# fengweie/UDA_CLR

Hardware: AMD Instinct MI355X
Metric: training images/sec (512x512, src+tgt) at 1/2/4/8 MI355X; val Dice vs ref (higher is better)
Workload: dtype f32

## Files before the change

### include/uda_clr_hip.h

```cpp
#ifndef UDA_CLR_HIP_H
#define UDA_CLR_HIP_H

#include <stdint.h>

#ifdef __cplusplus
extern "C" {
#endif

#define UDA_STAT_SLOTS 16

#define UDA_ACT_NONE 0
#define UDA_ACT_RELU 1
#define UDA_ACT_RELU6 2

typedef struct uda_src {
    const float* x;
    int64_t ldx;
    int32_t N, H, W, C;
    const float* scale;
    const float* shift;
    int32_t act;
    int32_t _pad;
    const uint8_t* mask;
    int64_t ldm;
    float mask_scale;
    float _pad2;
} uda_src_t;

const char* uda_last_error(void);
int uda_version(void);

int uda_relayout_ohwi(const float* w, int O, int I, int k, float* out, void* stream);
int uda_relayout_dgrad(const float* w, int O, int I, int k, float* out, void* stream);
int uda_relayout_dw(const float* w, int C, float* out, void* stream);

#define UDA_MFMA_F32 0
#define UDA_MFMA_BF16X3 1
typedef struct uda_conv_args {
    uda_src_t src;
    const float* w;
    int32_t Cout, ksize, dil;
    int32_t origin;
    const float* bias;
    const float* addend;
    int64_t ld_add;
    float* y;
    int64_t ldy;
    double* stats;
    int32_t mfma;
    int32_t stride;
    const void* x3_src;
    const void* x3_w;
    void* workspace;
    uint64_t workspace_bytes;
} uda_conv_args_t;
int uda_conv_uses_x3(const uda_conv_args_t* a);
uint64_t uda_conv_fwd_workspace_bytes(const uda_conv_args_t* a);
int uda_conv_fwd(const uda_conv_args_t* a, void* stream);
uint64_t uda_x3_packed_bytes(int64_t rows, int K);
int uda_x3_pack(const uda_src_t* src, void* out, void* stream);

typedef struct uda_wgrad_args {
    uda_src_t src;
    const float* dy;
    int64_t lddy;
    int32_t Cout, ksize, dil;
    int32_t origin;
    float* dw;
    float* workspace;
    uint64_t workspace_bytes;
    int32_t mfma;
    int32_t stride;
    const void* x3_src;
    const void* x3_dy;
} uda_wgrad_args_t;
uint64_t uda_conv_wgrad_workspace_bytes(int64_t P, int Cout, int Cin, int ksize);
int uda_conv_wgrad_uses_x3(const uda_wgrad_args_t* a);
int uda_conv_wgrad(const uda_wgrad_args_t* a, void* stream);

uint64_t uda_dwconv_workspace_bytes(int64_t Pout, int C);
int uda_dwconv_fwd(const uda_src_t* src, const float* w9c, int stride, int dil, int border_mode,
                   float* y, int64_t ldy, double* stats , void* stream);
int uda_dwconv_dgrad(const float* dy, int64_t lddy, const float* w9c, int C, int stride, int dil,
                     int N, int H, int W, float* dx, int64_t lddx, void* stream);
int uda_dwconv_wgrad(const uda_src_t* src, const float* dy, int64_t lddy, int stride, int dil,
                     int border_mode, float* dw , float* workspace,
                     uint64_t workspace_bytes, void* stream);

int uda_dwconv_cb_fwd(const uda_src_t* src, const float* w9c, int stride, int dil, int border_mode,
                      float* y, int64_t ldy, double* stats , void* stream);
int uda_dwconv_cb_dgrad(const float* dy, int64_t lddy, const float* w9c, int C, int stride, int dil,
                        int N, int H, int W, float* dx, int64_t lddx, void* stream);
int uda_dwconv_cb_wgrad(const uda_src_t* src, const float* dy, int64_t lddy, int stride, int dil,
                        int border_mode, float* dw , float* workspace,
                        uint64_t workspace_bytes, void* stream);

uint64_t uda_stem_workspace_bytes(int64_t Pout);
int uda_stem_fwd(const float* x, int N, int H, int W, const float* w, float* y, int64_t ldy,
                 double* stats , void* stream);
int uda_stem_wgrad(const float* x, int N, int H, int W, const float* dy, int64_t lddy, float* dw,
                   float* workspace, uint64_t workspace_bytes, void* stream);

uint64_t uda_stem7_workspace_bytes(int64_t Pout);
int uda_stem7_fwd(const float* x, int N, int H, int W, const float* w, float* y, int64_t ldy,
                  double* stats , void* stream);
int uda_stem7_wgrad(const float* x, int N, int H, int W, const float* dy, int64_t lddy, float* dw,
                    float* workspace, uint64_t workspace_bytes, void* stream);
int uda_maxpool_fwd(const uda_src_t* src, float* out, int64_t ldo, uint8_t* idx, int64_t ldi, void* stream);
int uda_maxpool_bwd(const float* dz, int64_t lddz, const uint8_t* idx, int64_t ldi, int N, int H, int W,
                    int C, float* du, int64_t ldu, void* stream);
int uda_rows_stride(const float* src, int64_t ld_src, int N, int H, int W, int C, int stride, int scatter,
                    float* dst, int64_t ld_dst, void* stream);
int uda_bn_add_relu(const uda_src_t* a, const uda_src_t* b, float* out, int64_t ldo, void* stream);
int uda_relu_gate(const float* dz, int64_t lddz, const float* z, int64_t ldz, int64_t P, int C, float* out,
                  int64_t ldo, void* stream);

int uda_relayout_s2d(const float* w, int O, int C, int dgrad, float* out, void* stream);
int uda_s2d_fwd(const float* src, int64_t ld_src, int nchw_in, int N, int Hs, int Ws, int C, int valid_h,
                int valid_w, float slope, float* z, int64_t ld_z, int Hz, int Wz, void* stream);
int uda_s2d_bwd(const float* dz, const float* z_sign, int64_t ld_z, int Hz, int Wz, float slope, int N, int Hs,
                int Ws, int C, int valid_h, int valid_w, float* dst, int64_t ld_dst, int nchw_out, void* stream);
int uda_s2d_bwd_gate(const float* dz, int64_t ld_z, int Hz, int Wz, const float* gate_rows, int64_t ld_gate, float slope,
                     int N, int Hs, int Ws, int C, int valid_h, int valid_w, float* dst, int64_t ld_dst, void* stream);
int uda_x3_pack_s2d_fwd(const float* src, int64_t ld_src, int N, int Hs, int Ws, int C, int valid_h, int valid_w, float slope,
                        int Hz, int Wz, void* out, void* stream);
int uda_x3_pack_s2d_bwd(const float* dz, int64_t ld_z, int Hz, int Wz, const float* gate_rows, int64_t ld_gate, float slope,
                        int N, int Hs, int Ws, int C, int valid_h, int valid_w, void* out, void* stream);

int uda_bn_finalize(const double* stats, int C, double count, const float* gamma, const float* beta,
                    float* running_mean, float* running_var, float momentum, float eps, float* scale,
                    float* shift, float* mean, float* invstd, void* stream);
int uda_bn_running_replay(const float* mean, const float* invstd, int C, double count, int k, float momentum,
                          float eps, float* running_mean, float* running_var, void* stream);
int uda_bn_eval_coeffs(const float* gamma, const float* beta, const float* running_mean,
                       const float* running_var, int C, float eps, float* scale, float* shift,
                       void* stream);
int uda_tn_gain(const double* stats0, const double* stats1, int C, double count0, double count1, float eps,
                float* scale0, float* shift0, float* scale1, float* shift1, float* gain, void* stream);
int uda_tn_eval_coeffs(const float* gamma, const float* beta, const float* running_mean_source,
                       const float* running_var_source, const float* running_mean_target,
                       const float* running_var_target, int C, float eps, float* scale, float* shift, void* stream);
int uda_bn_apply(const uda_src_t* src, const float* residual, int64_t ldr, float* out, int64_t ldo,
                 void* stream);
int uda_colstats(const float* x, int64_t ldx, int64_t P, int C, int nq, double* out, void* stream);
int uda_colstats_window(const float* x, int64_t ldx, int64_t P, int C, int nq, double* out, int out_C, void* stream);
int uda_bnbwd_reduce(const float* dU, int64_t ldu, const uda_src_t* y, const float* mean,
                     const float* invstd, double* sums, void* stream);
int uda_bnbwd_finalize(const double* sums, int C, double count, int q1_border, int act,
                       const float* shift, const float* mean, const float* invstd, const float* q1_total,
                       float* c1, float* c2, float* dgamma, float* dbeta, void* stream);
int uda_bnbwd_apply(const float* dU, int64_t ldu, const uda_src_t* y, const float* mean,
                    const float* invstd, const float* c1, const float* c2, const float* addend,
                    int64_t ld_add, float* out, int64_t ldo, void* stream);
int uda_bnbwd_reduce_lowrank(const float* d, int64_t ldd, int k, const float* w, const uda_src_t* y, const float* mean,
                             const float* invstd, double* sums, void* stream);
int uda_bnbwd_apply_lowrank(const float* d, int64_t ldd, int k, const float* w, const uda_src_t* y, const float* mean,
                            const float* invstd, const float* c1, const float* c2, const float* addend, int64_t ld_add,
                            float* out, int64_t ldo, void* stream);

int uda_upsample_fwd(const float* x, int64_t ldx, int N, int h, int w, int C, float* out,
                     int64_t ldo, int H, int W, void* stream);
int uda_upsample_fwd_stats(const float* x, int64_t ldx, int N, int h, int w, int C, float* out, int64_t ldo, int H, int W,
                           double* stats, int stat_C, void* stream);
int uda_mc_seg_head(const float* feature, int64_t ld_feat, int N, int h, int w, int Cf, const float* low, int64_t ld_low,
                    int Cl, int64_t P_low, const float* boundary, int64_t ld_bnd, int H, int W, const float* scale,
                    const float* shift, int act, const uint8_t* mask, int64_t ldm, float mask_scale, const float* weight,
                    int64_t ldw, const float* bias, float* out, int64_t ldo, void* stream);
int uda_upsample_bwd(const float* dout, int64_t ldo, int N, int H, int W, int C, float* dx,
                     int64_t ldx, int h, int w, void* stream);
int uda_head_upsample_fwd(const float* x, int64_t ldx, int N, int h, int w, int C, float* out,
                          int H, int W, void* stream);
int uda_head_upsample_bwd(const float* dout, int N, int C, int H, int W, float* dx, int64_t ldx,
                          int h, int w, int accumulate, void* stream);
int uda_gap_fwd(const float* x, int64_t ldx, int N, int HW, int C, float scale, float* out,
                int64_t ldo, void* stream);
int uda_broadcast_rows(const float* g, int64_t ldg, int N, int HW, int C, float scale,
                       const float* addend, int64_t ld_add, float* out, int64_t ldo, void* stream);

int uda_dropout_mask(uint8_t* mask, int64_t ldm, int64_t P, int C, float p, uint64_t seed,
                     uint64_t offset, void* stream);

int uda_seg_loss_fwd(const float* o, const float* map, int64_t n_o, const float* b, const float* boundary,
                     int64_t n_b, float* loss3, double* workspace2, void* stream);
int uda_seg_loss_bwd(const float* o, const float* map, int64_t n_o, const float* b, const float* boundary,
                     int64_t n_b, const float* gscale, float* d_o, float* d_b, void* stream);
int uda_seg_counts(const float* logits, const float* target, int B, int C, int64_t HW, float thr,
                   uint64_t* counts, void* stream);

int uda_mc_stats(const float* preds, int T, int64_t n, float* std_map, float* mean_map, void* stream);
int uda_proto_weights(int mode, int B, int h, int w, int H, int W, const float* map, const float* logits,
                      int64_t ldl, const float* std_map, const float* mean_map, float* wts, float* mask0,
                      float* mask1, void* stream);
uint64_t uda_proto_workspace_bytes(int64_t P, int C);
int uda_proto_reduce(const float* feat, int64_t ldf, int64_t P, int C, const float* wts, double* sums,
                     float* workspace, uint64_t workspace_bytes, void* stream);
int uda_proto_finalize(const double* sums, int C, float* centroids , void* stream);
int uda_proto_bwd(const float* feat, int64_t ldf, int64_t P, int C, const float* wts, const double* sums,
                  const float* dC, float* coef_ws , float* d_feat, int64_t ldd,
                  int accumulate, float* d_w, void* stream);

int uda_feat_dot4(const float* feat, int64_t ldf, int64_t P, int C, const float* coef, float* out, void* stream);
int uda_feat_rank4(const float* wts, const float* coef, int64_t P, int C, float* d_feat, int64_t ldd,
                   int accumulate, void* stream);

int uda_adam_step(float* params, const float* grads, float* exp_avg, float* exp_avg_sq, int64_t n, double lr,
                  double beta1, double beta2, double eps, int64_t step, void* stream);

int uda_upconv_fused_stats(int h, int w, int H, int W, int C, int dil);
int uda_upconv_fwd(const float* g, int64_t ldg, int N, int h, int w, int C, int dil, const float* addend, int64_t ld_add,
                   int64_t addend_rows, float* y, int64_t ldy, int H, int W, double* stats, void* stream);
int uda_upconv_bwd(const float* dy, int64_t ldy, int N, int H, int W, int C, int dil, float* dg, int64_t ldg, int h, int w,
                   void* stream);

size_t uda_postprocess_workspace_bytes(int B, int H, int W);
int uda_postprocess(const float* pred, int B, int H, int W, float thr_cup, float thr_disc, int sweeps, uint8_t* out,
                    int* not_converged, void* workspace, size_t workspace_bytes, void* stream);

size_t uda_normalize_tf_workspace_bytes(int B, int H, int W);
int uda_normalize_tf(const uint8_t* image_hwc, const uint8_t* label, int B, int H, int W, const double* gauss_w, int radius,
                     float* image, float* map, float* boundary, void* workspace, size_t workspace_bytes, void* stream);
int uda_field_smooth(const double* noise, int B, int H, int W, const double* weights_dev, int radius, double alpha, double* tmp,
                     double* out, void* stream);
int uda_photometric_u8(uint8_t* image_hwc, int B, int H, int W, const int* sp_pos, const int* sp_count, const int* sp_value,
                       int sp_max, const uint8_t* lut, const int* erase_box, void* stream);
int uda_elastic_warp(const uint8_t* image_hwc, const uint8_t* label, const double* dx, const double* dy, const uint8_t* apply,
                     int B, int H, int W, uint8_t* image_out, uint8_t* label_out, void* stream);

int uda_proto_align_fwd(const float* cur_src, const float* cur_tgt, const float* prev_src, const float* prev_tgt, float keep,
                        float decay, int C, float* new_src, float* new_tgt, float* losses2, void* stream);
int uda_proto_align_bwd(const float* new_src, const float* new_tgt, const float* g_intra, float w_src, float w_tgt, int C,
                        float* d_cur_src, float* d_cur_tgt, void* stream);
int uda_adv_loss_fwd(const float* d1, int n1, const float* d2, int n2, float label, float scale, float* loss, void* stream);
int uda_adv_loss_bwd(const float* d1, int n1, const float* d2, int n2, float label, float scale, const float* g, float* g1,
                     float* g2, void* stream);
int uda_adv_s2d_fwd(const float* logits_nchw, int N, int C, int H, int W, int pre_op, float* z, int64_t ld_z, int Hz, int Wz,
                    void* stream);
int uda_adv_s2d_bwd(const float* dz, int64_t ld_z, int Hz, int Wz, const float* logits_nchw, int N, int C, int H, int W,
                    int pre_op, float* d_logits_nchw, void* stream);

#ifdef __cplusplus
}
#endif
#endif
```

### uda_clr_amd/csrc/bn_elementwise.hip

```cpp
#include "common.h"
#include <stdlib.h>

int uda_reduce_partials(const float* part, int nrows, int ncols, double* out, hipStream_t st);

#define RED_ITER 32
#define RED_CBLK 1024
#define RED_CBLK_SUM 128

__device__ __forceinline__ void st4_guard(float* p, const float v[4], int nvalid) {
    if (nvalid >= 4) {
        uda_st4(p, make_float4(v[0], v[1], v[2], v[3]));
    } else {
#pragma unroll
        for (int j = 0; j < 4; ++j)
            if (j < nvalid) p[j] = v[j];
    }
}

__global__ void bn_finalize_kernel(const double* __restrict__ stats, int C, double count,
                                   const float* __restrict__ gamma, const float* __restrict__ beta,
                                   float* __restrict__ rmean, float* __restrict__ rvar, float momentum, float eps,
                                   float* __restrict__ scale, float* __restrict__ shift,
                                   float* __restrict__ mean, float* __restrict__ invstd) {
    const int c = blockIdx.x * blockDim.x + threadIdx.x;
    if (c >= C) return;
    double s1 = 0.0, s2 = 0.0;
#pragma unroll
    for (int k = 0; k < UDA_STAT_SLOTS; ++k) {
        s1 += stats[(k * 2 + 0) * C + c];
        s2 += stats[(k * 2 + 1) * C + c];
    }
    const double m = s1 / count;
    double var = s2 / count - m * m;
    if (var < 0.0) var = 0.0;
    const double istd = 1.0 / sqrt(var + (double)eps);
    const double sc = (double)gamma[c] * istd;
    mean[c] = (float)m;
    invstd[c] = (float)istd;
    scale[c] = (float)sc;
    shift[c] = (float)((double)beta[c] - m * sc);
    const double unbiased = var * (count / (count > 1.0 ? count - 1.0 : 1.0));
    rmean[c] = (1.f - momentum) * rmean[c] + momentum * (float)m;
    rvar[c] = (1.f - momentum) * rvar[c] + momentum * (float)unbiased;
}

__global__ void bn_eval_coeffs_kernel(const float* __restrict__ gamma, const float* __restrict__ beta,
                                      const float* __restrict__ rmean, const float* __restrict__ rvar, int C,
                                      float eps, float* __restrict__ scale, float* __restrict__ shift) {
    const int c = blockIdx.x * blockDim.x + threadIdx.x;
    if (c >= C) return;
    const double sc = (double)gamma[c] / sqrt((double)rvar[c] + (double)eps);
    scale[c] = (float)sc;
    shift[c] = (float)((double)beta[c] - (double)rmean[c] * sc);
}

extern "C" int uda_bn_finalize(const double* stats, int C, double count, const float* gamma, const float* beta,
                               float* running_mean, float* running_var, float momentum, float eps, float* scale,
                               float* shift, float* mean, float* invstd, void* stream) {
    UDA_REQUIRE(stats && gamma && beta && running_mean && running_var && scale && shift && mean && invstd && C > 0 && count > 0,
                "uda_bn_finalize: bad args");
    hipLaunchKernelGGL(bn_finalize_kernel, dim3(uda_cdiv(C, 256)), dim3(256), 0, (hipStream_t)stream, stats, C, count,
                       gamma, beta, running_mean, running_var, momentum, eps, scale, shift, mean, invstd);
    UDA_LAUNCH_CHECK("bn_finalize");
    return 0;
}

__global__ void bn_running_replay_kernel(const float* __restrict__ mean, const float* __restrict__ invstd, int C,
                                         double count, int k, float momentum, float eps, float* __restrict__ rmean,
                                         float* __restrict__ rvar) {
    const int c = blockIdx.x * blockDim.x + threadIdx.x;
    if (c >= C) return;
    const double is = (double)invstd[c];
    double var = 1.0 / (is * is) - (double)eps;
    if (var < 0.0) var = 0.0;
    const double unbiased = var * (count / (count > 1.0 ? count - 1.0 : 1.0));
    const double a = pow(1.0 - (double)momentum, (double)k);
    rmean[c] = (float)(a * (double)rmean[c] + (1.0 - a) * (double)mean[c]);
    rvar[c] = (float)(a * (double)rvar[c] + (1.0 - a) * unbiased);
}

extern "C" int uda_bn_running_replay(const float* mean, const float* invstd, int C, double count, int k, float momentum,
                                     float eps, float* running_mean, float* running_var, void* stream) {
    UDA_REQUIRE(mean && invstd && running_mean && running_var && C > 0 && count > 0 && k >= 1, "uda_bn_running_replay: bad args");
    hipLaunchKernelGGL(bn_running_replay_kernel, dim3(uda_cdiv(C, 256)), dim3(256), 0, (hipStream_t)stream, mean, invstd, C,
                       count, k, momentum, eps, running_mean, running_var);
    UDA_LAUNCH_CHECK("bn_running_replay");
    return 0;
}

extern "C" int uda_bn_eval_coeffs(const float* gamma, const float* beta, const float* running_mean,
                                  const float* running_var, int C, float eps, float* scale, float* shift, void* stream) {
    UDA_REQUIRE(gamma && beta && running_mean && running_var && scale && shift && C > 0, "uda_bn_eval_coeffs: bad args");
    hipLaunchKernelGGL(bn_eval_coeffs_kernel, dim3(uda_cdiv(C, 256)), dim3(256), 0, (hipStream_t)stream, gamma, beta,
                       running_mean, running_var, C, eps, scale, shift);
    UDA_LAUNCH_CHECK("bn_eval_coeffs");
    return 0;
}

__device__ __forceinline__ double tn_block_sum(double v, double* red) {
    for (int d = 32; d > 0; d >>= 1) v += __shfl_xor(v, d);
    if ((threadIdx.x & 63) == 0) red[threadIdx.x >> 6] = v;
    __syncthreads();
    double t = 0.0;
    for (int w = 0; w < (int)(blockDim.x >> 6); ++w) t += red[w];
    __syncthreads();
    return t;
}

__global__ __launch_bounds__(256) void tn_gain_kernel(const double* __restrict__ st0, const double* __restrict__ st1, int C,
                                                      double n0, double n1, float eps, float* __restrict__ scale0,
                                                      float* __restrict__ shift0, float* __restrict__ scale1,
                                                      float* __restrict__ shift1, float* __restrict__ gain) {
    __shared__ double red[4];
    double part = 0.0;
    for (int c = threadIdx.x; c < C; c += 256) {
        double r[2];
#pragma unroll
        for (int h = 0; h < 2; ++h) {
            const double* st = h ? st1 : st0;
            const double n = h ? n1 : n0;
            double s1 = 0.0, s2 = 0.0;
            for (int k = 0; k < UDA_STAT_SLOTS; ++k) {
                s1 += st[(k * 2 + 0) * C + c];
                s2 += st[(k * 2 + 1) * C + c];
            }
            const double m = s1 / n;
            double var = s2 / n - m * m;
            if (var < 0.0) var = 0.0;
            r[h] = m / sqrt(var * (n / (n - 1.0)) + (double)eps);
        }
        const double prob = 1.0 / (1.0 + fabs(r[0] - r[1]));
        gain[c] = (float)prob;
        part += prob;
    }
    const double total = tn_block_sum(part, red);
    for (int c = threadIdx.x; c < C; c += 256) {
        const float g = (float)(1.0 + (double)C * (double)gain[c] / total);
        gain[c] = g;
        scale0[c] *= g; shift0[c] *= g;
        scale1[c] *= g; shift1[c] *= g;
    }
}

extern "C" int uda_tn_gain(const double* stats0, const double* stats1, int C, double count0, double count1, float eps,
                           float* scale0, float* shift0, float* scale1, float* shift1, float* gain, void* stream) {
    UDA_REQUIRE(stats0 && stats1 && scale0 && shift0 && scale1 && shift1 && gain && C > 0, "uda_tn_gain: bad args");
    UDA_REQUIRE(count0 > 1 && count1 > 1, "uda_tn_gain: each domain half needs more than 1 value per channel (got %g, %g)", count0, count1);
    hipLaunchKernelGGL(tn_gain_kernel, dim3(1), dim3(256), 0, (hipStream_t)stream, stats0, stats1, C, count0, count1, eps,
                       scale0, shift0, scale1, shift1, gain);
    UDA_LAUNCH_CHECK("tn_gain");
    return 0;
}

__global__ __launch_bounds__(256) void tn_eval_coeffs_kernel(const float* __restrict__ gamma, const float* __restrict__ beta,
                                                             const float* __restrict__ rms, const float* __restrict__ rvs,
                                                             const float* __restrict__ rmt, const float* __restrict__ rvt, int C,
                                                             float eps, float* __restrict__ scale, float* __restrict__ shift) {
    __shared__ double red[4];
    double part = 0.0;
    for (int c = threadIdx.x; c < C; c += 256) {
        const double rs = (double)rms[c] / sqrt((double)rvs[c] + (double)eps);
        const double rt = (double)rmt[c] / sqrt((double)rvt[c] + (double)eps);
        const double prob = 1.0 / (1.0 + fabs(rs - rt));
        scale[c] = (float)prob;
        part += prob;
    }
    const double total = tn_block_sum(part, red);
    for (int c = threadIdx.x; c < C; c += 256) {
        const double g = 1.0 + (double)C * (double)scale[c] / total;
        const double sc = (double)gamma[c] / sqrt((double)rvt[c] + (double)eps);
        scale[c] = (float)(sc * g);
        shift[c] = (float)(((double)beta[c] - (double)rmt[c] * sc) * g);
    }
}

extern "C" int uda_tn_eval_coeffs(const float* gamma, const float* beta, const float* running_mean_source,
                                  const float* running_var_source, const float* running_mean_target,
                                  const float* running_var_target, int C, float eps, float* scale, float* shift, void* stream) {
    UDA_REQUIRE(gamma && beta && running_mean_source && running_var_source && running_mean_target && running_var_target &&
                scale && shift && C > 0, "uda_tn_eval_coeffs: bad args");
    hipLaunchKernelGGL(tn_eval_coeffs_kernel, dim3(1), dim3(256), 0, (hipStream_t)stream, gamma, beta, running_mean_source,
                       running_var_source, running_mean_target, running_var_target, C, eps, scale, shift);
    UDA_LAUNCH_CHECK("tn_eval_coeffs");
    return 0;
}

#define EW_ITER 16
__global__ __launch_bounds__(256) void bn_apply_kernel(uda_src_t s, const float* __restrict__ res, int64_t ldr,
                                                       float* __restrict__ out, int64_t ldo, int64_t P) {
    const int C = s.C, cblk0 = blockIdx.y * RED_CBLK;
    const int Cb = min(RED_CBLK, C - cblk0), G = (Cb + 3) >> 2, PP = 256 / G;
    const int tid = threadIdx.x, cg = tid % G, pl = tid / G;
    if (pl >= PP) return;
    const int c0 = cblk0 + cg * 4;
    Xf4 xf;
    uda_load_xf4(xf, s.scale, s.shift, c0, C);
    const bool has_xf = s.scale != nullptr;
    const int64_t base = (int64_t)blockIdx.x * (PP * EW_ITER);
#pragma unroll 4
    for (int it = 0; it < EW_ITER; ++it) {
        const int64_t p = base + (int64_t)it * PP + pl;
        if (p >= P) break;
        const float4 xv = uda_ld4(s.x + p * s.ldx + c0);
        float v[4] = {xv.x, xv.y, xv.z, xv.w};
        uint32_t mk = 0x01010101u;
        if (s.mask) mk = *reinterpret_cast<const uint32_t*>(s.mask + p * s.ldm + c0);
        float r[4] = {0.f, 0.f, 0.f, 0.f};
        if (res) {
            const float4 rv = uda_ld4(res + p * ldr + c0);
            r[0] = rv.x; r[1] = rv.y; r[2] = rv.z; r[3] = rv.w;
        }
#pragma unroll
        for (int j = 0; j < 4; ++j) {
            float u = v[j];
            if (has_xf) u = u * xf.sc[j] + xf.sh[j];
            u = uda_act(u, s.act);
            if (s.mask) u *= (float)((mk >> (8 * j)) & 0xffu) * s.mask_scale;
            v[j] = u + r[j];
        }
        st4_guard(out + p * ldo + c0, v, C - c0);
    }
}

static int src_check(const uda_src_t* s, const char* who) {
    UDA_REQUIRE(s && s->x && uda_aligned16(s->x) && s->ldx % 4 == 0 && s->ldx >= ((s->C + 3) / 4) * 4 && s->C > 0,
                "%s: src must be 16-byte aligned with ldx %% 4 == 0 and >= round4(C)", who);
    UDA_REQUIRE((s->scale == nullptr) == (s->shift == nullptr), "%s: scale/shift must come together", who);
    if (s->mask) UDA_REQUIRE(s->ldm % 4 == 0 && s->ldm >= ((s->C + 3) / 4) * 4 && (reinterpret_cast<uintptr_t>(s->mask) & 3u) == 0,
                             "%s: bad mask layout", who);
    return 0;
}
// ... 370 lines not shown
```

### uda_clr_amd/csrc/igemm_conv.hip

```cpp
#include <algorithm>
#include "common.h"
#include <stdlib.h>
#include "igemm_args.h"

typedef float f32x16 __attribute__((ext_vector_type(16)));


#define IGC_MIN_WAVES(TM, TN, PIPE) ((PIPE) ? 2 : ((TM) * (TN) <= 3 ? 4 : 3))
template <int TM, int TN, int WM, int WN, bool PIPE = false, int XF = -1>
__global__ __launch_bounds__(256) void igemm_conv_kernel(ConvKArgs a) {
    constexpr int BM = 32 * TM * WM, BN = 32 * TN * WN;
    constexpr int A_IT = BM / 32, B_IT = BN / 32;
    constexpr int TILE = (BM + BN) * IG_LD;
    extern __shared__ __attribute__((aligned(16))) float smem[];

    const int tid = threadIdx.x, lane = tid & 63, wave = tid >> 6;
    const int wm = wave / WN, wn = wave % WN;
    const int lid = uda_xcd_remap(blockIdx.x, a.nMt * a.nNt);
    const int mt = lid / a.nNt, nt = lid % a.nNt;
    const int H = a.src.H, W = a.src.W, C = a.src.C;
    const int64_t P = (int64_t)a.src.N * H * W;
    const int64_t m0 = (int64_t)mt * BM;
    const int n0 = nt * BN;

// ... 153 lines not shown
            for (int i = 0; i < TM; ++i) af[i] = uda_ld4(&As[(arow + 32 * i) * IG_LD + g * 8 + koff]);
#pragma unroll
            for (int j = 0; j < TN; ++j) bf[j] = uda_ld4(&Bs[(brow + 32 * j) * IG_LD + g * 8 + koff]);
#pragma unroll
            for (int s = 0; s < 4; ++s) {
#pragma unroll
                for (int i = 0; i < TM; ++i) {
                    const float av = s == 0 ? af[i].x : s == 1 ? af[i].y : s == 2 ? af[i].z : af[i].w;
#pragma unroll
                    for (int j = 0; j < TN; ++j) {
                        const float bv = s == 0 ? bf[j].x : s == 1 ? bf[j].y : s == 2 ? bf[j].z : bf[j].w;
                        acc[i][j] = __builtin_amdgcn_mfma_f32_32x32x2f32(av, bv, acc[i][j], 0, 0, 0);
                    }
                }
            }
        }
    };
    float* As = smem;
    float* Bs = smem + BM * IG_LD;
    if constexpr (PIPE) {
        float* As1 = smem + TILE;
        float* Bs1 = As1 + BM * IG_LD;
        issue(0, R0);
        issue(1, R1);
        stage(R0, As, Bs);
        issue(2, R0);
        for (int c = 0; c < nchunks; c += 2) {
            __syncthreads();
            stage(R1, As1, Bs1);
            issue(c + 3, R1);
            math(As, Bs);
            __syncthreads();
            stage(R0, As, Bs);
            issue(c + 4, R0);
            if (c + 1 < nchunks) math(As1, Bs1);
        }
    } else {
        issue(0, R0);
        for (int c = 0; c < nchunks; ++c) {
            __syncthreads();
            stage(R0, As, Bs);
            __syncthreads();
            if (c + 1 < nchunks) issue(c + 1, R0);
            math(As, Bs);
        }
    }

    const int colb = n0 + wn * TN * 32 + (lane & 31);
    const bool vec_ok = uda_aligned16_dev(a.y) && (a.ldy & 3) == 0 && (!a.addend || (uda_aligned16_dev(a.addend) && (a.ld_add & 3) == 0));
    __syncthreads();
    float* patch = smem + wave * (32 * IG_LD);
    float s1[TN], s2[TN];
#pragma unroll
    for (int j = 0; j < TN; ++j) {
        s1[j] = 0.f;
        s2[j] = 0.f;
        const int col = colb + 32 * j;
        const bool cok = col < a.Cout;
        const float bv = (cok && a.bias) ? a.bias[col] : 0.f;
#pragma unroll
        for (int i = 0; i < TM; ++i) {
            const int64_t rbase = m0 + wm * TM * 32 + 32 * i;
#pragma unroll
            for (int r = 0; r < 16; ++r) {
                const int rl = (r & 3) + 8 * (r >> 2) + 4 * (lane >> 5);
                const float v = acc[i][j][r] + bv;
                if (cok && rbase + rl < P) {
                    s1[j] += v;
                    s2[j] += v * v;
                }
                if (vec_ok) {
                    patch[rl * IG_LD + (lane & 31)] = v;
                } else if (cok && rbase + rl < P) {
                    a.y[(rbase + rl) * a.ldy + col] = a.addend ? v + a.addend[(rbase + rl) * a.ld_add + col] : v;
                }
            }
            if (vec_ok) {
                const int cb = n0 + wn * TN * 32 + 32 * j + (lane & 7) * 4;
#pragma unroll
                for (int rq = 0; rq < 4; ++rq) {
                    const int rl = rq * 8 + (lane >> 3);
                    const int64_t row = rbase + rl;
                    float4 o = uda_ld4(&patch[rl * IG_LD + (lane & 7) * 4]);
                    if (row < P && cb < a.Cout) {
                        if (cb + 3 < a.Cout) {
                            if (a.addend) {
                                const float4 ad = uda_ld4(a.addend + row * a.ld_add + cb);
                                o.x += ad.x; o.y += ad.y; o.z += ad.z; o.w += ad.w;
                            }
                            uda_st4(a.y + row * a.ldy + cb, o);
                        } else {
                            const float ov[4] = {o.x, o.y, o.z, o.w};
                            for (int q = 0; q < 4; ++q)
                                if (cb + q < a.Cout) a.y[row * a.ldy + cb + q] = a.addend ? ov[q] + a.addend[row * a.ld_add + cb + q] : ov[q];
                        }
                    }
                }
            }
        }
    }
    if (a.stats) {
        __syncthreads();
        float* red = smem;
#pragma unroll
        for (int j = 0; j < TN; ++j) {
            const float t1 = s1[j] + __shfl_xor(s1[j], 32);
            const float t2 = s2[j] + __shfl_xor(s2[j], 32);
            if (lane < 32) {
                const int cl = wn * TN * 32 + 32 * j + lane;
                red[(wm * 2 + 0) * BN + cl] = t1;
                red[(wm * 2 + 1) * BN + cl] = t2;
            }
        }
        __syncthreads();
        double* dst = a.stats + (int64_t)(mt % UDA_STAT_SLOTS) * 2 * a.Cout;
        for (int e = tid; e < 2 * BN; e += 256) {
            const int qd = e / BN, cl = e % BN;
            if (n0 + cl < a.Cout) {
                float t = 0.f;
#pragma unroll
                for (int m = 0; m < WM; ++m) t += red[(m * 2 + qd) * BN + cl];
                atomicAdd(&dst[qd * a.Cout + n0 + cl], (double)t);
            }
        }
    }
}

__global__ void reduce_partials_kernel(const float* __restrict__ part, int nrows, int ncols,
                                       int rows_per_seg, double* __restrict__ out) {
    __shared__ double red[4][64];
    const int cl = threadIdx.x & 63, rg = threadIdx.x >> 6;
    const int col = blockIdx.x * 64 + cl;
    const int r0 = blockIdx.y * rows_per_seg;
    const int r1 = min(nrows, r0 + rows_per_seg);
    double s = 0.0;
    if (col < ncols)
        for (int r = r0 + rg; r < r1; r += 4) s += (double)part[(int64_t)r * ncols + col];
    red[rg][cl] = s;
    __syncthreads();
    if (rg == 0 && col < ncols) atomicAdd(&out[col], red[0][cl] + red[1][cl] + red[2][cl] + red[3][cl]);
}

int uda_reduce_partials(const float* part, int nrows, int ncols, double* out, hipStream_t st) {
    int segs = nrows / 64;
    if (segs < 1) segs = 1;
    if (segs > 64) segs = 64;
    const int rps = (nrows + segs - 1) / segs;
    dim3 grid(uda_cdiv(ncols, 64), uda_cdiv(nrows, rps));
    hipLaunchKernelGGL(reduce_partials_kernel, grid, dim3(256), 0, st, part, nrows, ncols, rps, out);
    UDA_LAUNCH_CHECK("reduce_partials");
    return 0;
}

static inline int uda_k_row(int C, int ksize) {
    const int Kc = ((C + 3) / 4) * 4;
    if (ksize == 1 || Kc < IG_BK) return ksize * ksize * Kc;
    return ((Kc + IG_BK - 1) / IG_BK) * ksize * ksize * IG_BK;
}

static int check_src(const uda_src_t& s, const char* who) {
    UDA_REQUIRE(s.x && uda_aligned16(s.x), "%s: src.x must be 16-byte aligned", who);
    UDA_REQUIRE(s.ldx % 4 == 0 && s.ldx >= ((s.C + 3) / 4) * 4, "%s: src.ldx=%lld must be a multiple of 4 and >= round4(C=%d)",
                who, (long long)s.ldx, s.C);
    UDA_REQUIRE(s.N > 0 && s.H > 0 && s.W > 0 && s.C > 0, "%s: bad src dims", who);
    UDA_REQUIRE((s.scale == nullptr) == (s.shift == nullptr), "%s: scale/shift must come together", who);
    if (s.mask) UDA_REQUIRE(s.ldm % 4 == 0 && (reinterpret_cast<uintptr_t>(s.mask) & 3u) == 0 && s.ldm >= ((s.C + 3) / 4) * 4,
                            "%s: mask must be 4-byte aligned with ldm %% 4 == 0", who);
    return 0;
}

__global__ __launch_bounds__(256) void conv_cout1_kernel(ConvKArgs a) {
    const int lane = threadIdx.x & 63;
    const int64_t p = (int64_t)blockIdx.x * 4 + (threadIdx.x >> 6);
    const int H = a.src.H, W = a.src.W;
    const int64_t P = (int64_t)a.src.N * H * W;
    if (p >= P) return;
    const int pw = (int)(p % W), ph = (int)((p / W) % H);
    const int T = a.ksize * a.ksize;
    float acc = 0.f;
    for (int t = 0; t < T; ++t) {
        const int th = t / a.ksize;
        const int hh = ph + (th - a.cen) * a.dil, ww = pw + (t - th * a.ksize - a.cen) * a.dil;
        if (hh < 0 || hh >= H || ww < 0 || ww >= W) continue;
        const float* xr = a.src.x + (p + (int64_t)(hh - ph) * W + (ww - pw)) * a.src.ldx;
        for (int c = lane * 4; c < a.Kc; c += 256) {
            const int kq = (T == 1 || a.Kc < IG_BK) ? t * a.Kc + c : ((c / IG_BK) * T + t) * IG_BK + (c % IG_BK);
            const float4 xv = uda_ld4(xr + c), wv = uda_ld4(a.w + kq);
            float s = xv.x * wv.x;
            if (c + 1 < a.src.C) s += xv.y * wv.y;
            if (c + 2 < a.src.C) s += xv.z * wv.z;
            if (c + 3 < a.src.C) s += xv.w * wv.w;
            acc += s;
        }
    }
#pragma unroll
    for (int o = 32; o > 0; o >>= 1) acc += __shfl_xor(acc, o);
    if (lane == 0) {
        float v = acc + (a.bias ? a.bias[0] : 0.f);
        if (a.addend) v += a.addend[p * a.ld_add];
        a.y[p * a.ldy] = v;
    }
}

template <int NO>
__global__ __launch_bounds__(256) void conv_heads_kernel(ConvKArgs a) {
    extern __shared__ __attribute__((aligned(16))) float hsm[];
    const int Kc = a.Kc, C = a.src.C;
    for (int e = threadIdx.x; e < Kc; e += 256) {
        const bool in = e < C;
        hsm[e] = (in && a.src.scale) ? a.src.scale[e] : 1.f;
        hsm[Kc + e] = (in && a.src.shift) ? a.src.shift[e] : 0.f;
#pragma unroll
        for (int o = 0; o < NO; ++o) hsm[(2 + o) * Kc + e] = in ? a.w[(int64_t)o * a.Ktot + e] : 0.f;
    }
    __syncthreads();
    const int l16 = threadIdx.x & 15, pl = threadIdx.x >> 4;
    const int64_t P = (int64_t)a.src.N * a.src.H * a.src.W;
    const float alo = a.src.act == ACT_NONE ? -INFINITY : 0.f, ahi = a.src.act == ACT_RELU6 ? 6.f : INFINITY;
    const float ms = a.src.mask_scale;
    const int G = Kc >> 2;
    for (int it = 0; it < 8; ++it) {
        const int64_t p = (int64_t)blockIdx.x * 128 + it * 16 + pl;
        float acc[NO];
#pragma unroll
        for (int o = 0; o < NO; ++o) acc[o] = 0.f;
        if (p < P) {
            const float* xr = a.src.x + p * a.src.ldx;
            for (int g = l16; g < G; g += 16) {
                const int c = g * 4;
                float4 xv = uda_ld4(xr + c);
                const float4 sc = uda_ld4(&hsm[c]), sh = uda_ld4(&hsm[Kc + c]);
                if (c + 4 > C) {
                    if (c + 1 >= C) xv.y = 0.f;
                    if (c + 2 >= C) xv.z = 0.f;
                    xv.w = 0.f;
                }
                float u[4] = {__builtin_amdgcn_fmed3f(xv.x * sc.x + sh.x, alo, ahi), __builtin_amdgcn_fmed3f(xv.y * sc.y + sh.y, alo, ahi),
                              __builtin_amdgcn_fmed3f(xv.z * sc.z + sh.z, alo, ahi), __builtin_amdgcn_fmed3f(xv.w * sc.w + sh.w, alo, ahi)};
                if (a.src.mask) {
                    uint32_t mk = *reinterpret_cast<const uint32_t*>(a.src.mask + p * a.src.ldm + c);
                    if (c + 4 > C) mk &= 0xffffffffu >> (8 * (c + 4 - C));
                    u[0] *= (float)(mk & 0xffu) * ms; u[1] *= (float)((mk >> 8) & 0xffu) * ms;
                    u[2] *= (float)((mk >> 16) & 0xffu) * ms; u[3] *= (float)(mk >> 24) * ms;
                }
#pragma unroll
                for (int o = 0; o < NO; ++o) {
                    const float4 wv = uda_ld4(&hsm[(2 + o) * Kc + c]);
                    acc[o] += u[0] * wv.x + u[1] * wv.y + u[2] * wv.z + u[3] * wv.w;
                }
            }
        }
#pragma unroll
        for (int o = 0; o < NO; ++o) {
#pragma unroll
            for (int d = 8; d > 0; d >>= 1) acc[o] += __shfl_xor(acc[o], d);
        }
        if (l16 == 0 && p < P) {
#pragma unroll
            for (int o = 0; o < NO; ++o) {
                float v = acc[o] + (a.bias ? a.bias[o] : 0.f);
                if (a.addend) v += a.addend[p * a.ld_add + o];
                a.y[p * a.ldy + o] = v;
            }
        }
    }
}

template <int KH, int NB>
__global__ __launch_bounds__(256, 2) void conv1x1_stream_kernel(ConvKArgs a, int64_t P, int ntiles, int ngroups) {
    const int lane = threadIdx.x & 63, r = lane & 31, h = lane >> 5;
    const int wave = (int)((blockIdx.x * blockDim.x + threadIdx.x) >> 6), nwaves = (int)((gridDim.x * blockDim.x) >> 6);
    const int K = 2 * KH;
    const int grp = wave % ngroups, col0 = grp * (NB * 32);
    float b[NB][KH];
#pragma unroll
    for (int nb = 0; nb < NB; ++nb) {
        const int col = col0 + nb * 32 + r;
#pragma unroll
        for (int q = 0; q < KH / 4; ++q) {
            float4 v = make_float4(0.f, 0.f, 0.f, 0.f);
            if (col < a.Cout) v = uda_ld4(a.w + (int64_t)col * K + h * KH + 4 * q);
            b[nb][4 * q] = v.x; b[nb][4 * q + 1] = v.y; b[nb][4 * q + 2] = v.z; b[nb][4 * q + 3] = v.w;
        }
    }
    const bool has_xf = a.src.scale != nullptr;
    const bool xf16 = has_xf && ((reinterpret_cast<uintptr_t>(a.src.scale) | reinterpret_cast<uintptr_t>(a.src.shift)) & 15) == 0;
    const float alo = a.src.act == ACT_NONE ? -INFINITY : 0.f, ahi = a.src.act == ACT_RELU6 ? 6.f : INFINITY;
    double s1[NB], s2[NB];
#pragma unroll
    for (int nb = 0; nb < NB; ++nb) s1[nb] = s2[nb] = 0.0;
    constexpr int OOB = 0x7ffffff0;
    const int ldy4 = (int)a.ldy * 4, lda4 = (int)a.ld_add * 4;
    for (int t = wave / ngroups; t < ntiles; t += nwaves / ngroups) {
        const int64_t p0 = (int64_t)t * 32;
        const int64_t p = min(p0 + r, P - 1);
        float av[KH];
#pragma unroll
        for (int q = 0; q < KH / 4; ++q) {
            const float4 v = uda_ld4(a.src.x + p * a.src.ldx + h * KH + 4 * q);
            av[4 * q] = v.x; av[4 * q + 1] = v.y; av[4 * q + 2] = v.z; av[4 * q + 3] = v.w;
        }
        if (has_xf) {
#pragma unroll
            for (int q = 0; q < KH / 4; ++q) {
                float4 sc, sh;
                if (xf16) {
                    sc = uda_ld4(a.src.scale + h * KH + 4 * q);
// ... 281 lines not shown
    constexpr int ARPP = 256 / AV, BRPP = 256 / BV;
    constexpr int APASS = WGN_BKP / ARPP, BPASS = WGN_BKP / BRPP;
    __shared__ __attribute__((aligned(16))) float smem[WGN_BKP * (BM + BN)];
    float* As = smem;
    float* Bs = smem + WGN_BKP * BM;

    const int tid = threadIdx.x, lane = tid & 63, wave = tid >> 6;
    const int wm = wave / WN, wn = wave % WN;
    const int cot = blockIdx.x / a.nJt, jt = blockIdx.x % a.nJt;
    const int split = blockIdx.y;
    const int H = a.src.H, W = a.src.W, C = a.src.C;
    const int64_t P = (int64_t)a.src.N * H * W;

    const int acv = (tid % AV) * 4, apr = tid / AV;
    const int co = cot * BM + acv;
    const int bjv = (tid % BV) * 4, bpr = tid / BV;
    const int j0 = jt * BN + bjv;
    const bool jok = j0 < a.Jtot;
    int t = 0, ci = j0;
    if (a.ksize >= 2 && jok) {
        t = j0 / a.Kc;
        ci = j0 - t * a.Kc;
    }
    int dh = 0, dw = 0;
    if (a.ksize >= 2) {
        const int th = a.ksize == 3 ? t / 3 : t >> 1;
        dh = (th - a.cen) * a.dil;
        dw = (t - th * a.ksize - a.cen) * a.dil;
    }
    Xf4 xf;
    uda_load_xf4(xf, a.src.scale, a.src.shift, ci, jok ? C : 0);
    const bool has_xf = a.src.scale != nullptr;
    const int act = a.src.act;
    const float ms = a.src.mask_scale;

    float4 areg[APASS], breg[BPASS];
    uint32_t bmask[BPASS];
    unsigned bok = 0, aok = 0;

    auto issue = [&](int chunk) {
        const int64_t p0 = (int64_t)chunk * WGN_BKP;
        const int64_t plast = P - 1;
        const int coc = min(co, a.Cout > 4 ? a.Cout - 4 : 0);
        aok = 0;
#pragma unroll
        for (int i = 0; i < APASS; ++i) {
            const int64_t p = p0 + apr + i * ARPP;
            areg[i] = uda_ld4(a.dy + min(p, plast) * a.lddy + (co < a.Cout ? co : coc));
            aok |= ((p < P && co < a.Cout) ? 1u : 0u) << i;
        }
        bok = 0;
#pragma unroll
        for (int i = 0; i < BPASS; ++i) {
            const int64_t p = p0 + bpr + i * BRPP;
            bool in = jok && p < P;
            int64_t q = min(p, plast);
            if (a.ksize >= 2) {
                const int w0 = (int)(q % W), h0 = (int)((q / W) % H);
                const int hh = h0 + dh, ww = w0 + dw;
                const bool inside = hh >= 0 && hh < H && ww >= 0 && ww < W;
                in = in && inside;
                q = inside ? q + (int64_t)dh * W + dw : q;
            }
            const int cic = jok ? ci : 0;
            breg[i] = uda_ld4(a.src.x + q * a.src.ldx + cic);
            bmask[i] = a.src.mask ? *reinterpret_cast<const uint32_t*>(a.src.mask + q * a.src.ldm + cic) : 0x01010101u;
            bok |= (in ? 1u : 0u) << i;
        }
    };
    auto stage = [&]() {
#pragma unroll
        for (int i = 0; i < APASS; ++i) {
            float v[4] = {areg[i].x, areg[i].y, areg[i].z, areg[i].w};
            const bool oka = (aok >> i) & 1u;
#pragma unroll
            for (int j = 0; j < 4; ++j)
                if (!oka || co + j >= a.Cout) v[j] = 0.f;
            uda_st4(&As[(apr + i * ARPP) * BM + acv], make_float4(v[0], v[1], v[2], v[3]));
        }
        typedef float f32x2 __attribute__((ext_vector_type(2)));
        const f32x2 sc01 = {xf.sc[0], xf.sc[1]}, sc23 = {xf.sc[2], xf.sc[3]};
        const f32x2 sh01 = {xf.sh[0], xf.sh[1]}, sh23 = {xf.sh[2], xf.sh[3]};
        const bool masked = a.src.mask != nullptr;
#pragma unroll
        for (int i = 0; i < BPASS; ++i) {
            const bool ok = (bok >> i) & 1u;
            f32x2 t01 = {breg[i].x, breg[i].y}, t23 = {breg[i].z, breg[i].w};
            if (has_xf) {
                t01 = t01 * sc01 + sh01;
                t23 = t23 * sc23 + sh23;
            }
            t01 = f32x2{uda_act(t01.x, act), uda_act(t01.y, act)};
            t23 = f32x2{uda_act(t23.x, act), uda_act(t23.y, act)};
            if (masked) {
                const uint32_t mk = bmask[i];
                t01 *= f32x2{(float)(mk & 0xffu), (float)((mk >> 8) & 0xffu)} * ms;
                t23 *= f32x2{(float)((mk >> 16) & 0xffu), (float)(mk >> 24)} * ms;
            }
            float v[4] = {t01.x, t01.y, t23.x, t23.y};
#pragma unroll
            for (int j = 0; j < 4; ++j)
                if (!(ok && (ci + j) < C)) v[j] = 0.f;
            uda_st4(&Bs[(bpr + i * BRPP) * BN + bjv], make_float4(v[0], v[1], v[2], v[3]));
        }
    };

    f32x16 acc[TM][TN];
#pragma unroll
    for (int i = 0; i < TM; ++i)
#pragma unroll
        for (int j = 0; j < TN; ++j)
#pragma unroll
            for (int r = 0; r < 16; ++r) acc[i][j][r] = 0.f;

    const int c0 = split * a.chunks_per_split;
    const int c1 = min(a.nchunks, c0 + a.chunks_per_split);
    const int acol = wm * TM * 32 + (lane & 31), bcol = wn * TN * 32 + (lane & 31);
    const int kh = lane >> 5;
    if (c0 < c1) issue(c0);
    for (int c = c0; c < c1; ++c) {
        __syncthreads();
        stage();
        __syncthreads();
        if (c + 1 < c1) issue(c + 1);
#pragma unroll
        for (int kk = 0; kk < WGN_BKP / 2; ++kk) {
            float af[TM], bf[TN];
#pragma unroll
            for (int i = 0; i < TM; ++i) af[i] = As[(2 * kk + kh) * BM + acol + 32 * i];
#pragma unroll
            for (int j = 0; j < TN; ++j) bf[j] = Bs[(2 * kk + kh) * BN + bcol + 32 * j];
#pragma unroll
            for (int i = 0; i < TM; ++i)
#pragma unroll
                for (int j = 0; j < TN; ++j)
                    acc[i][j] = __builtin_amdgcn_mfma_f32_32x32x2f32(af[i], bf[j], acc[i][j], 0, 0, 0);
        }
    }
    float* slab = a.slab + (int64_t)split * a.Cout * a.Jtot;
#pragma unroll
    for (int i = 0; i < TM; ++i)
#pragma unroll
        for (int j = 0; j < TN; ++j) {
            const int col = jt * BN + wn * TN * 32 + 32 * j + (lane & 31);
#pragma unroll
            for (int r = 0; r < 16; ++r) {
                const int row = cot * BM + wm * TM * 32 + 32 * i + (r & 3) + 8 * (r >> 2) + 4 * (lane >> 5);
                if (row < a.Cout && col < a.Jtot) slab[(int64_t)row * a.Jtot + col] = acc[i][j][r];
            }
        }
}

template <int Q>
__global__ __launch_bounds__(256) void wgrad_reduce_kernel(const float* __restrict__ slab, int S, int Cout, int Cin, int T,
                                                           int Kc, float* __restrict__ dw) {
    constexpr int NO = 256 / Q;
    __shared__ float red[Q][NO + 1];
    const int64_t total = (int64_t)Cout * T * Cin;
    const int64_t stride = (int64_t)Cout * T * Kc;
    const int ol = threadIdx.x % NO, q = threadIdx.x / NO;
    for (int64_t e0 = (int64_t)blockIdx.x * NO; e0 < total; e0 += (int64_t)gridDim.x * NO) {
        const int64_t e = e0 + ol;
        float s = 0.f;
        int64_t dst = 0;
        if (e < total) {
            const int ci = (int)(e % Cin);
            const int t = (int)((e / Cin) % T);
            const int co = (int)(e / ((int64_t)Cin * T));
            dst = ((int64_t)co * Cin + ci) * T + t;
            const float* src = slab + ((int64_t)co * T + t) * Kc + ci;
            int k = q;
            float s0 = 0.f, s1 = 0.f, s2 = 0.f, s3 = 0.f;
            for (; k + 3 * Q < S; k += 4 * Q) {
                s0 += src[(int64_t)k * stride];
                s1 += src[(int64_t)(k + Q) * stride];
                s2 += src[(int64_t)(k + 2 * Q) * stride];
                s3 += src[(int64_t)(k + 3 * Q) * stride];
            }
            for (; k < S; k += Q) s0 += src[(int64_t)k * stride];
            s = (s0 + s1) + (s2 + s3);
        }
        red[q][ol] = s;
        __syncthreads();
        if (q == 0 && e < total) {
            float acc[8];
#pragma unroll
            for (int j = 0; j < 8; ++j) acc[j] = 0.f;
#pragma unroll
            for (int j = 0; j < Q; ++j) acc[j & 7] += red[j][ol];
            dw[dst] = ((acc[0] + acc[1]) + (acc[2] + acc[3])) + ((acc[4] + acc[5]) + (acc[6] + acc[7]));
        }
        __syncthreads();
    }
}

struct WgradPlan {
    int bm, bn, nCot, nJt, S, cps, nchunks;
};

static WgradPlan wgrad_plan(int64_t P, int Cout, int Cin, int ksize) {
    WgradPlan p;
    const int Kc = ((Cin + 3) / 4) * 4, J = ksize * ksize * Kc;
    const int cm = Cout <= 32 ? 32 : (Cout <= 64 ? 64 : 128);
    const int cn = J <= 32 ? 32 : (J <= 64 ? 64 : 128);
    const bool big = Cout >= 192 && J >= 256 && uda_cdiv(P, WG_BKP) >= 4096;
    if (big) { p.bm = 256; p.bn = 256; }
    else if (cm == 128 && cn == 32) { p.bm = 128; p.bn = 32; }
    else if (cm == 32 && cn == 128) { p.bm = 32; p.bn = 128; }
    else if (cm <= 64 && cn <= 64) { p.bm = 64; p.bn = 64; }
    else { p.bm = 128; p.bn = 128; }
    p.nCot = uda_cdiv(Cout, p.bm);
    p.nJt = uda_cdiv(J, p.bn);
    p.nchunks = uda_cdiv(P, ((p.bm == 128 && p.bn == 128) || p.bm == 256) ? WG_BKP : WGN_BKP);
    int S = (p.bm == 256 ? 512 : 1024) / (p.nCot * p.nJt);
    if (S > p.nchunks / 4) S = p.nchunks / 4;
    if (S < 1) S = 1;
    const int scap = (int64_t)Cout * J <= 8192 ? 1024 : 256;
    if (S > scap) S = scap;
    p.cps = uda_cdiv(p.nchunks, S);
    p.S = uda_cdiv(p.nchunks, p.cps);
    return p;
}

extern "C" uint64_t uda_conv_wgrad_workspace_bytes(int64_t P, int Cout, int Cin, int ksize) {
    const WgradPlan p = wgrad_plan(P, Cout, Cin, ksize);
    const int Kc = ((Cin + 3) / 4) * 4;
    return (uint64_t)p.S * Cout * ksize * ksize * Kc * sizeof(float);
}

extern "C" int uda_conv_wgrad_uses_x3(const uda_wgrad_args_t* a) {
    if (!a || a->mfma != UDA_MFMA_BF16X3 || a->ksize < 1 || a->ksize > 3) return 0;
    const int sd = a->stride <= 1 ? 1 : a->stride;
    const int64_t P = (int64_t)a->src.N * ((a->src.H - 1) / sd + 1) * ((a->src.W - 1) / sd + 1);
    const WgradPlan p = wgrad_plan(P, a->Cout, a->src.C, a->ksize);
    const bool wide = p.bm == 256 || (p.bm == 128 && p.bn == 128);
    return wide && wgrad_x3_eligible(a->src.C, a->Cout, a->ksize, P) ? 1 : 0;
}

extern "C" int uda_conv_wgrad(const uda_wgrad_args_t* a, void* stream) {
    hipStream_t st = (hipStream_t)stream;
    UDA_REQUIRE(a != nullptr, "uda_conv_wgrad: null args");
    if (int e = check_src(a->src, "uda_conv_wgrad")) return e;
    UDA_REQUIRE(a->ksize >= 1 && a->ksize <= 3, "uda_conv_wgrad: ksize must be 1, 2 or 3");
    UDA_REQUIRE(a->ksize != 2 || a->origin == 0 || a->origin == 1, "uda_conv_wgrad: origin must be 0 or 1 for ksize 2");
    UDA_REQUIRE(a->dy && uda_aligned16(a->dy) && a->lddy % 4 == 0 && a->lddy >= ((a->Cout + 3) / 4) * 4,
                "uda_conv_wgrad: dy must be 16-byte aligned with lddy %% 4 == 0 and >= round4(Cout)");
    const int sd = a->stride <= 1 ? 1 : a->stride;
    UDA_REQUIRE(sd <= 2, "uda_conv_wgrad: stride must be 1 or 2");
    const int Ho = (a->src.H - 1) / sd + 1, Wo = (a->src.W - 1) / sd + 1;
    const int64_t P = (int64_t)a->src.N * Ho * Wo;
    const WgradPlan p = wgrad_plan(P, a->Cout, a->src.C, a->ksize);
    UDA_REQUIRE(a->workspace && a->workspace_bytes >= uda_conv_wgrad_workspace_bytes(P, a->Cout, a->src.C, a->ksize),
                "uda_conv_wgrad: workspace too small");
    UDA_REQUIRE(sd == 1 || p.bm == 256 || (p.bm == 128 && p.bn == 128),
                "uda_conv_wgrad: stride 2 is built on the wide-tile kernels only (Cout > 64, K > 64)");
    WgradKArgs k;
    k.src = a->src;
    k.stride = sd; k.Ho = Ho; k.Wo = Wo;
    k.dy = a->dy;
    k.lddy = a->lddy;
    k.Cout = a->Cout;
    k.ksize = a->ksize;
    k.dil = a->dil;
    k.cen = a->ksize == 3 ? 1 : (a->ksize == 2 ? a->origin : 0);
    k.Kc = ((a->src.C + 3) / 4) * 4;
    k.Jtot = a->ksize * a->ksize * k.Kc;
    k.slab = a->workspace;
    k.nCot = p.nCot;
    k.nJt = p.nJt;
    k.chunks_per_split = p.cps;
    k.nchunks = p.nchunks;
    dim3 grid(p.nCot * p.nJt, p.S);
    int S_used = p.S;
    if (uda_conv_wgrad_uses_x3(a)) { if (int e = launch_wgrad_x3(k, P, p.S, a->x3_src, a->x3_dy, st, S_used)) return e; }
    else if (p.bm == 256) { if (int e = launch_wgrad_ws(k, p.S, true, st)) return e; }
    else if (p.bm == 128 && p.bn == 128) { if (int e = launch_wgrad_ws(k, p.S, false, st)) return e; }
    else if (p.bm == 64) hipLaunchKernelGGL((igemm_wgrad_kernel<1, 1, 2, 2>), grid, dim3(256), 0, st, k);
    else if (p.bm == 128) hipLaunchKernelGGL((igemm_wgrad_kernel<1, 1, 4, 1>), grid, dim3(256), 0, st, k);
    else hipLaunchKernelGGL((igemm_wgrad_kernel<1, 1, 1, 4>), grid, dim3(256), 0, st, k);
    UDA_LAUNCH_CHECK("igemm_wgrad");
    const int T = a->ksize * a->ksize;
    const int64_t total = (int64_t)a->Cout * T * a->src.C;
    if (S_used > 256)
        hipLaunchKernelGGL(wgrad_reduce_kernel<64>, dim3(uda_cdiv(total, 4) > 4096 ? 4096 : uda_cdiv(total, 4)), dim3(256), 0, st,
                           k.slab, S_used, a->Cout, a->src.C, T, k.Kc, a->dw);
    else
        hipLaunchKernelGGL(wgrad_reduce_kernel<8>, dim3(uda_cdiv(total, 32) > 4096 ? 4096 : uda_cdiv(total, 32)), dim3(256), 0, st,
                           k.slab, S_used, a->Cout, a->src.C, T, k.Kc, a->dw);
    UDA_LAUNCH_CHECK("wgrad_reduce");
    return 0;
}

__device__ __forceinline__ void uda_k_decode(int64_t e, int T, int Kr, int Kc, int& c, int& t, int& row) {
    const int k = (int)(e % Kr);
    row = (int)(e / Kr);
    if (T == 1) {
        c = k;
        t = 0;
    } else if (Kc < IG_BK) {
        t = k / Kc;
        c = k - t * Kc;
    } else {
        const int chunk = k / IG_BK;
        t = chunk % T;
        c = (chunk / T) * IG_BK + (k % IG_BK);
    }
}
__global__ void relayout_ohwi_kernel(const float* __restrict__ w, int O, int I, int T, int Kr, float* __restrict__ out) {
    const int64_t total = (int64_t)O * Kr;
    const int Kc = ((I + 3) / 4) * 4;
    for (int64_t e = (int64_t)blockIdx.x * blockDim.x + threadIdx.x; e < total; e += (int64_t)gridDim.x * blockDim.x) {
        int ci, t, o;
        uda_k_decode(e, T, Kr, Kc, ci, t, o);
        out[e] = ci < I ? w[((int64_t)o * I + ci) * T + t] : 0.f;
    }
}
__global__ void relayout_dgrad_kernel(const float* __restrict__ w, int O, int I, int T, int Kr, float* __restrict__ out) {
    const int64_t total = (int64_t)I * Kr;
    const int Kc = ((O + 3) / 4) * 4;
    for (int64_t e = (int64_t)blockIdx.x * blockDim.x + threadIdx.x; e < total; e += (int64_t)gridDim.x * blockDim.x) {
        int o, t, ci;
        uda_k_decode(e, T, Kr, Kc, o, t, ci);
        out[e] = o < O ? w[((int64_t)o * I + ci) * T + (T - 1 - t)] : 0.f;
    }
}
__global__ void relayout_dw_kernel(const float* __restrict__ w, int C, float* __restrict__ out) {
    const int e = blockIdx.x * blockDim.x + threadIdx.x;
    if (e < 9 * C) out[e] = w[(e % C) * 9 + e / C];
}

static inline int grid_for(int64_t total) {
    int g = uda_cdiv(total, 256);
    return g > 4096 ? 4096 : (g < 1 ? 1 : g);
}

extern "C" int uda_relayout_ohwi(const float* w, int O, int I, int k, float* out, void* stream) {
    UDA_REQUIRE(w && out && O > 0 && I > 0 && (k >= 1 && k <= 3), "uda_relayout_ohwi: bad args");
    const int Kr = uda_k_row(I, k);
    hipLaunchKernelGGL(relayout_ohwi_kernel, dim3(grid_for((int64_t)O * Kr)), dim3(256), 0, (hipStream_t)stream,
                       w, O, I, k * k, Kr, out);
    UDA_LAUNCH_CHECK("relayout_ohwi");
    return 0;
}
extern "C" int uda_relayout_dgrad(const float* w, int O, int I, int k, float* out, void* stream) {
    UDA_REQUIRE(w && out && O > 0 && I > 0 && (k >= 1 && k <= 3), "uda_relayout_dgrad: bad args");
    const int Kr = uda_k_row(O, k);
    hipLaunchKernelGGL(relayout_dgrad_kernel, dim3(grid_for((int64_t)I * Kr)), dim3(256), 0, (hipStream_t)stream,
                       w, O, I, k * k, Kr, out);
    UDA_LAUNCH_CHECK("relayout_dgrad");
    return 0;
}
extern "C" int uda_relayout_dw(const float* w, int C, float* out, void* stream) {
    UDA_REQUIRE(w && out && C > 0, "uda_relayout_dw: bad args");
    hipLaunchKernelGGL(relayout_dw_kernel, dim3(uda_cdiv(9 * C, 256)), dim3(256), 0, (hipStream_t)stream, w, C, out);
    UDA_LAUNCH_CHECK("relayout_dw");
    return 0;
}
```

### uda_clr_amd/engine.py

```python
from __future__ import annotations

from typing import Dict, Optional

import torch

import os as _os

_MC_VIRTUAL = _os.environ.get("UDA_CLR_MC_VIRTUAL", "1") != "0"
_NATIVE_S2 = _os.environ.get("UDA_CLR_NATIVE_STRIDE2", "1") != "0"
POISON_BUFFERS = False

from .acts import ACT_NONE, ACT_RELU, ACT_RELU6, Act, BNRec, nchw_view, round4
from .domain_split import DomainSplit

BN_EPS = 1e-5
BN_MOMENTUM = 0.1

_MBV2 = ((1, 16, 1, 1), (6, 24, 2, 2), (6, 32, 3, 2), (6, 64, 4, 2), (6, 96, 3, 1),
         (6, 160, 3, 2), (6, 320, 1, 1))

DROPOUT = {"aspp.dropout": 0.5, "decoder.last_conv_boundary.3": 0.5,
           "decoder.last_conv_boundary.7": 0.1, "decoder.last_conv.2": 0.1}


def block_plan(output_stride: int = 16):
    plan, inp, cur, rate = [], 32, 2, 1
    for t, c, n, s in _MBV2:
        if cur == output_stride:
            stride, dil = 1, rate
            rate *= s
        else:
            stride, dil = s, 1
            cur *= s
        for i in range(n):
            plan.append((inp, c, stride if i == 0 else 1, dil, t))
            inp = c
    return plan


def _rows(g: torch.Tensor) -> torch.Tensor:
    n, c, h, w = g.shape
    return g.permute(0, 2, 3, 1).reshape(n * h * w, c)


STAT_SLOTS = 16


class _Arena:

    def __init__(self, like, n_doubles):
        self.buf = torch.zeros(n_doubles, dtype=torch.float64, device=like.device)
        self.off = 0

    def take(self, nq, C, halves=1):
        n = halves * STAT_SLOTS * nq * C
        if self.off + n > self.buf.numel():
            raise RuntimeError("statistics arena exhausted")
        v = self.buf[self.off:self.off + n]
        v = v.view(STAT_SLOTS, nq, C) if halves == 1 else v.view(halves, STAT_SLOTS, nq, C)
        self.off += n
        return v


class _Ctx:
    __slots__ = ("S", "N", "dims", "w_cache", "params", "x", "arena", "nbt", "bnlog", "tn_repeat", "need_grad")

    def __init__(self):
        self.S = {}
        self.w_cache = {}
        self.arena = None
        self.nbt = []
        self.bnlog = []
        self.tn_repeat = False


def resnet_plan(output_stride: int = 16, layers=(3, 4, 23)):
    if output_stride == 16:
        strides, dils = (1, 2, 2, 1), (1, 1, 1, 2)
    elif output_stride == 8:
        strides, dils = (1, 2, 1, 1), (1, 1, 2, 4)
    else:
        raise NotImplementedError
    plan, inp = [], 64
    for li, (planes, n) in enumerate(zip((64, 128, 256), layers), start=1):
        for b in range(n):
            st = strides[li - 1] if b == 0 else 1
            plan.append(("backbone.layer%d.%d" % (li, b), inp, planes, st, dils[li - 1],
                         b == 0 and (st != 1 or inp != 4 * planes)))
            inp = 4 * planes
    for b, mg in enumerate((1, 2, 4)):
        st = strides[3] if b == 0 else 1
        plan.append(("backbone.layer4.%d" % b, inp, 512, st, mg * dils[3], b == 0 and (st != 1 or inp != 2048)))
        inp = 2048
    return plan


class GeneratorEngine:
    C_FEAT = 256

    def __init__(self, kernels, output_stride: int = 16, seed: int = 1337, backbone: str = "mobilenet",
                 transnorm: bool = False):
        self.tn = bool(transnorm)
        self.K = DomainSplit(kernels) if self.tn else kernels
        self.os = output_stride
        self.backbone = backbone
        self.dils = (1, 6, 12, 18) if output_stride == 16 else (1, 12, 24, 36)
        self.seed = seed
        self.rng_offset = 0
        self.nonfinite = None
        if backbone == "mobilenet":
            self.blocks = block_plan(output_stride)
            self.c_high, self.c_low = 320, 24
            n = 32
            for inp, oup, stride, dil, t in self.blocks:
                n += (inp * t if t != 1 else 0) + inp * t + oup
        elif backbone == "resnet":
            self.rblocks = resnet_plan(output_stride)
            self.c_high, self.c_low = 2048, 256
            n = 64
            for pre, inp, planes, stride, dil, has_ds in self.rblocks:
                n += 2 * planes + 4 * planes * (2 if has_ds else 1)
        elif backbone == "xception":
            from .networks.backbone.xception import exit_plan, xception_plan
            self.xblocks, self.xexit = xception_plan(output_stride), exit_plan(output_stride)
            self.c_high, self.c_low = 2048, 128
            n = 32 + 64
            for name, inp, planes, stride, has_skip, seps in self.xblocks:
                n += sum(ci + co for _, ci, co, _, _ in seps) + (planes if has_skip else 0)
            n += sum(ci + co for _, _, ci, co, _ in self.xexit)
        else:
            raise NotImplementedError("backbone %r" % (backbone,))
        self.bn_channels = n + 5 * 256 + 256 + 48 + 256 + 256 + 305

    def _check_arena(self, ctx):
        if ctx.arena is not None:
            bad = ~torch.isfinite(ctx.arena.buf.sum())
            self.nonfinite = bad if self.nonfinite is None else (self.nonfinite | bad)

    def pop_nonfinite(self):
        f, self.nonfinite = self.nonfinite, None
        return f

    @staticmethod
    def _empty(x, *shape, dtype=torch.float32):
        t = torch.empty(shape, dtype=dtype, device=x.device)
        if POISON_BUFFERS and dtype == torch.float32 and t.dim() == 2:
            t.copy_(torch.tensor([float("nan"), float("inf"), -float("inf"), 3.0e38], device=x.device)[
                torch.arange(t.shape[0], device=x.device) % 4].unsqueeze(1).expand_as(t))
        return t

    def _buf(self, x, P, C):
        return self._empty(x, P, round4(C))[:, :C]

    def _stats(self, ctx, C, training):
        return ctx.arena.take(2, C, 2 if self._split(ctx) else 1) if training else None

    def _split(self, ctx):
        return self.tn and not ctx.tn_repeat

    def _w(self, ctx, key, kind):
        ck = (key, kind)
        if ck not in ctx.w_cache:
            w = ctx.params[key]
            K, CF = self.K, self.C_FEAT

            def taps(t):
                return t[:, :CF].permute(2, 3, 0, 1).reshape(9 * t.shape[0], CF, 1, 1).contiguous()
            ctx.w_cache[ck] = {"ohwi": K.relayout_ohwi, "dgrad": K.relayout_dgrad,
                               "dw": K.relayout_dw,
                               "dwflip": lambda t: K.relayout_dw(t).flip(0).contiguous(),
                               "up_taps": lambda t: K.relayout_ohwi(taps(t)),
                               "up_taps_dgrad": lambda t: K.relayout_dgrad(taps(t)),
                               "low_ohwi": lambda t: K.relayout_ohwi(t[:, CF:].contiguous()),
                               "low_dgrad": lambda t: K.relayout_dgrad(t[:, CF:].contiguous())}[kind](w)
        return ctx.w_cache[ck]

    def _bn(self, ctx, prefix, stats, count, training, scale, shift, mean=None, invstd=None,
            q1=False, N=None) -> Optional[BNRec]:
        p = ctx.params
        g, b = p[prefix + ".weight"], p[prefix + ".bias"]
        if self.tn:
            return self._tn(ctx, prefix, stats, count, training, scale, shift, mean, invstd, q1, ctx.N if N is None else N)
        rm, rv = p[prefix + ".running_mean"], p[prefix + ".running_var"]
        if training:
            if count <= 1:
                raise ValueError("Expected more than 1 value per channel when training (%s)" % prefix)
            self.K.bn_finalize(stats, float(count), g, b, rm, rv, BN_MOMENTUM, BN_EPS,
                               scale, shift, mean, invstd)
            nbt = p.get(prefix + ".num_batches_tracked")
            if nbt is not None:
                ctx.nbt.append(nbt)
            rec = BNRec(prefix, mean, invstd, float(count), q1)
            ctx.bnlog.append((prefix, rec))
            return rec
        self.K.bn_eval_coeffs(g, b, rm, rv, BN_EPS, scale, shift)
        if not ctx.need_grad:
            return None
        istd = torch.rsqrt(rv + BN_EPS)
        if mean is not None:
            mean.copy_(rm)
            invstd.copy_(istd)
            return BNRec(prefix, mean, invstd, float("inf"), q1, frozen=True)
        return BNRec(prefix, rm, istd, float("inf"), q1, frozen=True)

    def _tn(self, ctx, prefix, stats, count, training, scale, shift, mean, invstd, q1, N):
        p, K = ctx.params, self.K
        g, b = p[prefix + ".weight"], p[prefix + ".bias"]
        rms, rvs = p[prefix + ".running_mean_source"], p[prefix + ".running_var_source"]
        rmt, rvt = p[prefix + ".running_mean_target"], p[prefix + ".running_var_target"]
        if not training:
            K.tn_eval_coeffs(g, b, rms, rvs, rmt, rvt, BN_EPS, scale, shift)
            if not ctx.need_grad:
                return None
            rs, rt = rms / torch.sqrt(rvs + BN_EPS), rmt / torch.sqrt(rvt + BN_EPS)
            prob = 1.0 / (1.0 + (rs - rt).abs())
            gain = 1.0 + prob.numel() * prob / prob.sum()
            istd = torch.rsqrt(rvt + BN_EPS)
            if mean is not None:
                mean.copy_(rmt)
                invstd.copy_(istd)
                return BNRec(prefix, mean, invstd, float("inf"), q1, gain, frozen=True)
            return BNRec(prefix, rmt, istd, float("inf"), q1, gain, frozen=True)
        if ctx.tn_repeat:
            if count <= 1:
                raise ValueError("Expected more than 1 value per channel when training (%s)" % prefix)
            K.bn_finalize(stats, float(count), g, b, rms.clone(), rvs.clone(), BN_MOMENTUM, BN_EPS, scale, shift, mean, invstd)
            scale.mul_(2.0)
            shift.mul_(2.0)
            rec = BNRec(prefix, mean, invstd, float(count), q1)
            ctx.bnlog.append((prefix, rec))
            return rec
        n0 = N // 2
        per_image = count // N
        counts = (float(n0 * per_image), float((N - n0) * per_image))
        if min(counts) <= 1:
            raise ValueError("Expected more than 1 value per channel when training (%s, TransNorm halves of %d and %d "
                             "images)" % (prefix, n0, N - n0))
        for h, (rm, rv) in enumerate(((rms, rvs), (rmt, rvt))):
            K.bn_finalize(stats[h], counts[h], g, b, rm, rv, BN_MOMENTUM, BN_EPS, scale[h], shift[h], mean[h], invstd[h])
        gain = torch.empty_like(g)
        K.tn_gain(stats[0], stats[1], counts[0], counts[1], BN_EPS, scale[0], shift[0], scale[1], shift[1], gain)
        ctx.nbt.append(p[prefix + ".num_batches_tracked"])
        rec = BNRec(prefix, mean, invstd, counts, q1, gain)
        ctx.bnlog.append((prefix, rec))
        return rec

    def _coef(self, ctx, x, C, training):
        return self._empty(x, 4, 2, C) if (self._split(ctx) and training) else self._empty(x, 4, C)

    def _bn_act(self, ctx, prefix, y, N, H, W, stats, count, training, act, mask=None,
                mask_scale=1.0, q1=False) -> Act:
        C = y.shape[1]
        coef = self._coef(ctx, y, C, training)
        rec = self._bn(ctx, prefix, stats, count, training, coef[0], coef[1], coef[2], coef[3], q1, N)
        return Act(y, N, H, W, coef[0], coef[1], act, mask, mask_scale, rec,
                   split=N // 2 if (self._split(ctx) and training) else 0)

    def _mask(self, x, name, P, C, N, H, W, training, masks):
        if not training:
            return None, 1.0
        p = DROPOUT[name]
        m = torch.empty((P, round4(C)), dtype=torch.uint8, device=x.device)[:, :C]
        if masks is not None:
            m.copy_(_rows(masks[name].to(x.device)))
        else:
            self.K.dropout_mask(m, p, self.seed, self.rng_offset)
            self.rng_offset += 1
        return m, 1.0 / (1.0 - p)

    def _conv0(self, ctx, feature, xf, N, H16, W16, H4, W4, out, stats, y0=None):
        K, key = self.K, "decoder.last_conv_boundary.0.weight"
        CF = self.C_FEAT
        Cout = out.shape[1]
        if y0 is None:
            y0 = self._empty(out, out.shape[0], Cout)
            K.conv(Act(xf[:, CF:CF + 48], N, H4, W4), self._w(ctx, key, "low_ohwi"), 3, 1, y0)
        g = self._empty(out, feature.shape[0], 9 * Cout)
        K.conv(Act(feature, N, H16, W16), self._w(ctx, key, "up_taps"), 1, 1, g)
        if self.tn and stats is not None:
            K.upconv_fwd(g, N, H16, W16, out, H4, W4, addend=y0)
            K.colstats(out, stats, N=N)
        else:
            K.upconv_fwd(g, N, H16, W16, out, H4, W4, addend=y0, stats=stats)
        return y0

    def _mobilenet_forward(self, ctx, x, training):
        K, S, params = self.K, ctx.S, ctx.params
        N, _, Hin, Win = x.shape
        H, W = (Hin - 1) // 2 + 1, (Win - 1) // 2 + 1
        y0 = self._buf(x, N * H * W, 32)
        st = self._stats(ctx, 32, training)
        K.stem_fwd(x, params["backbone.features.0.0.weight"], y0, st)
        a = self._bn_act(ctx, "backbone.features.0.1", y0, N, H, W, st, N * H * W, training, ACT_RELU6)
        S["stem"] = a
        recs = []
        low = None
        for i, (inp, oup, stride, dil, t) in enumerate(self.blocks, start=1):
            pre = "backbone.features.%d" % i
            zin, H, W = a, a.H, a.W
            hid = inp * t
            if t != 1:
                ye = self._buf(x, N * H * W, hid)
                st = self._stats(ctx, hid, training)
                K.conv(zin, self._w(ctx, pre + ".conv.0.weight", "ohwi"), 1, 1, ye, stats=st)
                cnt = N * (H + 2 * dil) * (W + 2 * dil)
                e = self._bn_act(ctx, pre + ".conv.1", ye, N, H, W, st, cnt, training, ACT_RELU6, q1=True)
                border, kd, kdb, kp, kpb = 1, ".conv.3", ".conv.4", ".conv.6", ".conv.7"
            else:
                e, border, kd, kdb, kp, kpb = zin, 0, ".conv.0", ".conv.1", ".conv.3", ".conv.4"
            Ho, Wo = (H - 1) // stride + 1, (W - 1) // stride + 1
            Po = N * Ho * Wo
            yd = self._buf(x, Po, hid)
            st = self._stats(ctx, hid, training)
            K.dwconv_fwd(e, self._w(ctx, pre + kd + ".weight", "dw"), stride, dil, border, yd, st)
            d = self._bn_act(ctx, pre + kdb, yd, N, Ho, Wo, st, Po, training, ACT_RELU6)
            yp = self._buf(x, Po, oup)
            st = self._stats(ctx, oup, training)
            K.conv(d, self._w(ctx, pre + kp + ".weight", "ohwi"), 1, 1, yp, stats=st)
            pb = self._bn_act(ctx, pre + kpb, yp, N, Ho, Wo, st, Po, training, ACT_NONE)
            use_res = stride == 1 and inp == oup
            z = self._buf(x, Po, oup)
            K.bn_apply(pb, z, zin.x if use_res else None)
            a = Act(z, N, Ho, Wo)
            recs.append(dict(pre=pre, t=t, stride=stride, dil=dil, zin=zin, e=e, d=d, pb=pb,
                             use_res=use_res, border=border, keys=(kd, kdb, kp, kpb)))
            if i == 3:
                low = a
        S["blocks"] = recs
# ... 160 lines not shown
            else:
                dU_stem = dUe
        dy0 = self._bn_backward(ctx, G, S["stem"], dU_stem)
        dw0 = torch.empty_like(ctx.params["backbone.features.0.0.weight"])
        K.stem_wgrad(x, dy0, dw0)
        G["backbone.features.0.0.weight"] = dw0

    def _sep_forward(self, ctx, v, pre, bn_key, cout, stride, dil, training, act):
        K, N = self.K, ctx.N
        Ho, Wo = (v.H - 1) // stride + 1, (v.W - 1) // stride + 1
        Po, cin = N * Ho * Wo, v.C
        yd = self._buf(v.x, Po, cin)
        st = self._stats(ctx, cin, training)
        K.dwconv_fwd(v, self._w(ctx, pre + ".conv1.weight", "dw"), stride, dil, 0, yd, st)
        d = self._bn_act(ctx, pre + ".bn", yd, N, Ho, Wo, st, Po, training, ACT_NONE)
        yp = self._buf(v.x, Po, cout)
        st = self._stats(ctx, cout, training)
        K.conv(d, self._w(ctx, pre + ".pointwise.weight", "ohwi"), 1, 1, yp, stats=st)
        p = self._bn_act(ctx, bn_key, yp, N, Ho, Wo, st, Po, training, act)
        return dict(pre=pre, v=v, d=d, p=p, stride=stride, dil=dil)

    def _xception_forward(self, ctx, x, training):
        K, S, params = self.K, ctx.S, ctx.params
        N, _, Hin, Win = x.shape
        H, W = (Hin - 1) // 2 + 1, (Win - 1) // 2 + 1
        y1 = self._buf(x, N * H * W, 32)
        st = self._stats(ctx, 32, training)
        K.stem_fwd(x, params["backbone.conv1.weight"], y1, st)
        a1 = self._bn_act(ctx, "backbone.bn1", y1, N, H, W, st, N * H * W, training, ACT_RELU)
        y2 = self._buf(x, N * H * W, 64)
        st = self._stats(ctx, 64, training)
        K.conv(a1, self._w(ctx, "backbone.conv2.weight", "ohwi"), 3, 1, y2, stats=st)
        a = self._bn_act(ctx, "backbone.bn2", y2, N, H, W, st, N * H * W, training, ACT_RELU)
        S["xstem"] = dict(a1=a1, a2=a)
        recs, low = [], None
        for name, inp, planes, stride, has_skip, seps in self.xblocks:
            pre = "backbone." + name
            u = a
            seprecs, v = [], u
            for j, (idx, ci, co, s, d) in enumerate(seps):
                last = j == len(seps) - 1
                r = self._sep_forward(ctx, v, "%s.rep.%d" % (pre, idx), "%s.rep.%d" % (pre, idx + 1), co, s, d, training,
                                      ACT_NONE if last else ACT_RELU)
                seprecs.append(r)
                v = r["p"]
            Ho, Wo = v.H, v.W
            Po = N * Ho * Wo
            us = ad = None
            if has_skip:
                us = u
                if stride != 1:
                    usb = self._buf(x, Po, inp)
                    K.rows_stride(u.x, N, u.H, u.W, stride, usb)
                    us = Act(usb, N, Ho, Wo, u.scale, u.shift, u.act, bn=u.bn)
                yk = self._buf(x, Po, planes)
                st = self._stats(ctx, planes, training)
                K.conv(us, self._w(ctx, pre + ".skip.weight", "ohwi"), 1, 1, yk, stats=st)
                ad = self._bn_act(ctx, pre + ".skipbn", yk, N, Ho, Wo, st, Po, training, ACT_NONE)
            zo = self._buf(x, Po, planes)
            K.bn_add_relu(v, ad if has_skip else u, zo)
            a = Act(zo, N, Ho, Wo)
            recs.append(dict(pre=pre, stride=stride, u=u, us=us, ad=ad, seps=seprecs, zo=a))
            if name == "block1":
                low = a
        exits = []
        for sep, bn, ci, co, d in self.xexit:
            r = self._sep_forward(ctx, a, "backbone." + sep, "backbone." + bn, co, 1, d, training, ACT_RELU)
            exits.append(r)
            a = r["p"]
        out = self._buf(x, a.P, a.C)
        K.bn_apply(a, out, None)
        S["xblocks"], S["xexit"] = recs, exits
        return Act(out, N, a.H, a.W), low

    def _sep_backward(self, ctx, G, r, dP):
        K, x, N = self.K, ctx.x, ctx.N
        pre, v, d, p, stride, dil = r["pre"], r["v"], r["d"], r["p"], r["stride"], r["dil"]
        dyp = self._buf(x, p.P, p.C)
        self._bn_backward(ctx, G, p, dP, out=dyp)
        self._wgrad(ctx, G, pre + ".pointwise.weight", d, dyp, 1, 1)
        dUd = self._buf(x, d.P, d.C)
        self._dgrad(ctx, pre + ".pointwise.weight", dyp, N, d.H, d.W, 1, 1, dUd)
        del dyp
        dyd = self._bn_backward(ctx, G, d, dUd)
        key = pre + ".conv1.weight"
        dwg = torch.empty_like(ctx.params[key])
        K.dwconv_wgrad(v, dyd, stride, dil, 0, dwg)
        G[key] = dwg
        dV = self._buf(x, v.P, v.C)
        if stride == 1:
            K.dwconv_fwd(Act(dyd, N, v.H, v.W), self._w(ctx, key, "dwflip"), 1, dil, 0, dV, None)
        else:
            K.dwconv_dgrad(dyd, self._w(ctx, key, "dw"), stride, dil, N, v.H, v.W, dV)
        return dV

    def _xception_backward(self, ctx, G, d_a, d_low):
        K, S, x = self.K, ctx.S, ctx.x
        N = ctx.N
        dP = d_a
        for r in reversed(S["xexit"]):
            dP = self._sep_backward(ctx, G, r, dP)
        d_z = dP
        for r in reversed(S["xblocks"]):
            pre, stride, u, us, ad, zo = r["pre"], r["stride"], r["u"], r["us"], r["ad"], r["zo"]
            if pre.endswith(".block1"):
                d_z.add_(d_low)
            g = self._buf(x, zo.P, zo.C)
            K.relu_gate(d_z, zo.x, g)
            del d_z
            seps = r["seps"]
            dP = g
            for j in range(len(seps) - 1, -1, -1):
                dP = self._sep_backward(ctx, G, seps[j], dP)
            d_u = dP
            if ad is not None:
                dyk = self._bn_backward(ctx, G, ad, g)
                self._wgrad(ctx, G, pre + ".skip.weight", us, dyk, 1, 1)
                if stride == 1:
                    self._dgrad(ctx, pre + ".skip.weight", dyk, N, u.H, u.W, 1, 1, d_u, addend=d_u)
                else:
                    d_us = self._buf(x, us.P, us.C)
                    self._dgrad(ctx, pre + ".skip.weight", dyk, N, us.H, us.W, 1, 1, d_us)
                    full = self._buf(x, u.P, u.C)
                    K.rows_stride(d_us, N, u.H, u.W, stride, full, scatter=True)
                    d_u.add_(full)
                    del d_us, full
                del dyk
            else:
                d_u.add_(g)
            del g
            d_z = d_u
        st = S["xstem"]
        a1, a2 = st["a1"], st["a2"]
        dy2 = self._bn_backward(ctx, G, a2, d_z)
        self._wgrad(ctx, G, "backbone.conv2.weight", a1, dy2, 3, 1)
        dU1 = self._buf(x, a1.P, a1.C)
        self._dgrad(ctx, "backbone.conv2.weight", dy2, N, a1.H, a1.W, 3, 1, dU1)
        del dy2
        dy1 = self._bn_backward(ctx, G, a1, dU1)
        dw1 = torch.empty_like(ctx.params["backbone.conv1.weight"])
        K.stem_wgrad(x, dy1, dw1)
        G["backbone.conv1.weight"] = dw1

    def forward(self, params: Dict[str, torch.Tensor], x: torch.Tensor, training: bool,
                need_grad: bool, masks=None, repeat_prefix: bool = False, bn_training: Optional[bool] = None,
                w_share: Optional[dict] = None):
        K = self.K
        ctx = _Ctx()
        if w_share is not None:
            ctx.w_cache = w_share
        ctx.tn_repeat = bool(repeat_prefix and self.tn)
        ctx.params, ctx.x = params, x
        ctx.need_grad = bool(need_grad)
        drop_tr = training
        training = training if bn_training is None else bool(bn_training)
        S = ctx.S
        N, _, Hin, Win = x.shape
        if Hin % 16 or Win % 16:
            raise ValueError("input height/width must be multiples of 16, got %dx%d" % (Hin, Win))
        ctx.N = N
        if training:
            ctx.arena = _Arena(x, STAT_SLOTS * 2 * self.bn_channels * (2 if self.tn else 1))
        if ctx.tn_repeat and not training:
            raise ValueError("repeat_prefix describes a training-mode (batch statistics) forward")
        if self.backbone == "mobilenet":
            a, low = self._mobilenet_forward(ctx, x, training)
        elif self.backbone == "xception":
            a, low = self._xception_forward(ctx, x, training)
        else:
            a, low = self._resnet_forward(ctx, x, training)
        a17, H16, W16 = a, a.H, a.W
        P16 = N * H16 * W16
        cat = self._empty(x, P16, 1280)
        coef = self._coef(ctx, x, 1280, training)
        split = N // 2 if (self._split(ctx) and training) else 0
        brecs = []
        for j, dl in enumerate(self.dils, start=1):
            sl = slice(256 * (j - 1), 256 * j)
            st = self._stats(ctx, 256, training)
            key = "aspp.aspp%d" % j
            K.conv(a17, self._w(ctx, key + ".atrous_conv.weight", "ohwi"), 1 if j == 1 else 3, dl,
                   cat[:, sl], stats=st)
            brecs.append(self._bn(ctx, key + ".bn", st, P16, training, coef[0][..., sl], coef[1][..., sl],
                                  coef[2][..., sl], coef[3][..., sl]))
        gp = self._empty(x, N, self.c_high)
        K.gap_fwd(a17.x, N, gp, 1.0 / (H16 * W16))
        yg = self._empty(x, N, 256)
        st = self._stats(ctx, 256, training)
        gpa = Act(gp, N, 1, 1)
        K.conv(gpa, self._w(ctx, "aspp.global_avg_pool.1.weight", "ohwi"), 1, 1, yg, stats=st)
        sl = slice(1024, 1280)
        grec = self._bn(ctx, "aspp.global_avg_pool.2", st, N, training, coef[0][..., sl], coef[1][..., sl],
                        coef[2][..., sl], coef[3][..., sl])
        K.broadcast_rows(yg, N, cat[:, sl], 1.0)
        catA = Act(cat, N, H16, W16, coef[0], coef[1], ACT_RELU, split=split)
        y1 = self._empty(x, P16, 256)
        st = self._stats(ctx, 256, training)
        K.conv(catA, self._w(ctx, "aspp.conv1.weight", "ohwi"), 1, 1, y1, stats=st)
        m, ms = self._mask(x, "aspp.dropout", P16, 256, N, H16, W16, drop_tr, masks)
        fa = self._bn_act(ctx, "aspp.bn1", y1, N, H16, W16, st, P16, training, ACT_RELU, m, ms)
        feature = self._empty(x, P16, 256)
        K.bn_apply(fa, feature, None)
        S["aspp"] = dict(a17=a17, cat=cat, coef=coef, brecs=brecs, grec=grec, gpa=gpa, yg=yg,
                         catA=catA, fa=fa)
        H4, W4 = low.H, low.W
        P4 = N * H4 * W4
        xf = self._empty(x, P4, 308)
        ylo = self._empty(x, P4, 48)
        st = self._stats(ctx, 48, training)
        K.conv(low, self._w(ctx, "decoder.conv1.weight", "ohwi"), 1, 1, ylo, stats=st)
        lo = self._bn_act(ctx, "decoder.bn1", ylo, N, H4, W4, st, P4, training, ACT_RELU)
        if ctx.tn_repeat:
            S["dec"] = dict(lo=lo, y0=None)
            ctx.dims = (N, Hin, Win, H16, W16, H4, W4)
            self._check_arena(ctx)
            ctx.arena, ctx.nbt = None, []
            return None, ctx
        K.bn_apply(lo, xf[:, 256:304], None)
        st305 = self._stats(ctx, 305, training)
        fused_up = training and 256 % (feature.shape[1] // 4) == 0
        K.upsample_fwd(feature, N, H16, W16, xf[:, 0:256], H4, W4, **({"stats": st305} if fused_up else {}))
        xbu = Act(xf[:, :304], N, H4, W4)
        yb1 = self._empty(x, P4, 256)
        st = self._stats(ctx, 256, training)
        y0 = self._conv0(ctx, feature, xf, N, H16, W16, H4, W4, yb1, st)
        m, ms = self._mask(x, "decoder.last_conv_boundary.3", P4, 256, N, H4, W4, drop_tr, masks)
        b1 = self._bn_act(ctx, "decoder.last_conv_boundary.1", yb1, N, H4, W4, st, P4, training,
                          ACT_RELU, m, ms)
        yb2 = self._empty(x, P4, 256)
        st = self._stats(ctx, 256, training)
        K.conv(b1, self._w(ctx, "decoder.last_conv_boundary.4.weight", "ohwi"), 3, 1, yb2, stats=st)
        m, ms = self._mask(x, "decoder.last_conv_boundary.7", P4, 256, N, H4, W4, drop_tr, masks)
        b2 = self._bn_act(ctx, "decoder.last_conv_boundary.5", yb2, N, H4, W4, st, P4, training,
                          ACT_RELU, m, ms)
        K.conv(b2, self._w(ctx, "decoder.last_conv_boundary.8.weight", "ohwi"), 1, 1,
               xf[:, 304:305], bias=params["decoder.last_conv_boundary.8.bias"])
        st = st305
        if training:
            if fused_up:
                K.colstats_window(xf[:, 256:305], st, 256, **({"N": N} if self.tn else {}))
            else:
                K.colstats(xf[:, :305], st, **({"N": N} if self.tn else {}))
        m, ms = self._mask(x, "decoder.last_conv.2", P4, 305, N, H4, W4, drop_tr, masks)
        sa = self._bn_act(ctx, "decoder.last_conv.0", xf[:, :305], N, H4, W4, st, P4, training,
                          ACT_RELU, m, ms)
        x1b = self._buf(x, P4, 2)
        K.conv(sa, self._w(ctx, "decoder.last_conv.3.weight", "ohwi"), 1, 1, x1b,
               bias=params["decoder.last_conv.3.bias"])
        x1 = self._empty(x, N, 2, Hin, Win)
        x2 = self._empty(x, N, 1, Hin, Win)
        K.head_upsample_fwd(x1b, N, H4, W4, x1)
        K.head_upsample_fwd(xf[:, 304:305], N, H4, W4, x2)
        S["dec"] = dict(low=low, xf=xf, lo=lo, xbu=xbu, b1=b1, b2=b2, sa=sa, x1b=x1b, feature=feature, y0=y0)
        ctx.dims = (N, Hin, Win, H16, W16, H4, W4)
        if ctx.nbt:
            torch._foreach_add_(ctx.nbt, 1)
            ctx.nbt = []
        self._check_arena(ctx)
        ctx.arena = None
        outs = (x1, x2, nchw_view(feature, N, H16, W16), nchw_view(xf[:, :304], N, H4, W4),
                nchw_view(xf[:, :305], N, H4, W4), nchw_view(x1b, N, H4, W4),
                nchw_view(xf[:, 304:305], N, H4, W4))
        return outs, (ctx if need_grad else None)

    _STOCHASTIC_BN = ("decoder.last_conv_boundary.1", "decoder.last_conv_boundary.5", "decoder.last_conv.0")

    def mc_forward(self, ctx, reps: int, passes: int, out=None, masks=None):
        K, S, params, x = self.K, ctx.S, ctx.params, ctx.x
        N, Hin, Win, H16, W16, H4, W4 = ctx.dims
        N2 = reps * N
        P16, P4 = N * H16 * W16, N * H4 * W4
        A, D = S["aspp"], S["dec"]
        fa, lo = A["fa"], D["lo"]
        if out is None:
            out = self._empty(x, passes * N2, 2, Hin, Win)
        repeated_tn = ctx.tn_repeat
        if repeated_tn and reps != 2:
            raise ValueError("the TransNorm fast path needs the batch repeated exactly twice (its halves are the two copies)")
        ctx.tn_repeat = False
        if D.get("y0") is None:
            tmp = self._empty(x, P4, 48)
            K.bn_apply(lo, tmp, None)
            D["y0"] = self._empty(x, P4, 256)
            K.conv(Act(tmp, N, H4, W4), self._w(ctx, "decoder.last_conv_boundary.0.weight", "low_ohwi"), 3, 1, D["y0"])
            del tmp
        p05 = DROPOUT["aspp.dropout"]
        virtual = hasattr(K, "mc_seg_head") and 256 % (self.C_FEAT // 4) == 0 and _MC_VIRTUAL
        if virtual:
            lo_rows = self._empty(x, P4, 48)
            K.bn_apply(lo, lo_rows, None)
            xf = None
        else:
            xf = self._empty(x, reps * P4, 308)
            for r in range(reps):
                K.bn_apply(lo, xf[r * P4:(r + 1) * P4, 256:304], None)
        for ps in range(passes):
            mk = None if masks is None else masks[ps]
            ctx.arena = _Arena(x, STAT_SLOTS * 2 * (256 + 256 + 305) * (2 if self.tn else 1))
            feature = self._empty(x, reps * P16, 256)
            for r in range(reps):
                m = torch.empty((P16, 256), dtype=torch.uint8, device=x.device)
                if mk is not None:
                    m.copy_(_rows(mk["aspp.dropout"][r * N:(r + 1) * N].to(x.device)))
                else:
                    K.dropout_mask(m, p05, self.seed, self.rng_offset)
                    self.rng_offset += 1
                K.bn_apply(Act(fa.x, N, H16, W16, fa.scale, fa.shift, ACT_RELU, m, 1.0 / (1.0 - p05)),
                           feature[r * P16:(r + 1) * P16], None)
            st305 = self._stats(ctx, 305, True)
            fused_up = 256 % (feature.shape[1] // 4) == 0
            if virtual:
                K.upsample_stats(feature, N2, H16, W16, H4, W4, st305)
            else:
                K.upsample_fwd(feature, N2, H16, W16, xf[:, 0:256], H4, W4, **({"stats": st305} if fused_up else {}))
            yb1 = self._empty(x, reps * P4, 256)
            st = self._stats(ctx, 256, True)
            self._conv0(ctx, feature, xf, N2, H16, W16, H4, W4, yb1, st, y0=D["y0"])
            m, ms = self._mask(x, "decoder.last_conv_boundary.3", reps * P4, 256, N2, H4, W4, True, mk)
            b1 = self._bn_act(ctx, "decoder.last_conv_boundary.1", yb1, N2, H4, W4, st, reps * P4, True, ACT_RELU, m, ms)
            yb2 = self._empty(x, reps * P4, 256)
            st = self._stats(ctx, 256, True)
            K.conv(b1, self._w(ctx, "decoder.last_conv_boundary.4.weight", "ohwi"), 3, 1, yb2, stats=st)
            m, ms = self._mask(x, "decoder.last_conv_boundary.7", reps * P4, 256, N2, H4, W4, True, mk)
            b2 = self._bn_act(ctx, "decoder.last_conv_boundary.5", yb2, N2, H4, W4, st, reps * P4, True, ACT_RELU, m, ms)
            bnd = self._buf(x, reps * P4, 1) if virtual else xf[:, 304:305]
            K.conv(b2, self._w(ctx, "decoder.last_conv_boundary.8.weight", "ohwi"), 1, 1, bnd,
                   bias=params["decoder.last_conv_boundary.8.bias"])
            st = st305
            m, ms = self._mask(x, "decoder.last_conv.2", reps * P4, 305, N2, H4, W4, True, mk)
            x1b = self._buf(x, reps * P4, 2)
            if virtual:
                split = self._split(ctx)
                for r in range(reps):
                    K.colstats_window(lo_rows, st[r] if split else st, 256)
                K.colstats_window(bnd, st, 304, **({"N": N2} if self.tn else {}))
                coef = self._coef(ctx, x, 305, True)
                self._bn(ctx, "decoder.last_conv.0", st, reps * P4, True, coef[0], coef[1], coef[2], coef[3], False, N2)
                K.mc_seg_head(feature, N2, H16, W16, lo_rows, bnd, H4, W4, coef[0], coef[1], ACT_RELU, m, ms,
                              self._w(ctx, "decoder.last_conv.3.weight", "ohwi"), params["decoder.last_conv.3.bias"], x1b)
            else:
                if fused_up:
                    K.colstats_window(xf[:, 256:305], st, 256, **({"N": N2} if self.tn else {}))
                else:
                    K.colstats(xf[:, :305], st, **({"N": N2} if self.tn else {}))
                sa = self._bn_act(ctx, "decoder.last_conv.0", xf[:, :305], N2, H4, W4, st, reps * P4, True, ACT_RELU, m, ms)
                K.conv(sa, self._w(ctx, "decoder.last_conv.3.weight", "ohwi"), 1, 1, x1b, bias=params["decoder.last_conv.3.bias"])
            K.head_upsample_fwd(x1b, N2, H4, W4, out[ps * N2:(ps + 1) * N2])
            self._check_arena(ctx)
            ctx.arena = None
            if ctx.nbt:
                torch._foreach_add_(ctx.nbt, 1)
                ctx.nbt = []
        stoch = set(self._STOCHASTIC_BN)
        det = [(prefix, rec) for prefix, rec in ctx.bnlog if prefix not in stoch]
        for prefix, rec in det:
            if repeated_tn:
                for dom in ("source", "target"):
                    K.bn_running_replay(rec.mean, rec.invstd, rec.count, passes, BN_MOMENTUM, BN_EPS,
                                        params[prefix + ".running_mean_" + dom], params[prefix + ".running_var_" + dom])
            else:
                K.bn_running_replay(rec.mean, rec.invstd, rec.count * reps, passes, BN_MOMENTUM, BN_EPS,
                                    params[prefix + ".running_mean"], params[prefix + ".running_var"])
        nbt = [params[p + ".num_batches_tracked"] for p, _ in det if (p + ".num_batches_tracked") in params]
        if nbt:
            torch._foreach_add_(nbt, passes)
        ctx.bnlog = ctx.bnlog[:len(ctx.bnlog) - 3 * passes]
        return out

    def _bn_backward(self, ctx, G, y: Act, dU, out=None, addend=None, keys=None, q1_total=None, lowrank=None):
        K = self.K
        lr = {} if lowrank is None else {"lowrank": lowrank}
        if y.bn is None:
            raise RuntimeError("this activation's BatchNorm kept no backward record (forward ran without gradient bookkeeping)")
        C = y.C
        if y.split:
            sums = ctx.arena.take(3, C, 2)
            cg = self._empty(y.x, 4, 2, C)
        else:
            sums = ctx.arena.take(3, C)
            cg = self._empty(y.x, 4, C)
        K.bnbwd_reduce(dU, y, sums, **lr)
        K.bnbwd_finalize(sums, y, cg[0], cg[1], cg[2], cg[3], **({} if q1_total is None else {"q1_total": q1_total}))
        out = dU if out is None else out
        K.bnbwd_apply(dU, y, cg[0], cg[1], out, addend, **lr)
        if y.split:
            dg, db = (cg[2] * y.bn.gain).sum(0), (cg[3] * y.bn.gain).sum(0)
        elif y.bn.gain is not None and y.bn.frozen:
            dg, db = cg[2] * y.bn.gain, cg[3] * y.bn.gain
        else:
            dg, db = cg[2], cg[3]
        if keys is None:
            keys = [(y.bn.key, slice(0, C))]
        for key, sl in keys:
            G[key + ".weight"] = dg[sl]
            G[key + ".bias"] = db[sl]
        return out

    def _wgrad(self, ctx, G, key, src: Act, dy, ksize, dil, stride=1):
        dw = torch.empty_like(ctx.params[key])
        self.K.conv_wgrad(src, dy, ksize, dil, dw, **({"stride": stride} if stride != 1 else {}))
        G[key] = dw

    def _dgrad(self, ctx, key, dy, N, H, W, ksize, dil, out, addend=None):
        self.K.conv(Act(dy, N, H, W), self._w(ctx, key, "dgrad"), ksize, dil, out, addend=addend)
        return out

    def _bias_grad(self, G, key, dy):
        g = torch.empty(dy.shape[1], dtype=torch.float32, device=dy.device)
        self.K.colsum(dy, g)
        G[key] = g

    def backward(self, ctx, grads):
        K = self.K
        gx1, gx2, gfeat, gxbu, gxf, gx1b, gx2b = grads
        S, x = ctx.S, ctx.x
        N, Hin, Win, H16, W16, H4, W4 = ctx.dims
        P4, P16 = N * H4 * W4, N * H16 * W16
        G: Dict[str, torch.Tensor] = {}
        ctx.arena = _Arena(x, STAT_SLOTS * 3 * (self.bn_channels + 64) * (2 if self.tn else 1))
        D = S["dec"]
        xf = D["xf"]
        d_x1b = self._buf(x, P4, 2)
        if gx1 is not None:
            K.head_upsample_bwd(gx1.contiguous(), d_x1b, N, H4, W4, False)
        else:
            d_x1b.zero_()
        if gx1b is not None:
            d_x1b.add_(_rows(gx1b))
        if gxf is not None:
            d_xf = torch.empty(P4, 308, dtype=torch.float32, device=x.device)
            d_xf[:, :305].copy_(_rows(gxf))
            d_xf[:, 305:].zero_()
        else:
            d_xf = torch.zeros(P4, 308, dtype=torch.float32, device=x.device)
        if gxbu is not None:
            d_xf[:, :304].add_(_rows(gxbu))
        if gx2b is not None:
            d_xf[:, 304:305].add_(_rows(gx2b))
        if gx2 is not None:
            K.head_upsample_bwd(gx2.contiguous(), d_xf[:, 304:305], N, H4, W4, True)
        sa = D["sa"]
        self._wgrad(ctx, G, "decoder.last_conv.3.weight", sa, d_x1b, 1, 1)
        self._bias_grad(G, "decoder.last_conv.3.bias", d_x1b)
        w_head = ctx.params["decoder.last_conv.3.weight"].reshape(2, 305).contiguous()
        self._bn_backward(ctx, G, sa, None, out=d_xf[:, :305], addend=d_xf[:, :305],
                          lowrank=(d_x1b, w_head))
        b1, b2 = D["b1"], D["b2"]
        d_x2b = d_xf[:, 304:305]
        self._wgrad(ctx, G, "decoder.last_conv_boundary.8.weight", b2, d_x2b, 1, 1)
        self._bias_grad(G, "decoder.last_conv_boundary.8.bias", d_x2b)
        dy2 = self._empty(x, P4, 256)
        w_bnd = ctx.params["decoder.last_conv_boundary.8.weight"].reshape(1, 256).contiguous()
        self._bn_backward(ctx, G, b2, None, out=dy2, lowrank=(d_x2b, w_bnd))
        self._wgrad(ctx, G, "decoder.last_conv_boundary.4.weight", b1, dy2, 3, 1)
        dU1 = self._empty(x, P4, 256)
        self._dgrad(ctx, "decoder.last_conv_boundary.4.weight", dy2, N, H4, W4, 3, 1, dU1)
        del dy2
        dy1 = self._bn_backward(ctx, G, b1, dU1)
        key0, CF = "decoder.last_conv_boundary.0.weight", self.C_FEAT
        w0 = ctx.params[key0]
        dw_low = self._empty(x, w0.shape[0], w0.shape[1] - CF, 3, 3)
        K.conv_wgrad(Act(xf[:, CF:304], N, H4, W4), dy1, 3, 1, dw_low)
        K.conv(Act(dy1, N, H4, W4), self._w(ctx, key0, "low_dgrad"), 3, 1, d_xf[:, CF:304], addend=d_xf[:, CF:304])
        dG = self._empty(x, P16, 9 * w0.shape[0])
        K.upconv_bwd(dy1, N, H4, W4, dG, H16, W16)
        dw_taps = self._empty(x, 9 * w0.shape[0], CF, 1, 1)
        K.conv_wgrad(Act(D["feature"], N, H16, W16), dG, 1, 1, dw_taps)
        dw0 = torch.empty_like(w0)
        dw0[:, :CF] = dw_taps.view(3, 3, w0.shape[0], CF).permute(2, 3, 0, 1)
        dw0[:, CF:] = dw_low
        G[key0] = dw0
        del dU1, dy1, dw_low, dw_taps
        lo, low = D["lo"], D["low"]
        dylo = self._empty(x, P4, 48)
        self._bn_backward(ctx, G, lo, d_xf[:, 256:304], out=dylo)
        self._wgrad(ctx, G, "decoder.conv1.weight", low, dylo, 1, 1)
        d_low = self._buf(x, P4, self.c_low)
        self._dgrad(ctx, "decoder.conv1.weight", dylo, N, H4, W4, 1, 1, d_low)
        d_feat = self._empty(x, P16, 256)
        K.upsample_bwd(d_xf[:, 0:256], N, H4, W4, d_feat, H16, W16)
        del d_xf
        K.conv(Act(dG, N, H16, W16), self._w(ctx, key0, "up_taps_dgrad"), 1, 1, d_feat, addend=d_feat)
        del dG
        if gfeat is not None:
            d_feat.add_(_rows(gfeat))
        A = S["aspp"]
        dy1a = self._bn_backward(ctx, G, A["fa"], d_feat)
        self._wgrad(ctx, G, "aspp.conv1.weight", A["catA"], dy1a, 1, 1)
        dUc = self._empty(x, P16, 1280)
        self._dgrad(ctx, "aspp.conv1.weight", dy1a, N, H16, W16, 1, 1, dUc)
        coef, cat = A["coef"], A["cat"]
        catA = A["catA"]
        w4, wg = slice(0, 1024), slice(1024, 1280)
        if catA.split:
            n0 = catA.split
            cnt4, cntg = (float(n0 * H16 * W16), float((N - n0) * H16 * W16)), (float(n0), float(N - n0))
            gain4 = torch.cat([r.gain for r in A["brecs"]])
            gaing = A["grec"].gain
        else:
            cnt4, cntg, gain4, gaing = A["brecs"][0].count, A["grec"].count, None, None
            if A["brecs"][0].gain is not None:
                gain4, gaing = torch.cat([r.gain for r in A["brecs"]]), A["grec"].gain
        c4 = Act(cat[:, :1024], N, H16, W16, coef[0][..., w4], coef[1][..., w4], ACT_RELU, None, 1.0,
                 BNRec("aspp", coef[2][..., w4], coef[3][..., w4], cnt4, False, gain4, frozen=A["brecs"][0].frozen), split=catA.split)
        keys = [("aspp.aspp%d.bn" % j, slice(256 * (j - 1), 256 * j)) for j in (1, 2, 3, 4)]
        dyc = self._bn_backward(ctx, G, c4, dUc[:, :1024], keys=keys)
        dUg = self._empty(x, N, 256)
        K.gap_fwd(dUc[:, 1024:1280], N, dUg, 1.0)
        yga = Act(A["yg"], N, 1, 1, coef[0][..., wg], coef[1][..., wg], ACT_RELU, None, 1.0,
                  BNRec("aspp.global_avg_pool.2", coef[2][..., wg], coef[3][..., wg], cntg, False, gaing, frozen=A["grec"].frozen),
                  split=catA.split)
        dyg = self._bn_backward(ctx, G, yga, dUg)
        self._wgrad(ctx, G, "aspp.global_avg_pool.1.weight", A["gpa"], dyg, 1, 1)
        d_gp = self._empty(x, N, self.c_high)
        self._dgrad(ctx, "aspp.global_avg_pool.1.weight", dyg, N, 1, 1, 1, 1, d_gp)
        d_a = self._empty(x, P16, self.c_high)
        K.broadcast_rows(d_gp, N, d_a, 1.0 / (H16 * W16), None)
        a17 = A["a17"]
        for j, dl in enumerate(self.dils, start=1):
            key = "aspp.aspp%d.atrous_conv.weight" % j
            sl = slice(256 * (j - 1), 256 * j)
            k = 1 if j == 1 else 3
            self._wgrad(ctx, G, key, a17, dyc[:, sl], k, dl)
            self._dgrad(ctx, key, dyc[:, sl], N, H16, W16, k, dl, d_a, addend=d_a)
        del dUc, dyc
        if self.backbone == "mobilenet":
            self._mobilenet_backward(ctx, G, d_a, d_low)
        elif self.backbone == "xception":
            self._xception_backward(ctx, G, d_a, d_low)
        else:
            self._resnet_backward(ctx, G, d_a, d_low)
        self._check_arena(ctx)
        ctx.arena = None
        return G
```

### uda_clr_amd/kernels.py

```python
from __future__ import annotations

import ctypes as C
import os
from typing import Optional

import torch

from .acts import conv_weight_shape, Act, round4

STAT_SLOTS = 16
_LIB_PATH = os.path.join(os.path.dirname(os.path.abspath(__file__)), "lib", "libuda_clr_hip.so")
_lib = None


class UdaSrc(C.Structure):
    _fields_ = [("x", C.c_void_p), ("ldx", C.c_int64), ("N", C.c_int32), ("H", C.c_int32),
                ("W", C.c_int32), ("C", C.c_int32), ("scale", C.c_void_p), ("shift", C.c_void_p),
                ("act", C.c_int32), ("_pad", C.c_int32), ("mask", C.c_void_p), ("ldm", C.c_int64),
                ("mask_scale", C.c_float), ("_pad2", C.c_float)]


class UdaConvArgs(C.Structure):
    _fields_ = [("src", UdaSrc), ("w", C.c_void_p), ("Cout", C.c_int32), ("ksize", C.c_int32),
                ("dil", C.c_int32), ("origin", C.c_int32), ("bias", C.c_void_p), ("addend", C.c_void_p),
                ("ld_add", C.c_int64), ("y", C.c_void_p), ("ldy", C.c_int64), ("stats", C.c_void_p),
                ("mfma", C.c_int32), ("stride", C.c_int32), ("x3_src", C.c_void_p), ("x3_w", C.c_void_p),
                ("workspace", C.c_void_p), ("workspace_bytes", C.c_uint64)]


class UdaWgradArgs(C.Structure):
    _fields_ = [("src", UdaSrc), ("dy", C.c_void_p), ("lddy", C.c_int64), ("Cout", C.c_int32),
                ("ksize", C.c_int32), ("dil", C.c_int32), ("origin", C.c_int32), ("dw", C.c_void_p),
                ("workspace", C.c_void_p), ("workspace_bytes", C.c_uint64), ("mfma", C.c_int32), ("stride", C.c_int32),
                ("x3_src", C.c_void_p), ("x3_dy", C.c_void_p)]


_P, _I, _L, _F, _D, _U = C.c_void_p, C.c_int, C.c_int64, C.c_float, C.c_double, C.c_uint64
SYMBOLS = {
    "uda_last_error": (C.c_char_p, []),
    "uda_version": (_I, []),
    "uda_relayout_ohwi": (_I, [_P, _I, _I, _I, _P, _P]),
    "uda_relayout_dgrad": (_I, [_P, _I, _I, _I, _P, _P]),
    "uda_relayout_dw": (_I, [_P, _I, _P, _P]),
    "uda_conv_fwd": (_I, [C.POINTER(UdaConvArgs), _P]),
    "uda_conv_uses_x3": (_I, [C.POINTER(UdaConvArgs)]),
    "uda_conv_fwd_workspace_bytes": (_U, [C.POINTER(UdaConvArgs)]),
    "uda_x3_packed_bytes": (_U, [_L, _I]),
    "uda_x3_pack": (_I, [C.POINTER(UdaSrc), _P, _P]),
    "uda_conv_wgrad_workspace_bytes": (_U, [_L, _I, _I, _I]),
    "uda_conv_wgrad": (_I, [C.POINTER(UdaWgradArgs), _P]),
    "uda_conv_wgrad_uses_x3": (_I, [C.POINTER(UdaWgradArgs)]),
    "uda_dwconv_workspace_bytes": (_U, [_L, _I]),
    "uda_dwconv_fwd": (_I, [C.POINTER(UdaSrc), _P, _I, _I, _I, _P, _L, _P, _P]),
    "uda_dwconv_dgrad": (_I, [_P, _L, _P, _I, _I, _I, _I, _I, _I, _P, _L, _P]),
    "uda_dwconv_wgrad": (_I, [C.POINTER(UdaSrc), _P, _L, _I, _I, _I, _P, _P, _U, _P]),
    "uda_dwconv_cb_fwd": (_I, [C.POINTER(UdaSrc), _P, _I, _I, _I, _P, _L, _P, _P]),
    "uda_dwconv_cb_dgrad": (_I, [_P, _L, _P, _I, _I, _I, _I, _I, _I, _P, _L, _P]),
    "uda_dwconv_cb_wgrad": (_I, [C.POINTER(UdaSrc), _P, _L, _I, _I, _I, _P, _P, _U, _P]),
    "uda_stem_workspace_bytes": (_U, [_L]),
    "uda_stem_fwd": (_I, [_P, _I, _I, _I, _P, _P, _L, _P, _P]),
    "uda_stem_wgrad": (_I, [_P, _I, _I, _I, _P, _L, _P, _P, _U, _P]),
    "uda_stem7_workspace_bytes": (_U, [_L]),
    "uda_stem7_fwd": (_I, [_P, _I, _I, _I, _P, _P, _L, _P, _P]),
    "uda_stem7_wgrad": (_I, [_P, _I, _I, _I, _P, _L, _P, _P, _U, _P]),
    "uda_maxpool_fwd": (_I, [C.POINTER(UdaSrc), _P, _L, _P, _L, _P]),
    "uda_maxpool_bwd": (_I, [_P, _L, _P, _L, _I, _I, _I, _I, _P, _L, _P]),
    "uda_rows_stride": (_I, [_P, _L, _I, _I, _I, _I, _I, _I, _P, _L, _P]),
    "uda_bn_add_relu": (_I, [C.POINTER(UdaSrc), C.POINTER(UdaSrc), _P, _L, _P]),
    "uda_relu_gate": (_I, [_P, _L, _P, _L, _L, _I, _P, _L, _P]),
    "uda_relayout_s2d": (_I, [_P, _I, _I, _I, _P, _P]),
    "uda_s2d_fwd": (_I, [_P, _L, _I, _I, _I, _I, _I, _I, _I, _F, _P, _L, _I, _I, _P]),
    "uda_s2d_bwd": (_I, [_P, _P, _L, _I, _I, _F, _I, _I, _I, _I, _I, _I, _P, _L, _I, _P]),
    "uda_s2d_bwd_gate": (_I, [_P, _L, _I, _I, _P, _L, _F, _I, _I, _I, _I, _I, _I, _P, _L, _P]),
    "uda_x3_pack_s2d_fwd": (_I, [_P, _L, _I, _I, _I, _I, _I, _I, _F, _I, _I, _P, _P]),
    "uda_x3_pack_s2d_bwd": (_I, [_P, _L, _I, _I, _P, _L, _F, _I, _I, _I, _I, _I, _I, _P, _P]),
    "uda_bn_finalize": (_I, [_P, _I, _D, _P, _P, _P, _P, _F, _F, _P, _P, _P, _P, _P]),
    "uda_bn_running_replay": (_I, [_P, _P, _I, _D, _I, _F, _F, _P, _P, _P]),
    "uda_bn_eval_coeffs": (_I, [_P, _P, _P, _P, _I, _F, _P, _P, _P]),
    "uda_tn_gain": (_I, [_P, _P, _I, _D, _D, _F, _P, _P, _P, _P, _P, _P]),
    "uda_tn_eval_coeffs": (_I, [_P, _P, _P, _P, _P, _P, _I, _F, _P, _P, _P]),
    "uda_bn_apply": (_I, [C.POINTER(UdaSrc), _P, _L, _P, _L, _P]),
    "uda_colstats": (_I, [_P, _L, _L, _I, _I, _P, _P]),
    "uda_colstats_window": (_I, [_P, _L, _L, _I, _I, _P, _I, _P]),
    "uda_upsample_fwd_stats": (_I, [_P, _L, _I, _I, _I, _I, _P, _L, _I, _I, _P, _I, _P]),
    "uda_mc_seg_head": (_I, [_P, _L, _I, _I, _I, _I, _P, _L, _I, _L, _P, _L, _I, _I, _P, _P, _I, _P, _L, _F, _P, _L, _P, _P, _L, _P]),
    "uda_bnbwd_reduce": (_I, [_P, _L, C.POINTER(UdaSrc), _P, _P, _P, _P]),
    "uda_bnbwd_finalize": (_I, [_P, _I, _D, _I, _I, _P, _P, _P, _P, _P, _P, _P, _P, _P]),
    "uda_bnbwd_apply": (_I, [_P, _L, C.POINTER(UdaSrc), _P, _P, _P, _P, _P, _L, _P, _L, _P]),
    "uda_bnbwd_reduce_lowrank": (_I, [_P, _L, _I, _P, C.POINTER(UdaSrc), _P, _P, _P, _P]),
    "uda_bnbwd_apply_lowrank": (_I, [_P, _L, _I, _P, C.POINTER(UdaSrc), _P, _P, _P, _P, _P, _L, _P, _L, _P]),
    "uda_upsample_fwd": (_I, [_P, _L, _I, _I, _I, _I, _P, _L, _I, _I, _P]),
    "uda_upsample_bwd": (_I, [_P, _L, _I, _I, _I, _I, _P, _L, _I, _I, _P]),
    "uda_head_upsample_fwd": (_I, [_P, _L, _I, _I, _I, _I, _P, _I, _I, _P]),
    "uda_head_upsample_bwd": (_I, [_P, _I, _I, _I, _I, _P, _L, _I, _I, _I, _P]),
    "uda_gap_fwd": (_I, [_P, _L, _I, _I, _I, _F, _P, _L, _P]),
    "uda_broadcast_rows": (_I, [_P, _L, _I, _I, _I, _F, _P, _L, _P, _L, _P]),
    "uda_dropout_mask": (_I, [_P, _L, _L, _I, _F, _U, _U, _P]),
    "uda_seg_loss_fwd": (_I, [_P, _P, _L, _P, _P, _L, _P, _P, _P]),
    "uda_seg_loss_bwd": (_I, [_P, _P, _L, _P, _P, _L, _P, _P, _P, _P]),
    "uda_seg_counts": (_I, [_P, _P, _I, _I, _L, _F, _P, _P]),
    "uda_mc_stats": (_I, [_P, _I, _L, _P, _P, _P]),
    "uda_proto_weights": (_I, [_I, _I, _I, _I, _I, _I, _P, _P, _L, _P, _P, _P, _P, _P, _P]),
    "uda_proto_workspace_bytes": (_U, [_L, _I]),
    "uda_proto_reduce": (_I, [_P, _L, _L, _I, _P, _P, _P, _U, _P]),
    "uda_proto_finalize": (_I, [_P, _I, _P, _P]),
    "uda_proto_bwd": (_I, [_P, _L, _L, _I, _P, _P, _P, _P, _P, _L, _I, _P, _P]),
    "uda_feat_dot4": (_I, [_P, _L, _L, _I, _P, _P, _P]),
    "uda_feat_rank4": (_I, [_P, _P, _L, _I, _P, _L, _I, _P]),
    "uda_adam_step": (_I, [_P, _P, _P, _P, _L, _D, _D, _D, _D, _L, _P]),
    "uda_proto_align_fwd": (_I, [_P, _P, _P, _P, _F, _F, _I, _P, _P, _P, _P]),
    "uda_proto_align_bwd": (_I, [_P, _P, _P, _F, _F, _I, _P, _P, _P]),
    "uda_adv_loss_fwd": (_I, [_P, _I, _P, _I, _F, _F, _P, _P]),
    "uda_adv_loss_bwd": (_I, [_P, _I, _P, _I, _F, _F, _P, _P, _P, _P]),
    "uda_adv_s2d_fwd": (_I, [_P, _I, _I, _I, _I, _I, _P, _L, _I, _I, _P]),
    "uda_adv_s2d_bwd": (_I, [_P, _L, _I, _I, _P, _I, _I, _I, _I, _I, _P, _P]),
    "uda_upconv_fused_stats": (_I, [_I, _I, _I, _I, _I, _I]),
    "uda_upconv_fwd": (_I, [_P, _L, _I, _I, _I, _I, _I, _P, _L, _L, _P, _L, _I, _I, _P, _P]),
    "uda_upconv_bwd": (_I, [_P, _L, _I, _I, _I, _I, _I, _P, _L, _I, _I, _P]),
    "uda_postprocess_workspace_bytes": (_U, [_I, _I, _I]),
    "uda_postprocess": (_I, [_P, _I, _I, _I, _F, _F, _I, _P, _P, _P, _U, _P]),
    "uda_normalize_tf_workspace_bytes": (_U, [_I, _I, _I]),
    "uda_normalize_tf": (_I, [_P, _P, _I, _I, _I, C.POINTER(C.c_double), _I, _P, _P, _P, _P, _U, _P]),
    "uda_field_smooth": (_I, [_P, _I, _I, _I, _P, _I, _D, _P, _P, _P]),
    "uda_elastic_warp": (_I, [_P, _P, _P, _P, _P, _I, _I, _I, _P, _P, _P]),
    "uda_photometric_u8": (_I, [_P, _I, _I, _I, _P, _P, _P, _I, _P, _P, _P]),
}


def load_library(path: Optional[str] = None):
    global _lib
    if _lib is not None and path is None:
        return _lib
    path = path or _LIB_PATH
    if not os.path.exists(path):
        raise RuntimeError("libuda_clr_hip.so not found at %s - build it with "
                           "`python -c 'import __graft_entry__ as g; g.build()'` "
                           "(there is no CPU fallback)" % path)
    lib = C.CDLL(path)
    for name, (res, args) in SYMBOLS.items():
        fn = getattr(lib, name)
        fn.restype, fn.argtypes = res, args
    _lib = lib
    return lib


class UdaError(RuntimeError):
    pass


def _family(family: str) -> str:
    if family not in ("", "cb"):
        raise ValueError("depthwise kernel family %r" % (family,))
    return family + "_" if family else ""


def _ptr(t: Optional[torch.Tensor]):
    return None if t is None else t.data_ptr()


def _mat(t: torch.Tensor, name="tensor"):
    if t.dim() != 2 or t.stride(1) != 1:
        raise ValueError("%s must be a [P, C] row-major view" % name)
    return t.data_ptr(), t.stride(0)


class HipKernels:
    name = "hip"

    MFMA_F32, MFMA_BF16X3 = 0, 1

    def __init__(self, mfma=None):
        self.lib = load_library()
        mode = (mfma or os.environ.get("UDA_CLR_MFMA", "bf16x3")).lower()
        if mode not in ("f32", "bf16x3"):
            raise ValueError("UDA_CLR_MFMA must be 'f32' or 'bf16x3', got %r" % mode)
        self.mfma = self.MFMA_BF16X3 if mode == "bf16x3" else self.MFMA_F32

    @staticmethod
    def _stream():
        return torch.cuda.current_stream().cuda_stream

    def _ck(self, rc):
        if rc != 0:
            raise UdaError(self.lib.uda_last_error().decode())

    @staticmethod
    def _dev(t):
        if not t.is_cuda:
            raise UdaError("HIP kernels need device tensors (got %s); there is no CPU fallback" % t.device)
        if t.dtype not in (torch.float32, torch.float64, torch.uint8):
            raise UdaError("unsupported dtype %s" % t.dtype)

    def _src(self, a: Act) -> UdaSrc:
        a.check()
        self._dev(a.x)
        s = UdaSrc()
        s.x, s.ldx = a.x.data_ptr(), a.x.stride(0)
        s.N, s.H, s.W, s.C = a.N, a.H, a.W, a.C
        s.scale, s.shift = _ptr(a.scale), _ptr(a.shift)
        if a.scale is not None:
            assert a.scale.is_contiguous() and a.shift.is_contiguous() and a.scale.numel() == a.C
        s.act = a.act
        if a.mask is not None:
            s.mask, s.ldm = a.mask.data_ptr(), a.mask.stride(0)
        else:
            s.mask, s.ldm = None, 0
        s.mask_scale = a.mask_scale
        return s

    @staticmethod
    def _ws(like, nbytes):
        return torch.empty(max(int(nbytes), 16), dtype=torch.uint8, device=like.device)

    def relayout_ohwi(self, w):
        O, I, k, _ = w.shape
        out = torch.empty(conv_weight_shape(O, k, I), dtype=torch.float32, device=w.device)
        self._ck(self.lib.uda_relayout_ohwi(w.contiguous().data_ptr(), O, I, k, out.data_ptr(), self._stream()))
        return out

    def relayout_dgrad(self, w):
        O, I, k, _ = w.shape
        out = torch.empty(conv_weight_shape(I, k, O), dtype=torch.float32, device=w.device)
        self._ck(self.lib.uda_relayout_dgrad(w.contiguous().data_ptr(), O, I, k, out.data_ptr(), self._stream()))
        return out

    def relayout_dw(self, w):
        Cc = w.shape[0]
        out = torch.empty(9, Cc, dtype=torch.float32, device=w.device)
        self._ck(self.lib.uda_relayout_dw(w.contiguous().data_ptr(), Cc, out.data_ptr(), self._stream()))
        return out

    ELEM_LIMIT = 1 << 29

    def _image_groups(self, N, rows_per_image, widest_ld, x3_channels=0):
        lim_rows = self.ELEM_LIMIT // max(int(widest_ld), 1) - 256
        if x3_channels:
            lim_rows = min(lim_rows, (self.ELEM_LIMIT // 4) // (((x3_channels + 15) // 16) * 6) - 256)
        if N * rows_per_image <= lim_rows:
            return None
        g = lim_rows // rows_per_image
        if g < 1:
            raise UdaError("one image (%d pixels x %d floats per row) exceeds the 32-bit offsets of the conv kernels" % (rows_per_image, widest_ld))
        return [(n0, min(N, n0 + g)) for n0 in range(0, N, g)]

    @staticmethod
    def _act_rows(a: Act, n0, n1):
        ppi = a.P // a.N
        r = slice(n0 * ppi, n1 * ppi)
        return Act(a.x[r], n1 - n0, a.H, a.W, a.scale, a.shift, a.act, None if a.mask is None else a.mask[r], a.mask_scale, a.bn, a.meta)

    def conv(self, src: Act, w, ksize, dil, out, bias=None, addend=None, stats=None, origin=0, stride=1):
        groups = self._image_groups(src.N, src.P // src.N, max(src.x.stride(0), out.stride(0), 0 if addend is None else addend.stride(0),
                                                               0 if src.mask is None else src.mask.stride(0) // 4),
                                    src.C if self.mfma != self.MFMA_F32 else 0)
        Po = src.N * ((src.H - 1) // stride + 1) * ((src.W - 1) // stride + 1)
        if groups is not None:
            ppo = Po // src.N
            for n0, n1 in groups:
                r = slice(n0 * ppo, n1 * ppo)
                self.conv(self._act_rows(src, n0, n1), w, ksize, dil, out[r], bias, None if addend is None else addend[r], stats, origin, stride)
            return
        a = UdaConvArgs()
        a.origin = origin
        a.src = self._src(src)
        Cout = out.shape[1]
        assert w.is_contiguous() and tuple(w.shape) == conv_weight_shape(Cout, ksize, src.C), \
            "weight layout %s does not match conv %dx%d %d->%d" % (tuple(w.shape), ksize, ksize, src.C, Cout)
        assert out.shape[0] == Po and stride in (1, 2)
        a.w, a.Cout, a.ksize, a.dil, a.stride = w.data_ptr(), Cout, ksize, dil, stride
        a.bias = _ptr(bias)
        if bias is not None:
            assert bias.is_contiguous() and bias.numel() == Cout
        if addend is not None:
            assert addend.shape == out.shape
            a.addend, a.ld_add = _mat(addend, "addend")
        else:
            a.addend, a.ld_add = None, 0
        a.y, a.ldy = _mat(out, "out")
        if stats is not None:
            assert stats.dtype == torch.float64 and stats.is_contiguous() and tuple(stats.shape) == (STAT_SLOTS, 2, Cout)
        a.stats = _ptr(stats)
        a.mfma = self.mfma
        if self.mfma != self.MFMA_F32 and self.lib.uda_conv_uses_x3(C.byref(a)):
            xs = self._packed(src, a.src, out.device)
            xw = getattr(w, "_x3", None)
            if xw is None:
                xw = self.x3_pack_rows(w)
                w._x3 = xw
            a.x3_src, a.x3_w = xs.data_ptr(), xw.data_ptr()
            nws = int(self.lib.uda_conv_fwd_workspace_bytes(C.byref(a)))
            if nws:
                ws = self._ws(out, nws)
                a.workspace, a.workspace_bytes = ws.data_ptr(), nws
            return self._conv_x3(a)
        self._ck(self.lib.uda_conv_fwd(C.byref(a), self._stream()))

    def _conv_x3(self, a):
        self._ck(self.lib.uda_conv_fwd(C.byref(a), self._stream()))

    def x3_pack(self, usrc: UdaSrc, rows, K, device):
        out = torch.empty(int(self.lib.uda_x3_packed_bytes(rows, K)), dtype=torch.uint8, device=device)
        self._ck(self.lib.uda_x3_pack(C.byref(usrc), out.data_ptr(), self._stream()))
        return out

    def _packed(self, src: Act, usrc: UdaSrc, device):
        xs = getattr(src, "_x3", None)
        raw = not src.lazy
        if xs is None and raw:
            xs = getattr(src.x, "_x3", None)
        if xs is not None and xs.numel() != int(self.lib.uda_x3_packed_bytes(src.P, src.C)):
            raise RuntimeError("bf16x3 packed operand of %d bytes attached to a [%d, %d] matrix (expected %d): stale attachment"
                               % (xs.numel(), src.P, src.C, int(self.lib.uda_x3_packed_bytes(src.P, src.C))))
        if xs is None:
            xs = self.x3_pack(usrc, src.P, src.C, device)
            if raw:
                try:
                    src.x._x3 = xs
                except AttributeError:
                    pass
        src._x3 = xs
        return xs

    def x3_pack_rows(self, w):
        rows, klen = w.shape[0], w.numel() // w.shape[0]
        s = UdaSrc()
        s.x, s.ldx, s.N, s.H, s.W, s.C = w.data_ptr(), klen, 1, 1, rows, klen
        s.scale = s.shift = s.mask = None
        s.act, s.ldm, s.mask_scale = 0, 0, 1.0
        return self.x3_pack(s, rows, klen, w.device)

    def conv_wgrad(self, src: Act, dy, ksize, dil, dw, origin=0, stride=1):
        groups = self._image_groups(src.N, src.P // src.N, max(src.x.stride(0), dy.stride(0), 0 if src.mask is None else src.mask.stride(0) // 4))
        Ho, Wo = (src.H - 1) // stride + 1, (src.W - 1) // stride + 1
        Po = src.N * Ho * Wo
        if groups is not None:
            ppo = Po // src.N
            tmp = torch.empty_like(dw)
            for i, (n0, n1) in enumerate(groups):
                self.conv_wgrad(self._act_rows(src, n0, n1), dy[n0 * ppo:n1 * ppo], ksize, dil, dw if i == 0 else tmp, origin, stride)
                if i:
                    dw.add_(tmp)
            return
        a = UdaWgradArgs()
        a.origin = origin
        a.src = self._src(src)
        Cout = dy.shape[1]
        assert dy.shape[0] == Po and stride in (1, 2) and dw.is_contiguous() and tuple(dw.shape) == (Cout, src.C, ksize, ksize)
        a.dy, a.lddy = _mat(dy, "dy")
        a.Cout, a.ksize, a.dil, a.stride = Cout, ksize, dil, stride
        a.dw = dw.data_ptr()
        ws = self._ws(dy, self.lib.uda_conv_wgrad_workspace_bytes(Po, Cout, src.C, ksize))
        a.workspace, a.workspace_bytes = ws.data_ptr(), ws.numel()
        a.mfma = self.mfma
        if self.mfma != self.MFMA_F32 and self.lib.uda_conv_wgrad_uses_x3(C.byref(a)):
            xs = self._packed(src, a.src, dy.device)
            dsrc = Act(dy, src.N, Ho, Wo)
            xd = self._packed(dsrc, self._src(dsrc), dy.device)
            a.x3_src, a.x3_dy = xs.data_ptr(), xd.data_ptr()
        self._ck(self.lib.uda_conv_wgrad(C.byref(a), self._stream()))

    def dwconv_fwd(self, src: Act, w9c, stride, dil, border_mode, out, stats=None, family=""):
        s = self._src(src)
        Ho, Wo = (src.H - 1) // stride + 1, (src.W - 1) // stride + 1
        assert out.shape == (src.N * Ho * Wo, src.C) and w9c.is_contiguous() and tuple(w9c.shape) == (9, src.C)
        y, ldy = _mat(out, "out")
        if stats is not None:
            assert stats.dtype == torch.float64 and stats.is_contiguous() and tuple(stats.shape) == (STAT_SLOTS, 2, src.C)
        self._ck(getattr(self.lib, "uda_dwconv_%sfwd" % _family(family))(C.byref(s), w9c.data_ptr(), stride, dil, border_mode, y, ldy,
                                                                        _ptr(stats), self._stream()))

    def dwconv_dgrad(self, dy, w9c, stride, dil, N, H, W, out, family=""):
        Cc = dy.shape[1]
        Ho, Wo = (H - 1) // stride + 1, (W - 1) // stride + 1
        assert dy.shape[0] == N * Ho * Wo and out.shape == (N * H * W, Cc)
        g, ldg = _mat(dy, "dy")
        o, ldo = _mat(out, "out")
        self._ck(getattr(self.lib, "uda_dwconv_%sdgrad" % _family(family))(g, ldg, w9c.data_ptr(), Cc, stride, dil, N, H, W, o, ldo,
                                                                          self._stream()))

    def dwconv_wgrad(self, src: Act, dy, stride, dil, border_mode, dw, family=""):
        s = self._src(src)
        Ho, Wo = (src.H - 1) // stride + 1, (src.W - 1) // stride + 1
        assert dy.shape == (src.N * Ho * Wo, src.C) and dw.is_contiguous() and dw.numel() == 9 * src.C
        g, ldg = _mat(dy, "dy")
        ws = self._ws(dy, self.lib.uda_dwconv_workspace_bytes(dy.shape[0], src.C))
        self._ck(getattr(self.lib, "uda_dwconv_%swgrad" % _family(family))(C.byref(s), g, ldg, stride, dil, border_mode, dw.data_ptr(),
                                                                          ws.data_ptr(), ws.numel(), self._stream()))

    def stem_fwd(self, x, w, out, stats=None):
        self._dev(x)
        N, c3, H, W = x.shape
        assert c3 == 3 and x.is_contiguous() and w.is_contiguous() and tuple(w.shape) == (32, 3, 3, 3)
        Po = N * ((H - 1) // 2 + 1) * ((W - 1) // 2 + 1)
        assert out.shape == (Po, 32)
        y, ldy = _mat(out, "out")
        if stats is not None:
            assert stats.dtype == torch.float64 and stats.is_contiguous() and tuple(stats.shape) == (STAT_SLOTS, 2, 32)
        self._ck(self.lib.uda_stem_fwd(x.data_ptr(), N, H, W, w.data_ptr(), y, ldy, _ptr(stats), self._stream()))

    def stem_wgrad(self, x, dy, dw):
        N, _, H, W = x.shape
        Po = N * ((H - 1) // 2 + 1) * ((W - 1) // 2 + 1)
        assert dy.shape == (Po, 32) and dw.is_contiguous() and dw.numel() == 864
        g, ldg = _mat(dy, "dy")
        ws = self._ws(dy, self.lib.uda_stem_workspace_bytes(Po))
        self._ck(self.lib.uda_stem_wgrad(x.data_ptr(), N, H, W, g, ldg, dw.data_ptr(), ws.data_ptr(), ws.numel(),
                                         self._stream()))

    def stem7_fwd(self, x, w, out, stats=None):
        self._dev(x)
        N, c3, H, W = x.shape
        assert c3 == 3 and x.is_contiguous() and w.is_contiguous() and tuple(w.shape) == (64, 3, 7, 7)
        Po = N * ((H - 1) // 2 + 1) * ((W - 1) // 2 + 1)
        assert out.shape == (Po, 64)
        y, ldy = _mat(out, "out")
        if stats is not None:
            assert stats.dtype == torch.float64 and stats.is_contiguous() and tuple(stats.shape) == (STAT_SLOTS, 2, 64)
        self._ck(self.lib.uda_stem7_fwd(x.data_ptr(), N, H, W, w.data_ptr(), y, ldy, _ptr(stats), self._stream()))

    def stem7_wgrad(self, x, dy, dw):
        N, _, H, W = x.shape
        Po = N * ((H - 1) // 2 + 1) * ((W - 1) // 2 + 1)
        assert dy.shape == (Po, 64) and dw.is_contiguous() and dw.numel() == 64 * 147
        g, ldg = _mat(dy, "dy")
        ws = self._ws(dy, self.lib.uda_stem7_workspace_bytes(Po))
        self._ck(self.lib.uda_stem7_wgrad(x.data_ptr(), N, H, W, g, ldg, dw.data_ptr(), ws.data_ptr(), ws.numel(),
                                          self._stream()))

    def maxpool_fwd(self, src: Act, out, idx):
        s = self._src(src)
        Po = src.N * ((src.H - 1) // 2 + 1) * ((src.W - 1) // 2 + 1)
        assert out.shape == (Po, src.C) and idx.shape == (Po, src.C) and idx.dtype == torch.uint8
        o, ldo = _mat(out, "out")
        i, ldi = _mat(idx, "idx")
        self._ck(self.lib.uda_maxpool_fwd(C.byref(s), o, ldo, i, ldi, self._stream()))

    def maxpool_bwd(self, dz, idx, N, H, W, out):
        Cc = dz.shape[1]
        assert out.shape == (N * H * W, Cc) and idx.shape == dz.shape
        g, ldg = _mat(dz, "dz")
        i, ldi = _mat(idx, "idx")
        o, ldo = _mat(out, "out")
        self._ck(self.lib.uda_maxpool_bwd(g, ldg, i, ldi, N, H, W, Cc, o, ldo, self._stream()))

    def rows_stride(self, src, N, H, W, stride, out, scatter=False):
        Cc = src.shape[1]
        Po = N * ((H - 1) // stride + 1) * ((W - 1) // stride + 1)
        big, small = (out, src) if scatter else (src, out)
        assert big.shape == (N * H * W, Cc) and small.shape == (Po, Cc)
        a, lda = _mat(src, "src")
        o, ldo = _mat(out, "out")
        self._ck(self.lib.uda_rows_stride(a, lda, N, H, W, Cc, stride, int(scatter), o, ldo, self._stream()))

    def bn_add_relu(self, a: Act, b: Act, out):
        sa, sb = self._src(a), self._src(b)
        assert out.shape == a.x.shape == b.x.shape
        o, ldo = _mat(out, "out")
        self._ck(self.lib.uda_bn_add_relu(C.byref(sa), C.byref(sb), o, ldo, self._stream()))

    def relu_gate(self, dz, z, out):
        assert dz.shape == z.shape == out.shape
        g, ldg = _mat(dz, "dz")
        v, ldv = _mat(z, "z")
        o, ldo = _mat(out, "out")
        self._ck(self.lib.uda_relu_gate(g, ldg, v, ldv, dz.shape[0], dz.shape[1], o, ldo, self._stream()))

    def relayout_s2d(self, w, dgrad):
        O, Cc = w.shape[0], w.shape[1]
        assert tuple(w.shape[2:]) == (4, 4)
        out = torch.empty(conv_weight_shape(4 * Cc, 2, O) if dgrad else conv_weight_shape(O, 2, 4 * Cc), dtype=torch.float32,
                          device=w.device)
        self._ck(self.lib.uda_relayout_s2d(w.detach().contiguous().data_ptr(), O, Cc, int(bool(dgrad)), out.data_ptr(), self._stream()))
        return out

    def s2d_fwd(self, src, nchw, N, Hs, Ws, Cc, vh, vw, slope, z):
        self._dev(src)
        Hz, Wz = (vh + 5) // 2, (vw + 5) // 2
        assert z.shape == (N * Hz * Wz, 4 * Cc)
        if nchw:
            assert src.is_contiguous() and tuple(src.shape) == (N, Cc, Hs, Ws)
            sp, lds_ = src.data_ptr(), 0
        else:
            assert src.shape == (N * Hs * Ws, Cc)
            sp, lds_ = _mat(src, "src")
        zp, ldz = _mat(z, "z")
        self._ck(self.lib.uda_s2d_fwd(sp, lds_, int(nchw), N, Hs, Ws, Cc, vh, vw, float(slope), zp, ldz, Hz, Wz, self._stream()))

    def conv_route_x3(self, N, H, W, Cin, Cout, ksize):
        if self.mfma != self.MFMA_BF16X3 or self._image_groups(N, H * W, max(round4(Cin), round4(Cout)), Cin) is not None:
            return False
        a = UdaConvArgs()
        a.src.N, a.src.H, a.src.W, a.src.C = N, H, W, Cin
        a.src.scale = a.src.shift = a.src.mask = None
        a.src.act, a.Cout, a.ksize, a.dil, a.mfma = 0, Cout, ksize, 1, self.mfma
        a.stats = None
        return bool(self.lib.uda_conv_uses_x3(C.byref(a)))

    def wgrad_route_x3(self, N, H, W, Cin, Cout, ksize):
        if self.mfma != self.MFMA_BF16X3 or self._image_groups(N, H * W, max(round4(Cin), round4(Cout))) is not None:
            return False
        a = UdaWgradArgs()
        a.src.N, a.src.H, a.src.W, a.src.C = N, H, W, Cin
        a.src.scale = a.src.shift = a.src.mask = None
        a.src.act, a.Cout, a.ksize, a.dil, a.mfma = 0, Cout, ksize, 1, self.mfma
        return bool(self.lib.uda_conv_wgrad_uses_x3(C.byref(a)))

    def _packed_only(self, rows, Cc, device):
        xs = torch.empty(int(self.lib.uda_x3_packed_bytes(rows, Cc)), dtype=torch.uint8, device=device)
        m = xs[:rows * Cc * 4].view(torch.float32).view(rows, Cc)
        m._x3 = xs
        return m, xs

    def s2d_pack_fwd(self, src, N, Hs, Ws, Cc, vh, vw, slope):
        self._dev(src)
        Hz, Wz = (vh + 5) // 2, (vw + 5) // 2
        assert src.shape == (N * Hs * Ws, Cc) and Cc % 8 == 0
        sp, lds_ = _mat(src, "src")
        z, xs = self._packed_only(N * Hz * Wz, 4 * Cc, src.device)
        self._ck(self.lib.uda_x3_pack_s2d_fwd(sp, lds_, N, Hs, Ws, Cc, vh, vw, float(slope), Hz, Wz, xs.data_ptr(), self._stream()))
        return z

    def s2d_pack_bwd(self, dz, gate, slope, N, Hs, Ws, Cc, vh, vw):
        Hz, Wz = (vh + 5) // 2, (vw + 5) // 2
        assert dz.shape == (N * Hz * Wz, 4 * Cc) and Cc % 8 == 0 and (gate is None or gate.shape == (N * Hs * Ws, Cc))
        gp, ldz = _mat(dz, "dz")
        tp, ldt = (None, 0) if gate is None else _mat(gate, "gate")
        d, xs = self._packed_only(N * Hs * Ws, Cc, dz.device)
        self._ck(self.lib.uda_x3_pack_s2d_bwd(gp, ldz, Hz, Wz, tp, ldt, float(slope), N, Hs, Ws, Cc, vh, vw, xs.data_ptr(), self._stream()))
        return d

    def s2d_bwd(self, dz, z_sign, slope, N, Hs, Ws, Cc, vh, vw, dst, nchw, gate=None):
        Hz, Wz = (vh + 5) // 2, (vw + 5) // 2
        assert dz.shape == (N * Hz * Wz, 4 * Cc) and (z_sign is None or (z_sign.shape == dz.shape and z_sign.stride(0) == dz.stride(0)))
        gp, ldz = _mat(dz, "dz")
        if gate is not None:
            assert z_sign is None and not nchw and gate.shape == (N * Hs * Ws, Cc) and dst.shape == (N * Hs * Ws, Cc)
            tp, ldt = _mat(gate, "gate")
            dp, ldd = _mat(dst, "dst")
            self._ck(self.lib.uda_s2d_bwd_gate(gp, ldz, Hz, Wz, tp, ldt, float(slope), N, Hs, Ws, Cc, vh, vw, dp, ldd, self._stream()))
            return
        if nchw:
            assert dst.is_contiguous() and tuple(dst.shape) == (N, Cc, Hs, Ws)
            dp, ldd = dst.data_ptr(), 0
        else:
            assert dst.shape == (N * Hs * Ws, Cc)
            dp, ldd = _mat(dst, "dst")
        self._ck(self.lib.uda_s2d_bwd(gp, _ptr(z_sign), ldz, Hz, Wz, float(slope), N, Hs, Ws, Cc, vh, vw, dp, ldd, int(nchw),
                                      self._stream()))

    def adv_s2d_fwd(self, logits, pre_op, z):
        self._dev(logits)
        N, Cc, H, W = logits.shape
        Hz, Wz = (H + 5) // 2, (W + 5) // 2
        assert logits.is_contiguous() and logits.dtype == torch.float32 and z.shape == (N * Hz * Wz, 4 * Cc)
        zp, ldz = _mat(z, "z")
        self._ck(self.lib.uda_adv_s2d_fwd(logits.data_ptr(), N, Cc, H, W, int(pre_op), zp, ldz, Hz, Wz, self._stream()))

    def adv_s2d_bwd(self, dz, logits, pre_op, d_logits):
        N, Cc, H, W = logits.shape
        Hz, Wz = (H + 5) // 2, (W + 5) // 2
        assert dz.shape == (N * Hz * Wz, 4 * Cc) and logits.is_contiguous() and d_logits.is_contiguous()
        assert tuple(d_logits.shape) == tuple(logits.shape)
        gp, ldz = _mat(dz, "dz")
        self._ck(self.lib.uda_adv_s2d_bwd(gp, ldz, Hz, Wz, logits.data_ptr(), N, Cc, H, W, int(pre_op), d_logits.data_ptr(),
                                          self._stream()))

    def bn_finalize(self, stats, count, gamma, beta, rmean, rvar, momentum, eps, scale, shift, mean, invstd):
        Cc = gamma.numel()
        for t in (gamma, beta, rmean, rvar, scale, shift, mean, invstd):
            assert t.is_contiguous() and t.numel() == Cc
        assert stats.dtype == torch.float64 and stats.is_contiguous() and tuple(stats.shape) == (STAT_SLOTS, 2, Cc)
        self._ck(self.lib.uda_bn_finalize(stats.data_ptr(), Cc, float(count), gamma.data_ptr(), beta.data_ptr(),
                                          rmean.data_ptr(), rvar.data_ptr(), momentum, eps, scale.data_ptr(),
                                          shift.data_ptr(), mean.data_ptr(), invstd.data_ptr(), self._stream()))

    def bn_running_replay(self, mean, invstd, count, k, momentum, eps, rmean, rvar):
        Cc = mean.numel()
        for t in (mean, invstd, rmean, rvar):
            assert t.is_contiguous() and t.numel() == Cc
        self._ck(self.lib.uda_bn_running_replay(mean.data_ptr(), invstd.data_ptr(), Cc, float(count), int(k), momentum, eps,
                                                rmean.data_ptr(), rvar.data_ptr(), self._stream()))

    def bn_eval_coeffs(self, gamma, beta, rmean, rvar, eps, scale, shift):
        Cc = gamma.numel()
        for t in (gamma, beta, rmean, rvar, scale, shift):
            assert t.is_contiguous() and t.numel() == Cc
        self._ck(self.lib.uda_bn_eval_coeffs(gamma.data_ptr(), beta.data_ptr(), rmean.data_ptr(), rvar.data_ptr(), Cc,
                                             eps, scale.data_ptr(), shift.data_ptr(), self._stream()))

    def tn_gain(self, stats0, stats1, count0, count1, eps, scale0, shift0, scale1, shift1, gain):
        Cc = gain.numel()
        for t in (scale0, shift0, scale1, shift1, gain):
            assert t.is_contiguous() and t.numel() == Cc
        for st in (stats0, stats1):
            assert st.dtype == torch.float64 and st.is_contiguous() and tuple(st.shape) == (STAT_SLOTS, 2, Cc)
        self._ck(self.lib.uda_tn_gain(stats0.data_ptr(), stats1.data_ptr(), Cc, float(count0), float(count1), eps,
                                      scale0.data_ptr(), shift0.data_ptr(), scale1.data_ptr(), shift1.data_ptr(),
                                      gain.data_ptr(), self._stream()))

    def tn_eval_coeffs(self, gamma, beta, rmean_s, rvar_s, rmean_t, rvar_t, eps, scale, shift):
        Cc = gamma.numel()
        for t in (gamma, beta, rmean_s, rvar_s, rmean_t, rvar_t, scale, shift):
            assert t.is_contiguous() and t.numel() == Cc
        self._ck(self.lib.uda_tn_eval_coeffs(gamma.data_ptr(), beta.data_ptr(), rmean_s.data_ptr(), rvar_s.data_ptr(),
                                             rmean_t.data_ptr(), rvar_t.data_ptr(), Cc, eps, scale.data_ptr(),
                                             shift.data_ptr(), self._stream()))

    def bn_apply(self, src: Act, out, residual=None):
        s = self._src(src)
        assert out.shape == src.x.shape and src.C % 4 == 0
        o, ldo = _mat(out, "out")
        r, ldr = (None, 0) if residual is None else _mat(residual, "residual")
        self._ck(self.lib.uda_bn_apply(C.byref(s), r, ldr, o, ldo, self._stream()))

    def colstats(self, x, stats):
        self._dev(x)
        p, ld = _mat(x, "x")
        slots, nq, Cc = stats.shape
        assert slots == STAT_SLOTS and Cc == x.shape[1] and stats.dtype == torch.float64 and stats.is_contiguous()
        self._ck(self.lib.uda_colstats(p, ld, x.shape[0], Cc, nq, stats.data_ptr(), self._stream()))

    def colstats_window(self, x, stats, c_off):
        self._dev(x)
        p, ld = _mat(x, "x")
        slots, nq, Cs = stats.shape
        Cc = x.shape[1]
        assert slots == STAT_SLOTS and c_off >= 0 and c_off + Cc <= Cs and stats.dtype == torch.float64 and stats.is_contiguous()
        self._ck(self.lib.uda_colstats_window(p, ld, x.shape[0], Cc, nq, stats.data_ptr() + 8 * c_off, Cs, self._stream()))

    def colsum(self, x, out):
        st = torch.zeros(STAT_SLOTS, 1, x.shape[1], dtype=torch.float64, device=x.device)
        self.colstats(x, st)
        out.copy_(st.sum(0)[0])

    @staticmethod
    def _lowrank(lowrank, y):
        d, w = lowrank
        k = d.shape[1]
        assert k in (1, 2) and d.shape[0] == y.P and tuple(w.shape) == (k, y.C) and w.is_contiguous() and d.stride(1) == 1
        assert d.dtype == w.dtype == torch.float32
        return d.data_ptr(), d.stride(0), k, w.data_ptr()

    def bnbwd_reduce(self, dU, y: Act, sums, lowrank=None):
        s = self._src(y)
        assert sums.dtype == torch.float64 and tuple(sums.shape) == (STAT_SLOTS, 3, y.C) and sums.is_contiguous()
        if lowrank is not None:
            dp, ldd, k, wp = self._lowrank(lowrank, y)
            self._ck(self.lib.uda_bnbwd_reduce_lowrank(dp, ldd, k, wp, C.byref(s), y.bn.mean.data_ptr(), y.bn.invstd.data_ptr(),
                                                       sums.data_ptr(), self._stream()))
            return
        assert dU.shape == y.x.shape
        d, ldu = _mat(dU, "dU")
        self._ck(self.lib.uda_bnbwd_reduce(d, ldu, C.byref(s), y.bn.mean.data_ptr(), y.bn.invstd.data_ptr(),
                                           sums.data_ptr(), self._stream()))

    def bnbwd_finalize(self, sums, y: Act, c1, c2, dgamma, dbeta, q1_total=None):
        if q1_total is not None:
            assert q1_total.is_contiguous() and q1_total.numel() == y.C and q1_total.dtype == torch.float32
        self._ck(self.lib.uda_bnbwd_finalize(sums.data_ptr(), y.C, float(y.bn.count), int(y.bn.q1_border), y.act,
                                             y.shift.data_ptr(), y.bn.mean.data_ptr(), y.bn.invstd.data_ptr(), _ptr(q1_total),
                                             c1.data_ptr(), c2.data_ptr(), dgamma.data_ptr(), dbeta.data_ptr(),
                                             self._stream()))

    def bnbwd_apply(self, dU, y: Act, c1, c2, out, addend=None, lowrank=None):
        s = self._src(y)
        assert y.x.shape == out.shape
        o, ldo = _mat(out, "out")
        ad, lda = (None, 0) if addend is None else _mat(addend, "addend")
        if lowrank is not None:
            dp, ldd, k, wp = self._lowrank(lowrank, y)
            self._ck(self.lib.uda_bnbwd_apply_lowrank(dp, ldd, k, wp, C.byref(s), y.bn.mean.data_ptr(), y.bn.invstd.data_ptr(),
                                                      c1.data_ptr(), c2.data_ptr(), ad, lda, o, ldo, self._stream()))
            return
        assert dU.shape == y.x.shape
        d, ldu = _mat(dU, "dU")
        self._ck(self.lib.uda_bnbwd_apply(d, ldu, C.byref(s), y.bn.mean.data_ptr(), y.bn.invstd.data_ptr(),
                                          c1.data_ptr(), c2.data_ptr(), ad, lda, o, ldo, self._stream()))

    def upsample_fwd(self, x, N, h, w, out, H, W, stats=None):
        self._dev(x)
        p, ld = _mat(x, "x")
        o, ldo = _mat(out, "out")
        assert x.shape[0] == N * h * w and out.shape == (N * H * W, x.shape[1])
        if stats is not None:
            assert stats.dtype == torch.float64 and stats.is_contiguous() and stats.shape[:2] == (STAT_SLOTS, 2) and stats.shape[2] >= x.shape[1]
            self._ck(self.lib.uda_upsample_fwd_stats(p, ld, N, h, w, x.shape[1], o, ldo, H, W, stats.data_ptr(), stats.shape[2], self._stream()))
            return
        self._ck(self.lib.uda_upsample_fwd(p, ld, N, h, w, x.shape[1], o, ldo, H, W, self._stream()))

    def upsample_stats(self, x, N, h, w, H, W, stats):
        self._dev(x)
        p, ld = _mat(x, "x")
        assert x.shape[0] == N * h * w and stats.dtype == torch.float64 and stats.is_contiguous()
        assert stats.shape[:2] == (STAT_SLOTS, 2) and stats.shape[2] >= x.shape[1]
        self._ck(self.lib.uda_upsample_fwd_stats(p, ld, N, h, w, x.shape[1], None, 0, H, W, stats.data_ptr(), stats.shape[2], self._stream()))

    def mc_seg_head(self, feature, N, h, w, low, bnd, H, W, scale, shift, act, mask, mask_scale, wgt, bias, out):
        self._dev(feature)
        fp, ldf = _mat(feature, "feature")
        lp, ldl = _mat(low, "low")
        P = N * H * W
        Cf, Cl = feature.shape[1], low.shape[1]
        Cc = Cf + Cl + 1
        assert feature.shape[0] == N * h * w and P % low.shape[0] == 0 and bnd.shape == (P, 1) and out.shape == (P, 2)
        assert bnd.stride(1) == 1 and out.stride(1) == 1 and wgt.is_contiguous() and wgt.shape[0] == 2 and wgt.numel() // 2 >= Cc
        assert scale.is_contiguous() and shift.is_contiguous() and scale.numel() == Cc and bias.numel() == 2
        mp, ldm = (None, 0)
        if mask is not None:
            assert mask.dtype == torch.uint8 and mask.shape == (P, Cc) and mask.stride(1) == 1
            mp, ldm = mask.data_ptr(), mask.stride(0)
        self._ck(self.lib.uda_mc_seg_head(fp, ldf, N, h, w, Cf, lp, ldl, Cl, low.shape[0], bnd.data_ptr(), bnd.stride(0), H, W,
                                          scale.data_ptr(), shift.data_ptr(), int(act), mp, ldm, float(mask_scale), wgt.data_ptr(),
                                          wgt.numel() // 2, bias.data_ptr(), out.data_ptr(), out.stride(0), self._stream()))

    def upsample_bwd(self, dout, N, H, W, dx, h, w):
        p, ld = _mat(dout, "dout")
        o, ldo = _mat(dx, "dx")
        assert dout.shape[0] == N * H * W and dx.shape == (N * h * w, dout.shape[1])
        self._ck(self.lib.uda_upsample_bwd(p, ld, N, H, W, dout.shape[1], o, ldo, h, w, self._stream()))

    def upconv_fwd(self, g, N, h, w, out, H, W, addend=None, dil=1, stats=None):
        self._dev(g)
        Cc = out.shape[1]
        assert g.shape == (N * h * w, 9 * Cc) and out.shape[0] == N * H * W
        gp, ldg = _mat(g, "g")
        o, ldo = _mat(out, "out")
        ad, lda, rows = (None, 0, 1) if addend is None else (_mat(addend, "addend") + (addend.shape[0],))
        if addend is not None:
            assert addend.shape[1] == Cc and (N * H * W) % addend.shape[0] == 0
        fused = stats is not None and bool(self.lib.uda_upconv_fused_stats(h, w, H, W, Cc, dil))
        if stats is not None:
            assert stats.dtype == torch.float64 and stats.is_contiguous() and tuple(stats.shape) == (STAT_SLOTS, 2, Cc)
        self._ck(self.lib.uda_upconv_fwd(gp, ldg, N, h, w, Cc, dil, ad, lda, rows, o, ldo, H, W, _ptr(stats) if fused else None,
                                         self._stream()))
# ... 268 lines not shown
```

Measured before the change: 366.4.

## Batch wgrad reductions, weight relayouts and BN replays into multi-descriptor launches

Adds grouped kernels that process many weight-gradient slab reductions, weight relayouts and BN running-stat replays in one launch each. A block-range table with binary search picks the descriptor for each block. During backward, wgrad reductions are deferred and queued up to a byte budget, then flushed together. This cuts per-layer kernel launch and Python/ctypes overhead, but keeps slab workspaces alive longer and may lose some overlap or locality between each wgrad and its reduction.

```diff
diff --git a/include/uda_clr_hip.h b/include/uda_clr_hip.h
--- a/include/uda_clr_hip.h
+++ b/include/uda_clr_hip.h
@@ -33,6 +33,17 @@
 int uda_relayout_ohwi(const float* w, int O, int I, int k, float* out, void* stream);
 int uda_relayout_dgrad(const float* w, int O, int I, int k, float* out, void* stream);
 int uda_relayout_dw(const float* w, int C, float* out, void* stream);
+#define UDA_RELAYOUT_MULTI_MAX 64
+#define UDA_RELAYOUT_OHWI 0
+#define UDA_RELAYOUT_DGRAD 1
+#define UDA_RELAYOUT_DW 2
+#define UDA_RELAYOUT_DW_FLIP 3
+typedef struct uda_relayout_desc {
+    const float* w;
+    float* out;
+    int32_t O, I, k, kind;
+} uda_relayout_desc_t;
+int uda_relayout_multi(const uda_relayout_desc_t* d, int n, void* stream);
 
 #define UDA_MFMA_F32 0
 #define UDA_MFMA_BF16X3 1
@@ -77,6 +88,16 @@
 uint64_t uda_conv_wgrad_workspace_bytes(int64_t P, int Cout, int Cin, int ksize);
 int uda_conv_wgrad_uses_x3(const uda_wgrad_args_t* a);
 int uda_conv_wgrad(const uda_wgrad_args_t* a, void* stream);
+#define UDA_WGRAD_MULTI_MAX 64
+typedef struct uda_wgrad_reduce_desc {
+    const float* slab;
+    float* dw;
+    int32_t S, Cout, Cin;
+    int32_t T;
+    int32_t Kc;
+} uda_wgrad_reduce_desc_t;
+int uda_conv_wgrad_slabs(const uda_wgrad_args_t* a, int32_t* S_used, void* stream);
+int uda_wgrad_reduce_multi(const uda_wgrad_reduce_desc_t* d, int n, void* stream);
 
 uint64_t uda_dwconv_workspace_bytes(int64_t Pout, int C);
 int uda_dwconv_fwd(const uda_src_t* src, const float* w9c, int stride, int dil, int border_mode,
@@ -132,6 +153,16 @@
                     float* shift, float* mean, float* invstd, void* stream);
 int uda_bn_running_replay(const float* mean, const float* invstd, int C, double count, int k, float momentum,
                           float eps, float* running_mean, float* running_var, void* stream);
+#define UDA_BN_REPLAY_MULTI_MAX 64
+typedef struct uda_bn_replay_desc {
+    const float* mean;
+    const float* invstd;
+    float* running_mean;
+    float* running_var;
+    double count;
+    int32_t C;
+} uda_bn_replay_desc_t;
+int uda_bn_running_replay_multi(const uda_bn_replay_desc_t* d, int n, int k, float momentum, float eps, void* stream);
 int uda_bn_eval_coeffs(const float* gamma, const float* beta, const float* running_mean,
                        const float* running_var, int C, float eps, float* scale, float* shift,
                        void* stream);
diff --git a/uda_clr_amd/csrc/bn_elementwise.hip b/uda_clr_amd/csrc/bn_elementwise.hip
--- a/uda_clr_amd/csrc/bn_elementwise.hip
+++ b/uda_clr_amd/csrc/bn_elementwise.hip
@@ -65,11 +65,9 @@
     return 0;
 }
 
-__global__ void bn_running_replay_kernel(const float* __restrict__ mean, const float* __restrict__ invstd, int C,
-                                         double count, int k, float momentum, float eps, float* __restrict__ rmean,
-                                         float* __restrict__ rvar) {
-    const int c = blockIdx.x * blockDim.x + threadIdx.x;
-    if (c >= C) return;
+__device__ __forceinline__ void bn_running_replay_channel(const float* __restrict__ mean, const float* __restrict__ invstd, int c,
+                                                          double count, int k, float momentum, float eps,
+                                                          float* __restrict__ rmean, float* __restrict__ rvar) {
     const double is = (double)invstd[c];
     double var = 1.0 / (is * is) - (double)eps;
     if (var < 0.0) var = 0.0;
@@ -77,6 +75,50 @@
     const double a = pow(1.0 - (double)momentum, (double)k);
     rmean[c] = (float)(a * (double)rmean[c] + (1.0 - a) * (double)mean[c]);
     rvar[c] = (float)(a * (double)rvar[c] + (1.0 - a) * unbiased);
+}
+
+__global__ void bn_running_replay_kernel(const float* __restrict__ mean, const float* __restrict__ invstd, int C,
+                                         double count, int k, float momentum, float eps, float* __restrict__ rmean,
+                                         float* __restrict__ rvar) {
+    const int c = blockIdx.x * blockDim.x + threadIdx.x;
+    if (c >= C) return;
+    bn_running_replay_channel(mean, invstd, c, count, k, momentum, eps, rmean, rvar);
+}
+
+struct ReplayMultiArgs {
+    uda_bn_replay_desc_t d[UDA_BN_REPLAY_MULTI_MAX];
+    int blk_end[UDA_BN_REPLAY_MULTI_MAX];
+};
+__global__ __launch_bounds__(256) void bn_running_replay_multi_kernel(const ReplayMultiArgs a, int k, float momentum, float eps) {
+    const int b = blockIdx.x;
+    int i = 0;
+#pragma unroll
+    for (int step = UDA_BN_REPLAY_MULTI_MAX / 2; step >= 1; step >>= 1)
+        if (b >= a.blk_end[i + step - 1]) i += step;
+    const uda_bn_replay_desc_t& d = a.d[i];
+    const int c = (b - (i ? a.blk_end[i - 1] : 0)) * 256 + threadIdx.x;
+    if (c < d.C) bn_running_replay_channel(d.mean, d.invstd, c, d.count, k, momentum, eps, d.running_mean, d.running_var);
+}
+
+extern "C" int uda_bn_running_replay_multi(const uda_bn_replay_desc_t* d, int n, int k, float momentum, float eps, void* stream) {
+    UDA_REQUIRE(d && n > 0 && k >= 1, "uda_bn_running_replay_multi: bad args");
+    for (int i0 = 0; i0 < n; i0 += UDA_BN_REPLAY_MULTI_MAX) {
+        ReplayMultiArgs a;
+        const int m = n - i0 < UDA_BN_REPLAY_MULTI_MAX ? n - i0 : UDA_BN_REPLAY_MULTI_MAX;
+        int blocks = 0;
+        for (int i = 0; i < m; ++i) {
+            const uda_bn_replay_desc_t& t = d[i0 + i];
+            UDA_REQUIRE(t.mean && t.invstd && t.running_mean && t.running_var && t.C > 0 && t.count > 0,
+                        "uda_bn_running_replay_multi: bad descriptor %d", i0 + i);
+            blocks += uda_cdiv(t.C, 256);
+            a.d[i] = t;
+            a.blk_end[i] = blocks;
+        }
+        for (int i = m; i < UDA_BN_REPLAY_MULTI_MAX; ++i) { a.d[i] = a.d[0]; a.blk_end[i] = blocks; }
+        hipLaunchKernelGGL(bn_running_replay_multi_kernel, dim3(blocks), dim3(256), 0, (hipStream_t)stream, a, k, momentum, eps);
+        UDA_LAUNCH_CHECK("bn_running_replay_multi");
+    }
+    return 0;
 }
 
 extern "C" int uda_bn_running_replay(const float* mean, const float* invstd, int C, double count, int k, float momentum,
diff --git a/uda_clr_amd/csrc/igemm_conv.hip b/uda_clr_amd/csrc/igemm_conv.hip
--- a/uda_clr_amd/csrc/igemm_conv.hip
+++ b/uda_clr_amd/csrc/igemm_conv.hip
@@ -329,7 +329,7 @@
     return 0;
 }
 
-static inline int uda_k_row(int C, int ksize) {
+__host__ __device__ static inline int uda_k_row(int C, int ksize) {
     const int Kc = ((C + 3) / 4) * 4;
     if (ksize == 1 || Kc < IG_BK) return ksize * ksize * Kc;
     return ((Kc + IG_BK - 1) / IG_BK) * ksize * ksize * IG_BK;
@@ -917,46 +917,93 @@
 }
 
 template <int Q>
+__device__ __forceinline__ void wgrad_reduce_block(const float* __restrict__ slab, int S, int Cout, int Cin, int T, int Kc,
+                                                   float* __restrict__ dw, int64_t e0, float* red) {
+    constexpr int NO = 256 / Q;
+    const int64_t total = (int64_t)Cout * T * Cin;
+    const int64_t stride = (int64_t)Cout * T * Kc;
+    const int ol = threadIdx.x % NO, q = threadIdx.x / NO;
+    const int64_t e = e0 + ol;
+    float s = 0.f;
+    int64_t dst = 0;
+    if (e < total) {
+        const int ci = (int)(e % Cin);
+        const int t = (int)((e / Cin) % T);
+        const int co = (int)(e / ((int64_t)Cin * T));
+        dst = ((int64_t)co * Cin + ci) * T + t;
+        const float* src = slab + ((int64_t)co * T + t) * Kc + ci;
+        int k = q;
+        float s0 = 0.f, s1 = 0.f, s2 = 0.f, s3 = 0.f;
+        for (; k + 3 * Q < S; k += 4 * Q) {
+            s0 += src[(int64_t)k * stride];
+            s1 += src[(int64_t)(k + Q) * stride];
+            s2 += src[(int64_t)(k + 2 * Q) * stride];
+            s3 += src[(int64_t)(k + 3 * Q) * stride];
+        }
+        for (; k < S; k += Q) s0 += src[(int64_t)k * stride];
+        s = (s0 + s1) + (s2 + s3);
+    }
+    red[q * (NO + 1) + ol] = s;
+    __syncthreads();
+    if (q == 0 && e < total) {
+        float acc[8];
+#pragma unroll
+        for (int j = 0; j < 8; ++j) acc[j] = 0.f;
+#pragma unroll
+        for (int j = 0; j < Q; ++j) acc[j & 7] += red[j * (NO + 1) + ol];
+        dw[dst] = ((acc[0] + acc[1]) + (acc[2] + acc[3])) + ((acc[4] + acc[5]) + (acc[6] + acc[7]));
+    }
+    __syncthreads();
+}
+
+template <int Q>
 __global__ __launch_bounds__(256) void wgrad_reduce_kernel(const float* __restrict__ slab, int S, int Cout, int Cin, int T,
                                                            int Kc, float* __restrict__ dw) {
     constexpr int NO = 256 / Q;
-    __shared__ float red[Q][NO + 1];
+    __shared__ float red[Q * (NO + 1)];
     const int64_t total = (int64_t)Cout * T * Cin;
-    const int64_t stride = (int64_t)Cout * T * Kc;
-    const int ol = threadIdx.x % NO, q = threadIdx.x / NO;
-    for (int64_t e0 = (int64_t)blockIdx.x * NO; e0 < total; e0 += (int64_t)gridDim.x * NO) {
-        const int64_t e = e0 + ol;
-        float s = 0.f;
-        int64_t dst = 0;
-        if (e < total) {
-            const int ci = (int)(e % Cin);
-            const int t = (int)((e / Cin) % T);
-            const int co = (int)(e / ((int64_t)Cin * T));
-            dst = ((int64_t)co * Cin + ci) * T + t;
-            const float* src = slab + ((int64_t)co * T + t) * Kc + ci;
-            int k = q;
-            float s0 = 0.f, s1 = 0.f, s2 = 0.f, s3 = 0.f;
-            for (; k + 3 * Q < S; k += 4 * Q) {
-                s0 += src[(int64_t)k * stride];
-                s1 += src[(int64_t)(k + Q) * stride];
-                s2 += src[(int64_t)(k + 2 * Q) * stride];
-                s3 += src[(int64_t)(k + 3 * Q) * stride];
-            }
-            for (; k < S; k += Q) s0 += src[(int64_t)k * stride];
-            s = (s0 + s1) + (s2 + s3);
-        }
-        red[q][ol] = s;
-        __syncthreads();
-        if (q == 0 && e < total) {
-            float acc[8];
-#pragma unroll
-            for (int j = 0; j < 8; ++j) acc[j] = 0.f;
-#pragma unroll
-            for (int j = 0; j < Q; ++j) acc[j & 7] += red[j][ol];
-            dw[dst] = ((acc[0] + acc[1]) + (acc[2] + acc[3])) + ((acc[4] + acc[5]) + (acc[6] + acc[7]));
-        }
-        __syncthreads();
-    }
+    for (int64_t e0 = (int64_t)blockIdx.x * NO; e0 < total; e0 += (int64_t)gridDim.x * NO)
+        wgrad_reduce_block<Q>(slab, S, Cout, Cin, T, Kc, dw, e0, red);
+}
+
+struct WgradMultiArgs {
+    uda_wgrad_reduce_desc_t d[UDA_WGRAD_MULTI_MAX];
+    int blk_end[UDA_WGRAD_MULTI_MAX];
+    int n;
+};
+__global__ __launch_bounds__(256) void wgrad_reduce_multi_kernel(const WgradMultiArgs a) {
+    __shared__ float red[64 * (4 + 1)];
+    const int b = blockIdx.x;
+    int i = 0;
+#pragma unroll
+    for (int step = UDA_WGRAD_MULTI_MAX / 2; step >= 1; step >>= 1)
+        if (b >= a.blk_end[i + step - 1]) i += step;
+    const int lb = b - (i ? a.blk_end[i - 1] : 0);
+    const uda_wgrad_reduce_desc_t& d = a.d[i];
+    if (d.S > 256) wgrad_reduce_block<64>(d.slab, d.S, d.Cout, d.Cin, d.T, d.Kc, d.dw, (int64_t)lb * 4, red);
+    else wgrad_reduce_block<8>(d.slab, d.S, d.Cout, d.Cin, d.T, d.Kc, d.dw, (int64_t)lb * 32, red);
+}
+
+extern "C" int uda_wgrad_reduce_multi(const uda_wgrad_reduce_desc_t* d, int n, void* stream) {
+    UDA_REQUIRE(d && n > 0, "uda_wgrad_reduce_multi: bad args");
+    for (int i0 = 0; i0 < n; i0 += UDA_WGRAD_MULTI_MAX) {
+        WgradMultiArgs a;
+        a.n = n - i0 < UDA_WGRAD_MULTI_MAX ? n - i0 : UDA_WGRAD_MULTI_MAX;
+        int64_t blocks = 0;
+        for (int i = 0; i < a.n; ++i) {
+            const uda_wgrad_reduce_desc_t& t = d[i0 + i];
+            UDA_REQUIRE(t.slab && t.dw && t.S >= 1 && t.Cout > 0 && t.Cin > 0 && t.T >= 1 && t.Kc >= t.Cin,
+                        "uda_wgrad_reduce_multi: bad descriptor %d", i0 + i);
+            blocks += uda_cdiv((int64_t)t.Cout * t.T * t.Cin, t.S > 256 ? 4 : 32);
+            UDA_REQUIRE(blocks < (1ll << 30), "uda_wgrad_reduce_multi: too many outputs in one call");
+            a.d[i] = t;
+            a.blk_end[i] = (int)blocks;
+        }
+        for (int i = a.n; i < UDA_WGRAD_MULTI_MAX; ++i) { a.d[i] = a.d[0]; a.blk_end[i] = (int)blocks; }
+        hipLaunchKernelGGL(wgrad_reduce_multi_kernel, dim3((unsigned)blocks), dim3(256), 0, (hipStream_t)stream, a);
+        UDA_LAUNCH_CHECK("wgrad_reduce_multi");
+    }
+    return 0;
 }
 
 struct WgradPlan {
@@ -1002,7 +1049,7 @@
     return wide && wgrad_x3_eligible(a->src.C, a->Cout, a->ksize, P) ? 1 : 0;
 }
 
-extern "C" int uda_conv_wgrad(const uda_wgrad_args_t* a, void* stream) {
+static int conv_wgrad_impl(const uda_wgrad_args_t* a, int32_t* slabs_S, void* stream) {
     hipStream_t st = (hipStream_t)stream;
     UDA_REQUIRE(a != nullptr, "uda_conv_wgrad: null args");
     if (int e = check_src(a->src, "uda_conv_wgrad")) return e;
@@ -1044,6 +1091,11 @@
     else if (p.bm == 128) hipLaunchKernelGGL((igemm_wgrad_kernel<1, 1, 4, 1>), grid, dim3(256), 0, st, k);
     else hipLaunchKernelGGL((igemm_wgrad_kernel<1, 1, 1, 4>), grid, dim3(256), 0, st, k);
     UDA_LAUNCH_CHECK("igemm_wgrad");
+    if (slabs_S) {
+        *slabs_S = S_used;
+        return 0;
+    }
+    UDA_REQUIRE(a->dw != nullptr, "uda_conv_wgrad: null dw");
     const int T = a->ksize * a->ksize;
     const int64_t total = (int64_t)a->Cout * T * a->src.C;
     if (S_used > 256)
@@ -1054,6 +1106,13 @@
                            k.slab, S_used, a->Cout, a->src.C, T, k.Kc, a->dw);
     UDA_LAUNCH_CHECK("wgrad_reduce");
     return 0;
+}
+
+extern "C" int uda_conv_wgrad(const uda_wgrad_args_t* a, void* stream) { return conv_wgrad_impl(a, nullptr, stream); }
+
+extern "C" int uda_conv_wgrad_slabs(const uda_wgrad_args_t* a, int32_t* S_used, void* stream) {
+    UDA_REQUIRE(S_used != nullptr, "uda_conv_wgrad_slabs: null S_used");
+    return conv_wgrad_impl(a, S_used, stream);
 }
 
 __device__ __forceinline__ void uda_k_decode(int64_t e, int T, int Kr, int Kc, int& c, int& t, int& row) {
@@ -1071,27 +1130,60 @@
         c = (chunk / T) * IG_BK + (k % IG_BK);
     }
 }
+__device__ __forceinline__ void relayout_ohwi_elem(const float* __restrict__ w, int I, int T, int Kr, float* __restrict__ out, int64_t e) {
+    const int Kc = ((I + 3) / 4) * 4;
+    int ci, t, o;
+    uda_k_decode(e, T, Kr, Kc, ci, t, o);
+    out[e] = ci < I ? w[((int64_t)o * I + ci) * T + t] : 0.f;
+}
+__device__ __forceinline__ void relayout_dgrad_elem(const float* __restrict__ w, int O, int I, int T, int Kr, float* __restrict__ out, int64_t e) {
+    const int Kc = ((O + 3) / 4) * 4;
+    int o, t, ci;
+    uda_k_decode(e, T, Kr, Kc, o, t, ci);
+    out[e] = o < O ? w[((int64_t)o * I + ci) * T + (T - 1 - t)] : 0.f;
+}
+__device__ __forceinline__ void relayout_dw_elem(const float* __restrict__ w, int C, bool flip, float* __restrict__ out, int e) {
+    const int t = e / C;
+    out[e] = w[(e % C) * 9 + (flip ? 8 - t : t)];
+}
+
 __global__ void relayout_ohwi_kernel(const float* __restrict__ w, int O, int I, int T, int Kr, float* __restrict__ out) {
     const int64_t total = (int64_t)O * Kr;
-    const int Kc = ((I + 3) / 4) * 4;
-    for (int64_t e = (int64_t)blockIdx.x * blockDim.x + threadIdx.x; e < total; e += (int64_t)gridDim.x * blockDim.x) {
-        int ci, t, o;
-        uda_k_decode(e, T, Kr, Kc, ci, t, o);
-        out[e] = ci < I ? w[((int64_t)o * I + ci) * T + t] : 0.f;
-    }
+    for (int64_t e = (int64_t)blockIdx.x * blockDim.x + threadIdx.x; e < total; e += (int64_t)gridDim.x * blockDim.x)
+        relayout_ohwi_elem(w, I, T, Kr, out, e);
 }
 __global__ void relayout_dgrad_kernel(const float* __restrict__ w, int O, int I, int T, int Kr, float* __restrict__ out) {
     const int64_t total = (int64_t)I * Kr;
-    const int Kc = ((O + 3) / 4) * 4;
-    for (int64_t e = (int64_t)blockIdx.x * blockDim.x + threadIdx.x; e < total; e += (int64_t)gridDim.x * blockDim.x) {
-        int o, t, ci;
-        uda_k_decode(e, T, Kr, Kc, o, t, ci);
-        out[e] = o < O ? w[((int64_t)o * I + ci) * T + (T - 1 - t)] : 0.f;
-    }
+    for (int64_t e = (int64_t)blockIdx.x * blockDim.x + threadIdx.x; e < total; e += (int64_t)gridDim.x * blockDim.x)
+        relayout_dgrad_elem(w, O, I, T, Kr, out, e);
 }
 __global__ void relayout_dw_kernel(const float* __restrict__ w, int C, float* __restrict__ out) {
     const int e = blockIdx.x * blockDim.x + threadIdx.x;
-    if (e < 9 * C) out[e] = w[(e % C) * 9 + e / C];
+    if (e < 9 * C) relayout_dw_elem(w, C, false, out, e);
+}
+
+struct RelayoutMultiArgs {
+    uda_relayout_desc_t d[UDA_RELAYOUT_MULTI_MAX];
+    int blk_end[UDA_RELAYOUT_MULTI_MAX];
+};
+__global__ __launch_bounds__(256) void relayout_multi_kernel(const RelayoutMultiArgs a) {
+    const int b = blockIdx.x;
+    int i = 0;
+#pragma unroll
+    for (int step = UDA_RELAYOUT_MULTI_MAX / 2; step >= 1; step >>= 1)
+        if (b >= a.blk_end[i + step - 1]) i += step;
+    const uda_relayout_desc_t& d = a.d[i];
+    const int64_t e = (int64_t)(b - (i ? a.blk_end[i - 1] : 0)) * 256 + threadIdx.x;
+    const int T = d.k * d.k;
+    if (d.kind == UDA_RELAYOUT_OHWI) {
+        const int Kr = uda_k_row(d.I, d.k);
+        if (e < (int64_t)d.O * Kr) relayout_ohwi_elem(d.w, d.I, T, Kr, d.out, e);
+    } else if (d.kind == UDA_RELAYOUT_DGRAD) {
+        const int Kr = uda_k_row(d.O, d.k);
+        if (e < (int64_t)d.I * Kr) relayout_dgrad_elem(d.w, d.O, d.I, T, Kr, d.out, e);
+    } else {
+        if (e < 9 * (int64_t)d.O) relayout_dw_elem(d.w, d.O, d.kind == UDA_RELAYOUT_DW_FLIP, d.out, (int)e);
+    }
 }
 
 static inline int grid_for(int64_t total) {
@@ -1121,3 +1213,29 @@
     UDA_LAUNCH_CHECK("relayout_dw");
     return 0;
 }
+
+extern "C" int uda_relayout_multi(const uda_relayout_desc_t* d, int n, void* stream) {
+    UDA_REQUIRE(d && n > 0, "uda_relayout_multi: bad args");
+    for (int i0 = 0; i0 < n; i0 += UDA_RELAYOUT_MULTI_MAX) {
+        RelayoutMultiArgs a;
+        const int m = n - i0 < UDA_RELAYOUT_MULTI_MAX ? n - i0 : UDA_RELAYOUT_MULTI_MAX;
+        int64_t blocks = 0;
+        for (int i = 0; i < m; ++i) {
+            const uda_relayout_desc_t& t = d[i0 + i];
+            UDA_REQUIRE(t.w && t.out && t.O > 0 && t.kind >= UDA_RELAYOUT_OHWI && t.kind <= UDA_RELAYOUT_DW_FLIP,
+                        "uda_relayout_multi: bad descriptor %d", i0 + i);
+            const bool dw = t.kind == UDA_RELAYOUT_DW || t.kind == UDA_RELAYOUT_DW_FLIP;
+            UDA_REQUIRE(dw || (t.I > 0 && t.k >= 1 && t.k <= 3), "uda_relayout_multi: bad descriptor %d", i0 + i);
+            const int64_t total = dw ? 9 * (int64_t)t.O
+                                     : (t.kind == UDA_RELAYOUT_OHWI ? (int64_t)t.O * uda_k_row(t.I, t.k) : (int64_t)t.I * uda_k_row(t.O, t.k));
+            blocks += uda_cdiv(total, 256);
+            UDA_REQUIRE(blocks < (1ll << 30), "uda_relayout_multi: too many elements in one call");
+            a.d[i] = t;
+            a.blk_end[i] = (int)blocks;
+        }
+        for (int i = m; i < UDA_RELAYOUT_MULTI_MAX; ++i) { a.d[i] = a.d[0]; a.blk_end[i] = (int)blocks; }
+        hipLaunchKernelGGL(relayout_multi_kernel, dim3((unsigned)blocks), dim3(256), 0, (hipStream_t)stream, a);
+        UDA_LAUNCH_CHECK("relayout_multi");
+    }
+    return 0;
+}
diff --git a/uda_clr_amd/engine.py b/uda_clr_amd/engine.py
--- a/uda_clr_amd/engine.py
+++ b/uda_clr_amd/engine.py
@@ -63,7 +63,7 @@
 
 
 class _Ctx:
-    __slots__ = ("S", "N", "dims", "w_cache", "params", "x", "arena", "nbt", "bnlog", "tn_repeat", "need_grad")
+    __slots__ = ("S", "N", "dims", "w_cache", "params", "x", "arena", "nbt", "bnlog", "tn_repeat", "need_grad", "phase")
 
     def __init__(self):
         self.S = {}
@@ -71,6 +71,7 @@
         self.arena = None
         self.nbt = []
         self.bnlog = []
+        self.phase = "fwd"
         self.tn_repeat = False
 
 
@@ -102,6 +103,8 @@
                  transnorm: bool = False):
         self.tn = bool(transnorm)
         self.K = DomainSplit(kernels) if self.tn else kernels
+        self._defer_wgrad = hasattr(kernels, "wgrad_deferred") and not self.tn
+        self._w_seen = {"fwd": {}, "bwd": {}}
         self.os = output_stride
         self.backbone = backbone
         self.dils = (1, 6, 12, 18) if output_stride == 16 else (1, 12, 24, 36)
@@ -161,6 +164,8 @@
     def _w(self, ctx, key, kind):
         ck = (key, kind)
         if ck not in ctx.w_cache:
+            if kind in self._W_MULTI:
+                self._w_seen[ctx.phase][ck] = True
             w = ctx.params[key]
             K, CF = self.K, self.C_FEAT
 
@@ -174,6 +179,17 @@
                                "low_ohwi": lambda t: K.relayout_ohwi(t[:, CF:].contiguous()),
                                "low_dgrad": lambda t: K.relayout_dgrad(t[:, CF:].contiguous())}[kind](w)
         return ctx.w_cache[ck]
+
+    _W_MULTI = ("ohwi", "dgrad", "dw", "dwflip")
+
+    def _prefill_w(self, ctx, phase):
+        ctx.phase = phase
+        if not hasattr(self.K, "relayout_multi"):
+            return
+        todo = [ck for ck in self._w_seen[phase] if ck not in ctx.w_cache and ck[0] in ctx.params]
+        if len(todo) > 1:
+            for ck, t in zip(todo, self.K.relayout_multi([(kind, ctx.params[key]) for key, kind in todo])):
+                ctx.w_cache[ck] = t
 
     def _bn(self, ctx, prefix, stats, count, training, scale, shift, mean=None, invstd=None,
             q1=False, N=None) -> Optional[BNRec]:
@@ -640,6 +656,7 @@
         ctx.tn_repeat = bool(repeat_prefix and self.tn)
         ctx.params, ctx.x = params, x
         ctx.need_grad = bool(need_grad)
+        self._prefill_w(ctx, "fwd")
         drop_tr = training
         training = training if bn_training is None else bool(bn_training)
         S = ctx.S
@@ -841,14 +858,19 @@
                 ctx.nbt = []
         stoch = set(self._STOCHASTIC_BN)
         det = [(prefix, rec) for prefix, rec in ctx.bnlog if prefix not in stoch]
+        recs = []
         for prefix, rec in det:
             if repeated_tn:
                 for dom in ("source", "target"):
-                    K.bn_running_replay(rec.mean, rec.invstd, rec.count, passes, BN_MOMENTUM, BN_EPS,
-                                        params[prefix + ".running_mean_" + dom], params[prefix + ".running_var_" + dom])
+                    recs.append((rec.mean, rec.invstd, rec.count, params[prefix + ".running_mean_" + dom],
+                                 params[prefix + ".running_var_" + dom]))
             else:
-                K.bn_running_replay(rec.mean, rec.invstd, rec.count * reps, passes, BN_MOMENTUM, BN_EPS,
-                                    params[prefix + ".running_mean"], params[prefix + ".running_var"])
+                recs.append((rec.mean, rec.invstd, rec.count * reps, params[prefix + ".running_mean"], params[prefix + ".running_var"]))
+        if hasattr(K, "bn_running_replay_multi") and len({r[3].data_ptr() for r in recs}) == len(recs):
+            K.bn_running_replay_multi(recs, passes, BN_MOMENTUM, BN_EPS)
+        else:
+            for mean, invstd, count, rm, rv in recs:
+                K.bn_running_replay(mean, invstd, count, passes, BN_MOMENTUM, BN_EPS, rm, rv)
         nbt = [params[p + ".num_batches_tracked"] for p, _ in det if (p + ".num_batches_tracked") in params]
         if nbt:
             torch._foreach_add_(nbt, passes)
@@ -886,7 +908,10 @@
 
     def _wgrad(self, ctx, G, key, src: Act, dy, ksize, dil, stride=1):
         dw = torch.empty_like(ctx.params[key])
-        self.K.conv_wgrad(src, dy, ksize, dil, dw, **({"stride": stride} if stride != 1 else {}))
+        kw = {"stride": stride} if stride != 1 else {}
+        if self._defer_wgrad:
+            kw["defer"] = True
+        self.K.conv_wgrad(src, dy, ksize, dil, dw, **kw)
         G[key] = dw
 
     def _dgrad(self, ctx, key, dy, N, H, W, ksize, dil, out, addend=None):
@@ -899,7 +924,14 @@
         G[key] = g
 
     def backward(self, ctx, grads):
+        if not self._defer_wgrad:
+            return self._backward(ctx, grads)
+        with self.K.wgrad_deferred():
+            return self._backward(ctx, grads)
+
+    def _backward(self, ctx, grads):
         K = self.K
+        self._prefill_w(ctx, "bwd")
         gx1, gx2, gfeat, gxbu, gxf, gx1b, gx2b = grads
         S, x = ctx.S, ctx.x
         N, Hin, Win, H16, W16, H4, W4 = ctx.dims
diff --git a/uda_clr_amd/kernels.py b/uda_clr_amd/kernels.py
--- a/uda_clr_amd/kernels.py
+++ b/uda_clr_amd/kernels.py
@@ -1,5 +1,6 @@
 from __future__ import annotations
 
+import contextlib
 import ctypes as C
 import os
 from typing import Optional
@@ -33,6 +34,20 @@
                 ("ksize", C.c_int32), ("dil", C.c_int32), ("origin", C.c_int32), ("dw", C.c_void_p),
                 ("workspace", C.c_void_p), ("workspace_bytes", C.c_uint64), ("mfma", C.c_int32), ("stride", C.c_int32),
                 ("x3_src", C.c_void_p), ("x3_dy", C.c_void_p)]
+
+
+class UdaWgradReduceDesc(C.Structure):
+    _fields_ = [("slab", C.c_void_p), ("dw", C.c_void_p), ("S", C.c_int32), ("Cout", C.c_int32), ("Cin", C.c_int32),
+                ("T", C.c_int32), ("Kc", C.c_int32)]
+
+
+class UdaRelayoutDesc(C.Structure):
+    _fields_ = [("w", C.c_void_p), ("out", C.c_void_p), ("O", C.c_int32), ("I", C.c_int32), ("k", C.c_int32), ("kind", C.c_int32)]
+
+
+class UdaBnReplayDesc(C.Structure):
+    _fields_ = [("mean", C.c_void_p), ("invstd", C.c_void_p), ("running_mean", C.c_void_p), ("running_var", C.c_void_p),
+                ("count", C.c_double), ("C", C.c_int32)]
 
 
 _P, _I, _L, _F, _D, _U = C.c_void_p, C.c_int, C.c_int64, C.c_float, C.c_double, C.c_uint64
@@ -42,6 +57,7 @@
     "uda_relayout_ohwi": (_I, [_P, _I, _I, _I, _P, _P]),
     "uda_relayout_dgrad": (_I, [_P, _I, _I, _I, _P, _P]),
     "uda_relayout_dw": (_I, [_P, _I, _P, _P]),
+    "uda_relayout_multi": (_I, [C.POINTER(UdaRelayoutDesc), _I, _P]),
     "uda_conv_fwd": (_I, [C.POINTER(UdaConvArgs), _P]),
     "uda_conv_uses_x3": (_I, [C.POINTER(UdaConvArgs)]),
     "uda_conv_fwd_workspace_bytes": (_U, [C.POINTER(UdaConvArgs)]),
@@ -50,6 +66,8 @@
     "uda_conv_wgrad_workspace_bytes": (_U, [_L, _I, _I, _I]),
     "uda_conv_wgrad": (_I, [C.POINTER(UdaWgradArgs), _P]),
     "uda_conv_wgrad_uses_x3": (_I, [C.POINTER(UdaWgradArgs)]),
+    "uda_conv_wgrad_slabs": (_I, [C.POINTER(UdaWgradArgs), C.POINTER(C.c_int32), _P]),
+    "uda_wgrad_reduce_multi": (_I, [C.POINTER(UdaWgradReduceDesc), _I, _P]),
     "uda_dwconv_workspace_bytes": (_U, [_L, _I]),
     "uda_dwconv_fwd": (_I, [C.POINTER(UdaSrc), _P, _I, _I, _I, _P, _L, _P, _P]),
     "uda_dwconv_dgrad": (_I, [_P, _L, _P, _I, _I, _I, _I, _I, _I, _P, _L, _P]),
@@ -76,6 +94,7 @@
     "uda_x3_pack_s2d_bwd": (_I, [_P, _L, _I, _I, _P, _L, _F, _I, _I, _I, _I, _I, _I, _P, _P]),
     "uda_bn_finalize": (_I, [_P, _I, _D, _P, _P, _P, _P, _F, _F, _P, _P, _P, _P, _P]),
     "uda_bn_running_replay": (_I, [_P, _P, _I, _D, _I, _F, _F, _P, _P, _P]),
+    "uda_bn_running_replay_multi": (_I, [C.POINTER(UdaBnReplayDesc), _I, _I, _F, _F, _P]),
     "uda_bn_eval_coeffs": (_I, [_P, _P, _P, _P, _I, _F, _P, _P, _P]),
     "uda_tn_gain": (_I, [_P, _P, _I, _D, _D, _F, _P, _P, _P, _P, _P, _P]),
     "uda_tn_eval_coeffs": (_I, [_P, _P, _P, _P, _P, _P, _I, _F, _P, _P, _P]),
@@ -175,6 +194,8 @@
         if mode not in ("f32", "bf16x3"):
             raise ValueError("UDA_CLR_MFMA must be 'f32' or 'bf16x3', got %r" % mode)
         self.mfma = self.MFMA_BF16X3 if mode == "bf16x3" else self.MFMA_F32
+        self._wgrad_queue = None
+        self._wgrad_queued_bytes = 0
 
     @staticmethod
     def _stream():
@@ -229,6 +250,28 @@
         out = torch.empty(9, Cc, dtype=torch.float32, device=w.device)
         self._ck(self.lib.uda_relayout_dw(w.contiguous().data_ptr(), Cc, out.data_ptr(), self._stream()))
         return out
+
+    RELAYOUT_KINDS = {"ohwi": 0, "dgrad": 1, "dw": 2, "dwflip": 3}
+
+    def relayout_multi(self, items):
+        descs, outs, keep = [], [], []
+        for kind, w in items:
+            wc = w.contiguous()
+            self._dev(wc)
+            if kind in ("dw", "dwflip"):
+                O, I, k = wc.shape[0], 0, 0
+                assert tuple(wc.shape[1:]) == (1, 3, 3)
+                out = torch.empty(9, O, dtype=torch.float32, device=w.device)
+            else:
+                O, I, k, _ = wc.shape
+                out = torch.empty(conv_weight_shape(O, k, I) if kind == "ohwi" else conv_weight_shape(I, k, O),
+                                  dtype=torch.float32, device=w.device)
+            descs.append(UdaRelayoutDesc(wc.data_ptr(), out.data_ptr(), O, I, k, self.RELAYOUT_KINDS[kind]))
+            outs.append(out)
+            keep.append(wc)
+        if descs:
+            self._ck(self.lib.uda_relayout_multi((UdaRelayoutDesc * len(descs))(*descs), len(descs), self._stream()))
+        return outs
 
     ELEM_LIMIT = 1 << 29
 
@@ -329,7 +372,30 @@
         s.act, s.ldm, s.mask_scale = 0, 0, 1.0
         return self.x3_pack(s, rows, klen, w.device)
 
-    def conv_wgrad(self, src: Act, dy, ksize, dil, dw, origin=0, stride=1):
+    WGRAD_DEFER_BYTES = 48 << 20
+    WGRAD_QUEUE_BYTES = 128 << 20
+
+    @contextlib.contextmanager
+    def wgrad_deferred(self):
+        if self._wgrad_queue is not None:
+            yield
+            return
+        self._wgrad_queue, self._wgrad_queued_bytes = [], 0
+        try:
+            yield
+            self.wgrad_flush()
+        finally:
+            self._wgrad_queue, self._wgrad_queued_bytes = None, 0
+
+    def wgrad_flush(self):
+        q = self._wgrad_queue
+        if q:
+            arr = (UdaWgradReduceDesc * len(q))(*[d for d, _, _ in q])
+            self._ck(self.lib.uda_wgrad_reduce_multi(arr, len(q), self._stream()))
+            del q[:]
+            self._wgrad_queued_bytes = 0
+
+    def conv_wgrad(self, src: Act, dy, ksize, dil, dw, origin=0, stride=1, defer=False):
         groups = self._image_groups(src.N, src.P // src.N, max(src.x.stride(0), dy.stride(0), 0 if src.mask is None else src.mask.stride(0) // 4))
         Ho, Wo = (src.H - 1) // stride + 1, (src.W - 1) // stride + 1
         Po = src.N * Ho * Wo
@@ -357,6 +423,15 @@
             dsrc = Act(dy, src.N, Ho, Wo)
             xd = self._packed(dsrc, self._src(dsrc), dy.device)
             a.x3_src, a.x3_dy = xs.data_ptr(), xd.data_ptr()
+        if defer and self._wgrad_queue is not None and ws.numel() <= self.WGRAD_DEFER_BYTES:
+            if self._wgrad_queued_bytes + ws.numel() > self.WGRAD_QUEUE_BYTES:
+                self.wgrad_flush()
+            S_used = C.c_int32(0)
+            self._ck(self.lib.uda_conv_wgrad_slabs(C.byref(a), C.byref(S_used), self._stream()))
+            d = UdaWgradReduceDesc(ws.data_ptr(), dw.data_ptr(), S_used.value, Cout, src.C, ksize * ksize, (src.C + 3) // 4 * 4)
+            self._wgrad_queue.append((d, ws, dw))
+            self._wgrad_queued_bytes += ws.numel()
+            return
         self._ck(self.lib.uda_conv_wgrad(C.byref(a), self._stream()))
 
     def dwconv_fwd(self, src: Act, w9c, stride, dil, border_mode, out, stats=None, family=""):
@@ -580,6 +655,17 @@
             assert t.is_contiguous() and t.numel() == Cc
         self._ck(self.lib.uda_bn_running_replay(mean.data_ptr(), invstd.data_ptr(), Cc, float(count), int(k), momentum, eps,
                                                 rmean.data_ptr(), rvar.data_ptr(), self._stream()))
+
+    def bn_running_replay_multi(self, records, k, momentum, eps):
+        descs = []
+        for mean, invstd, count, rmean, rvar in records:
+            Cc = mean.numel()
+            for t in (mean, invstd, rmean, rvar):
+                assert t.is_contiguous() and t.numel() == Cc and t.dtype == torch.float32
+            descs.append(UdaBnReplayDesc(mean.data_ptr(), invstd.data_ptr(), rmean.data_ptr(), rvar.data_ptr(), float(count), Cc))
+        if descs:
+            self._ck(self.lib.uda_bn_running_replay_multi((UdaBnReplayDesc * len(descs))(*descs), len(descs), int(k), momentum, eps,
+                                                          self._stream()))
 
     def bn_eval_coeffs(self, gamma, beta, rmean, rvar, eps, scale, shift):
         Cc = gamma.numel()
```

Measured after the change: 370.6 (median of 6 runs). 1.1% higher.
